# TusKANNy/seismic

Measured on AMD Instinct MI355X. Metric: queries/sec + mean latency (µs) at fixed recall@10 vs exact, SPLADE-v3 MSMARCO, higher is better.
Workload: dtype f32

## Files before the change

### include/seismic_hip_testing.h

```cpp
#ifndef SEISMIC_HIP_TESTING_H
#define SEISMIC_HIP_TESTING_H
#include "seismic_hip.h"
#ifdef __cplusplus
extern "C" {
#endif

uint32_t sgpu_debug_host_threads(void);
uint32_t sgpu_debug_chunk_bounds(uint32_t nq, uint32_t chunk_min, uint32_t chunk_max, uint32_t lanes_free, uint32_t* bounds);
uint32_t sgpu_debug_call_bounds(uint32_t nq, uint32_t chunk_min, uint32_t chunk_max, uint32_t lanes_free, uint32_t first_pm,
                                uint32_t* bounds, uint32_t cap);
uint32_t sgpu_debug_lane_chunk(sgpu_index* idx, uint32_t lane, uint32_t* info4, uint32_t* order_out, uint32_t cap);
sgpu_status sgpu_debug_pack_forward(const sgpu_index* idx, uint8_t* out_fwd, uint64_t cap, uint64_t* out_doc_ref,
                                    uint64_t* out_bytes);
sgpu_status sgpu_debug_row_dir(const sgpu_index* idx, uint32_t* out, uint64_t cap_words, uint64_t* n_words, uint32_t* n_buckets);
sgpu_status sgpu_debug_plan(const sgpu_index* idx, const uint64_t* q_off, const uint32_t* comps, const float* vals,
                            uint32_t nq, uint32_t query_cut, uint32_t* order_out, uint32_t* out3);
sgpu_status sgpu_debug_device_plan(sgpu_index* idx, const uint64_t* q_off, const uint32_t* comps, const float* vals,
                                   uint32_t nq, uint32_t query_cut, uint32_t* order_out, uint32_t* out3);
void sgpu_debug_call_timing(double* buf8);
uint32_t sgpu_debug_coop_trace(sgpu_index* idx, uint64_t* out, uint32_t cap);
sgpu_status sgpu_debug_score_stats(sgpu_index* idx, uint32_t replica, double* out8);

#ifdef __cplusplus
}
#endif
#endif
```

### seismic_amd/csrc/abi.cpp

```cpp
#include <algorithm>
#include <chrono>
#include <cstdlib>
#include <mutex>
#include <new>
#include <string>
#include <thread>
#include <vector>

#include "host_index.hpp"

struct sgpu_batch;

namespace sgpu {
struct Lane;
sgpu_status device_index_upload(const HostIndex& h, int device, DeviceIndex** out);
sgpu_status device_index_clone(const DeviceIndex* src, int device, DeviceIndex** out);
void device_index_free(DeviceIndex* d);
uint64_t device_index_bytes(const DeviceIndex* d);
Lane* lane_acquire(DeviceIndex* d);
Lane* lane_try_acquire(DeviceIndex* d);
bool call_enter(DeviceIndex* d);
void call_exit(DeviceIndex* d);
void lane_release(DeviceIndex* d, Lane* l);
Lane* lane_main(DeviceIndex* d);
sgpu_batch** lane_scratch(Lane* l);
sgpu_status batch_create(DeviceIndex* d, Lane* lane, uint64_t dim, const uint64_t* q_off, const uint32_t* comps,
                         const float* vals, uint32_t nq, uint32_t k_max, sgpu_batch** out);
void batch_free(sgpu_batch* b);
sgpu_status batch_run(DeviceIndex* d, Lane* lane, sgpu_batch* b, const sgpu_search_params& sp, uint32_t mode,
                      int sync, sgpu_launch_stats* stats);
sgpu_status batch_sync(DeviceIndex* d, sgpu_launch_stats* stats);
sgpu_status batch_fetch(DeviceIndex* d, Lane* lane, sgpu_batch* b, uint32_t k, float* out_scores, uint64_t* out_ids,
                        uint32_t* out_n);
sgpu_status batch_fetch_stats(DeviceIndex* d, sgpu_batch* b, uint32_t* out);
sgpu_status staged_launch(DeviceIndex* d, Lane* lane, uint64_t dim, const uint64_t* q_off, const uint32_t* comps,
                          const float* vals, uint32_t nq, uint32_t q_base, const sgpu_search_params& sp, sgpu_batch** slot,
                          uint32_t followed,
                          const FilterRef* flt, uint32_t chunk);
sgpu_status staged_finish(DeviceIndex* d, Lane* lane, sgpu_batch* b, float* out_scores, uint64_t* out_ids, uint32_t* out_n);
sgpu_status summary_distances(DeviceIndex* d, const HostIndex& h, uint32_t list, const uint32_t* comps,
                              const float* vals, uint32_t nnz, float* out_dots, uint32_t* out_nb);
int device_count();
double*& call_timing();
uint32_t device_plan_dots(DeviceIndex* d, const sgpu_search_params& sp, uint32_t nq, uint32_t cut);
sgpu_status debug_device_plan(DeviceIndex* d, const uint64_t* q_off, const uint32_t* comps, const float* vals, uint32_t nq,
                              uint32_t query_cut, uint32_t* order_out, uint32_t* out3);
sgpu_status debug_plan(const HostIndex& h, const uint64_t* q_off, const uint32_t* comps, const float* vals, uint32_t nq,
                       uint32_t query_cut, uint32_t* order_out, uint32_t* out3);
uint32_t coop_trace_dump(DeviceIndex* d, uint64_t* out, uint32_t cap);
uint32_t debug_lane_chunk(DeviceIndex* d, uint32_t lane, uint32_t* info4, uint32_t* order_out, uint32_t cap);
const DeviceIndex* batch_replica(const sgpu_batch* b);
sgpu_status device_index_set_knn(DeviceIndex* d, const std::vector<uint32_t>& knn, uint32_t knn_dim);
sgpu_status build_knn_on_device(DeviceIndex* d, HostIndex& h, uint32_t nknn);
sgpu_status exact_search_device(sgpu_index* idx, uint32_t replica, const uint64_t* q_off, const uint32_t* comps,
                                const float* vals, uint32_t nq, uint32_t k, float* out_scores, uint64_t* out_ids,
                                uint32_t* out_n, const sgpu_filter* filter);
sgpu_status score_documents_device(sgpu_index* idx, uint32_t replica, const uint64_t* q_off, const uint32_t* comps,
                                   const float* vals, uint32_t nq, const uint64_t* cand_off, const uint64_t* cand_ids,
                                   float* out_scores);
bool score_debug_stats(sgpu_index* idx, uint32_t replica, double* out8);
sgpu_status filter_create(sgpu_index* idx, const uint32_t* doc_ids, uint64_t n, sgpu_filter** out);
const sgpu_index* filter_index(const sgpu_filter* f);
const uint32_t* filter_host_bits(const sgpu_filter* f);
uint64_t filter_count(const sgpu_filter* f);
uint64_t filter_device_bytes(const sgpu_filter* f);
void filter_destroy(sgpu_filter* f);
bool filter_build_times(const sgpu_filter* f, uint32_t replica, double* out2);
}

using namespace sgpu;

extern "C" {

const char* sgpu_last_error(void) { return last_error().c_str(); }
uint32_t sgpu_abi_version(void) { return 4; }

sgpu_status sgpu_device_count(int32_t* n) {
  if (!n) return fail(SGPU_EINVAL, "null argument");
  *n = device_count();
  if (*n <= 0) {
    *n = 0;
    return fail(SGPU_EDEVICE, "no HIP device visible");
  }
  return SGPU_OK;
}

sgpu_status sgpu_index_create(const sgpu_index_desc* desc, sgpu_index** out) {
  if (!desc || !out) return fail(SGPU_EINVAL, "null argument");
  sgpu_index* ix = new (std::nothrow) sgpu_index();
  if (!ix) return fail(SGPU_ENOMEM, "out of memory");
  sgpu_status st = host_index_from_desc(*desc, &ix->host);
  if (st != SGPU_OK) {
    delete ix;
    return st;
  }
  *out = ix;
  return SGPU_OK;
}

sgpu_status sgpu_index_build(uint32_t comp_width, uint64_t n_docs, uint64_t dim, const uint64_t* offsets,
                             const void* comps, const float* vals, const sgpu_build_config* cfg,
                             sgpu_index** out) {
  if (!offsets || !cfg || !out || (offsets[n_docs] && (!comps || !vals))) return fail(SGPU_EINVAL, "null argument");
  sgpu_index* ix = new (std::nothrow) sgpu_index();
  if (!ix) return fail(SGPU_ENOMEM, "out of memory");
  sgpu_status st = build_host_index(comp_width, n_docs, dim, offsets, comps, vals, *cfg, &ix->host);
  if (st != SGPU_OK) {
    delete ix;
    return st;
  }
  *out = ix;
  return SGPU_OK;
}

sgpu_status sgpu_index_convert(const sgpu_index* src, uint32_t value_type, sgpu_index** out) {
  if (!src || !out) return fail(SGPU_EINVAL, "null argument");
  sgpu_index* ix = new (std::nothrow) sgpu_index();
  if (!ix) return fail(SGPU_ENOMEM, "out of memory");
  sgpu_status st = host_index_convert(src->host, value_type, &ix->host);
  if (st != SGPU_OK) {
    delete ix;
    return st;
  }
  *out = ix;
  return SGPU_OK;
}

sgpu_status sgpu_index_get_desc(const sgpu_index* idx, sgpu_index_desc* out) {
  if (!idx || !out) return fail(SGPU_EINVAL, "null argument");
  idx->host.fill_desc(out);
  return SGPU_OK;
}

sgpu_status sgpu_index_save(const sgpu_index* idx, const char* path) {
  if (!idx || !path) return fail(SGPU_EINVAL, "null argument");
  return host_index_save(idx->host, path);
}

sgpu_status sgpu_index_load(const char* path, sgpu_index** out) {
  if (!path || !out) return fail(SGPU_EINVAL, "null argument");
  sgpu_index* ix = new (std::nothrow) sgpu_index();
  if (!ix) return fail(SGPU_ENOMEM, "out of memory");
  sgpu_status st = host_index_load(path, &ix->host);
  if (st != SGPU_OK) {
    delete ix;
    return st;
  }
  *out = ix;
  return SGPU_OK;
}

struct GenerationBump {
  sgpu_index* idx;
  ~GenerationBump() { idx->generation.fetch_add(1, std::memory_order_acq_rel); }
};

static void drop_replicas(sgpu_index* idx) {
  for (ExactFile* f : idx->exact) exact_file_free(f);
  idx->exact.clear();
  for (ScoreState* s : idx->score) score_state_free(s);
  idx->score.clear();
  for (DeviceIndex* d : idx->replicas) device_index_free(d);
  idx->replicas.clear();
  idx->dev = nullptr;
}

sgpu_status sgpu_index_upload_many(sgpu_index* idx, const int32_t* device_ids, uint32_t n) {
  if (!idx || !device_ids || n == 0) return fail(SGPU_EINVAL, "null argument / no device given");
  GenerationBump bump{idx};
  drop_replicas(idx);
  DeviceIndex* first = nullptr;
  sgpu_status st = device_index_upload(idx->host, device_ids[0], &first);
  if (st != SGPU_OK) return st;
  idx->replicas.push_back(first);
  idx->dev = first;
  for (uint32_t i = 1; i < n; ++i) {
    DeviceIndex* r = nullptr;
    st = device_index_clone(first, device_ids[i], &r);
    if (st != SGPU_OK) {
      const std::string msg = last_error();
      drop_replicas(idx);
      last_error() = msg;
      return st;
    }
    idx->replicas.push_back(r);
  }
  return SGPU_OK;
}

sgpu_status sgpu_index_upload(sgpu_index* idx, int32_t device) { return sgpu_index_upload_many(idx, &device, 1); }

uint32_t sgpu_index_replicas(const sgpu_index* idx) { return idx ? (uint32_t)idx->replicas.size() : 0; }

sgpu_status sgpu_index_set_knn(sgpu_index* idx, const uint32_t* neighbours, uint64_t n_total, uint32_t knn_dim) {
  if (!idx || (n_total && !neighbours)) return fail(SGPU_EINVAL, "null argument");
  if (n_total && knn_dim == 0) return fail(SGPU_EINVAL, "knn_dim == 0 with a non-empty neighbour array");
  for (uint64_t i = 0; i < n_total; ++i)
    if (neighbours[i] >= idx->host.n_docs) return fail(SGPU_EINVAL, "neighbour id >= n_docs");
  GenerationBump bump{idx};
  try {
    idx->host.knn.assign(neighbours, neighbours + n_total);
  } catch (const std::bad_alloc&) {
    return fail(SGPU_ENOMEM, "out of memory");
  }
  idx->host.knn_dim = n_total ? knn_dim : 0;
  for (DeviceIndex* d : idx->replicas) {
    sgpu_status st = device_index_set_knn(d, idx->host.knn, idx->host.knn_dim);
    if (st != SGPU_OK) return st;
  }
  return SGPU_OK;
}

sgpu_status sgpu_index_get_knn(const sgpu_index* idx, const uint32_t** neighbours, uint64_t* n_total,
                               uint32_t* knn_dim) {
  if (!idx || !neighbours || !n_total || !knn_dim) return fail(SGPU_EINVAL, "null argument");
  *neighbours = idx->host.knn.data();
  *n_total = idx->host.knn.size();
  *knn_dim = idx->host.knn_dim;
  return SGPU_OK;
}

sgpu_status sgpu_index_build_knn(sgpu_index* idx, uint32_t nknn) {
  if (!idx) return fail(SGPU_EINVAL, "null argument");
  GenerationBump bump{idx};
  try {
    sgpu_status st = build_knn_on_device(idx->dev, idx->host, nknn);
    for (size_t i = 1; st == SGPU_OK && i < idx->replicas.size(); ++i)
      st = device_index_set_knn(idx->replicas[i], idx->host.knn, idx->host.knn_dim);
    return st;
  } catch (const std::exception&) {
    return fail(SGPU_ENOMEM, "out of host memory building the kNN graph");
  }
}

uint64_t sgpu_index_device_bytes(const sgpu_index* idx) { return idx ? device_index_bytes(idx->dev) : 0; }

sgpu_status sgpu_index_stream_stats(const sgpu_index* idx, uint64_t* raw_docs, uint64_t* raw_elements) {
  if (!idx || !raw_docs || !raw_elements) return fail(SGPU_EINVAL, "null argument");
  *raw_docs = *raw_elements = 0;
  try {
    std::vector<uint8_t> raw;
    pack_dvb_raw_flags(idx->host, &raw);
    for (uint64_t d = 0; d < raw.size(); ++d)
      if (raw[d]) {
        *raw_docs += 1;
        *raw_elements += idx->host.fwd_offsets[d + 1] - idx->host.fwd_offsets[d];
      }
  } catch (const std::bad_alloc&) {
    return fail(SGPU_ENOMEM, "out of host memory");
  }
  return SGPU_OK;
}

void sgpu_index_destroy(sgpu_index* idx) {
  if (!idx) return;
  drop_replicas(idx);
  delete idx;
}

static DeviceIndex* replica_of(sgpu_index* idx, uint32_t replica) {
  if (!idx || replica >= idx->replicas.size()) {
    fail(SGPU_EDEVICE, "index is not uploaded to a device (call sgpu_index_upload) / replica out of range");
    return nullptr;
  }
  return idx->replicas[replica];
}
static DeviceIndex* replica_of_batch(sgpu_index* idx, const sgpu_batch* b) {
  for (DeviceIndex* d : idx->replicas)
    if (batch_replica(b) == d) return d;
  fail(SGPU_EINVAL, "batch does not belong to this index");
  return nullptr;
}

sgpu_status sgpu_batch_create_on(sgpu_index* idx, uint32_t replica, const uint64_t* q_off, const uint32_t* comps,
                                 const float* vals, uint32_t nq, uint32_t k_max, sgpu_batch** out) {
  if (!idx || !q_off || !out || (q_off[nq] && (!comps || !vals))) return fail(SGPU_EINVAL, "null argument");
  *out = nullptr;
  DeviceIndex* d = replica_of(idx, replica);
  if (!d) return SGPU_EDEVICE;
  return batch_create(d, lane_main(d), idx->host.dim, q_off, comps, vals, nq, k_max, out);
}

sgpu_status sgpu_batch_create(sgpu_index* idx, const uint64_t* q_off, const uint32_t* comps, const float* vals,
                              uint32_t nq, uint32_t k_max, sgpu_batch** out) {
  return sgpu_batch_create_on(idx, 0, q_off, comps, vals, nq, k_max, out);
}

sgpu_status sgpu_batch_run(sgpu_index* idx, sgpu_batch* batch, const sgpu_search_params* params, int32_t sync,
                           sgpu_launch_stats* stats) {
  if (!idx || !batch || !params) return fail(SGPU_EINVAL, "null argument");
  DeviceIndex* d = replica_of_batch(idx, batch);
  if (!d) return SGPU_EINVAL;
  return batch_run(d, nullptr, batch, *params, 0 , sync, stats);
}

sgpu_status sgpu_batch_run_counted(sgpu_index* idx, sgpu_batch* batch, const sgpu_search_params* params,
                                   sgpu_launch_stats* stats) {
  if (!idx || !batch || !params) return fail(SGPU_EINVAL, "null argument");
  DeviceIndex* d = replica_of_batch(idx, batch);
  if (!d) return SGPU_EINVAL;
  return batch_run(d, nullptr, batch, *params, 2 , 1, stats);
}

sgpu_status sgpu_batch_sync(sgpu_index* idx, sgpu_launch_stats* stats) {
  if (!idx) return fail(SGPU_EINVAL, "null argument");
  for (size_t i = idx->replicas.size(); i-- > 1;) {
    sgpu_status st = batch_sync(idx->replicas[i], nullptr);
    if (st != SGPU_OK) return st;
  }
  return batch_sync(idx->dev, stats);
}

sgpu_status sgpu_batch_fetch(sgpu_index* idx, sgpu_batch* batch, uint32_t k, float* out_scores,
                             uint64_t* out_doc_ids, uint32_t* out_n) {
  if (!idx || !batch || !out_scores || !out_doc_ids || !out_n) return fail(SGPU_EINVAL, "null argument");
  DeviceIndex* d = replica_of_batch(idx, batch);
  if (!d) return SGPU_EINVAL;
  return batch_fetch(d, nullptr, batch, k, out_scores, out_doc_ids, out_n);
}

sgpu_status sgpu_batch_fetch_stats(sgpu_index* idx, sgpu_batch* batch, uint32_t* out_counters) {
  if (!idx || !batch || !out_counters) return fail(SGPU_EINVAL, "null argument");
  DeviceIndex* d = replica_of_batch(idx, batch);
  if (!d) return SGPU_EINVAL;
  return batch_fetch_stats(d, batch, out_counters);
}

void sgpu_batch_destroy(sgpu_batch* batch) { batch_free(batch); }

static uint32_t chunk_jobs(uint32_t nq, uint32_t chunk_min, uint32_t chunk_max) {
  if (!chunk_min) return 1u;
  const uint32_t by_rule = nq >= 2 * (uint64_t)chunk_min ? std::min<uint32_t>(chunk_max, nq / chunk_min) : 1u;
  const uint32_t by_size = (uint32_t)std::min<uint64_t>(((uint64_t)nq + kChunkQueriesMax - 1) / kChunkQueriesMax, 8u);
  return std::max(by_rule, by_size);
}
static void chunk_bounds(uint32_t nq, uint32_t n_jobs, uint32_t j, uint32_t* q0, uint32_t* q1, uint32_t first_pm = 0) {
  if (first_pm == 0 || first_pm >= 1000 || n_jobs < 2) {
    *q0 = (uint32_t)((uint64_t)nq * j / n_jobs);
    *q1 = (uint32_t)((uint64_t)nq * (j + 1) / n_jobs);
    return;
  }
  const uint32_t first = std::min<uint32_t>(std::max<uint32_t>((uint32_t)((uint64_t)nq * first_pm / 1000), 1u), nq - (n_jobs - 1));
  const uint32_t rest = nq - first;
  *q0 = j == 0 ? 0u : first + (uint32_t)((uint64_t)rest * (j - 1) / (n_jobs - 1));
  *q1 = j == 0 ? first : first + (uint32_t)((uint64_t)rest * j / (n_jobs - 1));
}
static uint32_t call_segments(uint32_t nq) {
  return (uint32_t)std::max<uint64_t>(((uint64_t)nq + 8ull * kChunkQueriesMax - 1) / (8ull * kChunkQueriesMax), 1u);
}

static sgpu_status search_segment(DeviceIndex* d, uint64_t dim, const uint64_t* q_off, const uint32_t* comps,
                                  const float* vals, uint32_t s0, uint32_t s1, uint32_t q_base, const sgpu_search_params& params,
                                  float* out_scores, uint64_t* out_doc_ids, uint32_t* out_n, const FilterRef* flt, bool shared) {
  static const uint32_t chunk_min = [] {
    const char* v = std::getenv("SGPU_CHUNK_MIN");
    return v && *v ? (uint32_t)std::strtoul(v, nullptr, 10) : 0xffffffffu;
  }();
  struct Job {
    Lane* lane;
    uint32_t q0, q1;
  };
  static const uint32_t chunk_max_env = [] {
    const char* v = std::getenv("SGPU_CHUNK_MAX");
    const uint32_t n = v && *v ? (uint32_t)std::strtoul(v, nullptr, 10) : 0u;
    return n > 8 ? 8u : n;
  }();
  static const uint32_t chunk_first_pm = [] {
    const char* t = std::getenv("SGPU_TEST_HOOKS");
    const char* v = (t && *t && *t != '0') ? std::getenv("SGPU_CHUNK_FIRST") : nullptr;
    return v && *v ? (uint32_t)std::strtoul(v, nullptr, 10) : 0u;
  }();
  const uint32_t nq = s1 - s0;
  const bool device_plans = device_plan_dots(d, params, std::min<uint32_t>(std::max<uint32_t>(nq / 2, 1u), kChunkQueriesMax), params.query_cut) != 0;
  const uint32_t chunk_max = chunk_max_env ? chunk_max_env : ((shared || device_plans) ? 2u : 4u);
  Job jobs[8];
  const uint32_t cmin = chunk_min != 0xffffffffu ? chunk_min : (device_plans ? 1300u : 600u);
  uint32_t n_jobs = chunk_jobs(nq, cmin, chunk_max);
  jobs[0].lane = lane_acquire(d);
  for (uint32_t j = 1; j < n_jobs; ++j) {
    jobs[j].lane = lane_try_acquire(d);
    if (!jobs[j].lane) {
      n_jobs = j;
      break;
    }
  }
  std::vector<uint64_t> off;
  for (;;) {
    uint32_t longest = 0;
    for (uint32_t j = 0; j < n_jobs; ++j) {
      chunk_bounds(nq, n_jobs, j, &jobs[j].q0, &jobs[j].q1, chunk_first_pm);
      jobs[j].q0 += s0;
      jobs[j].q1 += s0;
      if (jobs[j].q0 != 0) longest = std::max(longest, jobs[j].q1 - jobs[j].q0);
    }
    if (n_jobs == 1 && s0 == 0) break;
    try {
      off.resize((size_t)longest + 1);
      break;
    } catch (const std::exception&) {
      if (n_jobs == 1) {
        lane_release(d, jobs[0].lane);
        return fail(SGPU_ENOMEM, "out of host memory cutting a query batch");
      }
      for (uint32_t j = 1; j < n_jobs; ++j) lane_release(d, jobs[j].lane);
      n_jobs = 1;
    }
  }
  const uint32_t k = params.k;
  sgpu_status st = SGPU_OK;
  std::string msg;
  uint32_t launched = 0;
  if (n_jobs > 1 || s0 != 0) {
    uint32_t max_nnz = 0;
    st = q_off[0] != 0 ? fail(SGPU_EINVAL, "q_off[0] must be 0") : validate_query_offsets(q_off + s0, nq, q_base + s0, &max_nnz);
    if (st != SGPU_OK) msg = last_error();
  }
  for (uint32_t j = 0; j < n_jobs && st == SGPU_OK; ++j) {
    Job& jb = jobs[j];
    const uint64_t* qo = q_off;
    if (jb.q0 != 0) {
      for (uint32_t q = jb.q0; q <= jb.q1; ++q) off[q - jb.q0] = q_off[q] - q_off[jb.q0];
      qo = off.data();
    }
    st = staged_launch(d, jb.lane, dim, qo, comps ? comps + q_off[jb.q0] : nullptr, vals ? vals + q_off[jb.q0] : nullptr,
                       jb.q1 - jb.q0, q_base + jb.q0, params, lane_scratch(jb.lane), j + 1 < n_jobs ? 2u : (shared ? 1u : 0u),
                       flt, j);
    if (st == SGPU_OK) ++launched;
    else msg = last_error();
  }
  for (uint32_t j = 0; j < launched; ++j) {
    Job& jb = jobs[j];
    const sgpu_status fs = staged_finish(d, jb.lane, *lane_scratch(jb.lane), out_scores + (size_t)jb.q0 * k,
                                         out_doc_ids + (size_t)jb.q0 * k, out_n + jb.q0);
    if (fs != SGPU_OK && st == SGPU_OK) {
      st = fs;
      msg = last_error();
    }
  }
  for (uint32_t j = 0; j < n_jobs; ++j) lane_release(d, jobs[j].lane);
  if (st != SGPU_OK) last_error() = msg;
  return st;
}

static sgpu_status search_shard(DeviceIndex* d, uint64_t dim, const uint64_t* q_off, const uint32_t* comps,
                                const float* vals, uint32_t nq, uint32_t q_base, const sgpu_search_params& params,
                                float* out_scores, uint64_t* out_doc_ids, uint32_t* out_n, const FilterRef* flt) {
  struct InFlight {
    DeviceIndex* d;
    bool shared;
    explicit InFlight(DeviceIndex* d_) : d(d_), shared(call_enter(d_)) {}
    ~InFlight() { call_exit(d); }
  } in_flight(d);
  const uint32_t n_seg = call_segments(nq);
  sgpu_status st = SGPU_OK;
  for (uint32_t s = 0; s < n_seg && st == SGPU_OK; ++s)
    st = search_segment(d, dim, q_off, comps, vals, (uint32_t)((uint64_t)nq * s / n_seg), (uint32_t)((uint64_t)nq * (s + 1) / n_seg),
                        q_base, params, out_scores, out_doc_ids, out_n, flt, in_flight.shared);
  return st;
}

}

static sgpu_status batch_search(sgpu_index* idx, const uint64_t* q_off, const uint32_t* comps, const float* vals,
                                uint32_t nq, const sgpu_search_params* params, float* out_scores,
                                uint64_t* out_doc_ids, uint32_t* out_n, const sgpu_filter* filter) {
  if (!idx || !params || !q_off || !out_scores || !out_doc_ids || !out_n) return fail(SGPU_EINVAL, "null argument");
  if (params->k == 0) return fail(SGPU_EINVAL, "k must be > 0 (KHeap::new asserts, reference src/utils.rs:23)");
  if (idx->replicas.empty()) return fail(SGPU_EDEVICE, "index is not uploaded to a device (call sgpu_index_upload)");
  if (q_off[nq] && (!comps || !vals)) return fail(SGPU_EINVAL, "null argument");
  const uint32_t n_rep = (uint32_t)idx->replicas.size();
  if (n_rep == 1) {
    const FilterRef fr{filter, 0};
    return search_shard(idx->dev, idx->host.dim, q_off, comps, vals, nq, 0, *params, out_scores, out_doc_ids, out_n,
                        filter ? &fr : nullptr);
  }
  if (nq < 2 * n_rep) {
    const uint32_t r = idx->next_replica.fetch_add(1, std::memory_order_relaxed) % n_rep;
    const FilterRef fr{filter, r};
    return search_shard(idx->replicas[r], idx->host.dim, q_off, comps, vals, nq, 0, *params, out_scores, out_doc_ids, out_n,
                        filter ? &fr : nullptr);
  }
  {
    uint32_t max_nnz = 0;
    if (q_off[0] != 0) return fail(SGPU_EINVAL, "q_off[0] must be 0");
    const sgpu_status vst = validate_query_offsets(q_off, nq, 0, &max_nnz);
    if (vst != SGPU_OK) return vst;
  }
  const uint32_t k = params->k;
  try {
    std::vector<sgpu_status> sts(n_rep, SGPU_OK);
    std::vector<std::string> msgs(n_rep);
    std::vector<std::vector<uint64_t>> offs(n_rep);
    for (uint32_t r = 0; r < n_rep; ++r) {
      const uint32_t q0 = (uint32_t)((uint64_t)nq * r / n_rep), q1 = (uint32_t)((uint64_t)nq * (r + 1) / n_rep);
      offs[r].resize(q1 - q0 + 1);
      for (uint32_t q = q0; q <= q1; ++q) offs[r][q - q0] = q_off[q] - q_off[q0];
    }
    auto shard = [&](uint32_t r) {
      const uint32_t q0 = (uint32_t)((uint64_t)nq * r / n_rep), q1 = (uint32_t)((uint64_t)nq * (r + 1) / n_rep);
      try {
        const FilterRef fr{filter, r};
        sts[r] = search_shard(idx->replicas[r], idx->host.dim, offs[r].data(), comps ? comps + q_off[q0] : nullptr,
                              vals ? vals + q_off[q0] : nullptr, q1 - q0, q0, *params, out_scores + (size_t)q0 * k,
                              out_doc_ids + (size_t)q0 * k, out_n + q0, filter ? &fr : nullptr);
        if (sts[r] != SGPU_OK) msgs[r] = last_error();
      } catch (const std::exception&) {
        sts[r] = SGPU_ENOMEM;
      }
    };
    std::vector<std::thread> threads;
    threads.reserve(n_rep);
    for (uint32_t r = 1; r < n_rep; ++r) {
      try {
        threads.emplace_back(shard, r);
      } catch (const std::exception&) {
        shard(r);
      }
    }
    shard(0);
    for (auto& t : threads) t.join();
    for (uint32_t r = 0; r < n_rep; ++r)
      if (sts[r] != SGPU_OK) {
        if (msgs[r].empty()) return fail(sts[r], "out of host memory searching shard %u", r);
        last_error() = msgs[r];
        return sts[r];
      }
  } catch (const std::exception&) {
    return fail(SGPU_ENOMEM, "out of host memory sharding a query batch");
  }
  return SGPU_OK;
}

static sgpu_status foreign_filter(const sgpu_index* idx, const sgpu_filter* filter) {
  return filter && filter_index(filter) != idx ? fail(SGPU_EINVAL, "the filter was created on another index") : SGPU_OK;
}

extern "C" {

sgpu_status sgpu_batch_search(sgpu_index* idx, const uint64_t* q_off, const uint32_t* comps, const float* vals,
                              uint32_t nq, const sgpu_search_params* params, float* out_scores,
                              uint64_t* out_doc_ids, uint32_t* out_n) {
  return batch_search(idx, q_off, comps, vals, nq, params, out_scores, out_doc_ids, out_n, nullptr);
}

sgpu_status sgpu_batch_search_filtered(sgpu_index* idx, const uint64_t* q_off, const uint32_t* comps, const float* vals,
                                       uint32_t nq, const sgpu_search_params* params, float* out_scores,
                                       uint64_t* out_doc_ids, uint32_t* out_n, const sgpu_filter* filter) {
  const sgpu_status st = foreign_filter(idx, filter);
  if (st != SGPU_OK) return st;
  return batch_search(idx, q_off, comps, vals, nq, params, out_scores, out_doc_ids, out_n, filter);
}

sgpu_status sgpu_search_filtered(sgpu_index* idx, const uint32_t* comps, const float* vals, uint32_t nnz,
                                 const sgpu_search_params* params, float* out_scores, uint64_t* out_doc_ids,
                                 uint32_t* out_n, const sgpu_filter* filter) {
  const uint64_t q_off[2] = {0, nnz};
  return sgpu_batch_search_filtered(idx, q_off, comps, vals, 1, params, out_scores, out_doc_ids, out_n, filter);
}

sgpu_status sgpu_filter_create(sgpu_index* idx, const uint32_t* doc_ids, uint64_t n, sgpu_filter** out) {
  return filter_create(idx, doc_ids, n, out);
}
uint64_t sgpu_filter_count(const sgpu_filter* filter) { return filter_count(filter); }
uint64_t sgpu_filter_device_bytes(const sgpu_filter* filter) { return filter_device_bytes(filter); }
void sgpu_filter_destroy(sgpu_filter* filter) { filter_destroy(filter); }

sgpu_status sgpu_search(sgpu_index* idx, const uint32_t* comps, const float* vals, uint32_t nnz,
                        const sgpu_search_params* params, float* out_scores, uint64_t* out_doc_ids,
                        uint32_t* out_n) {
  const uint64_t q_off[2] = {0, nnz};
  return sgpu_batch_search(idx, q_off, comps, vals, 1, params, out_scores, out_doc_ids, out_n);
}

sgpu_status sgpu_search_sequential_timed(sgpu_index* idx, const uint64_t* q_off, const uint32_t* comps, const float* vals,
                                         uint32_t nq, const sgpu_search_params* params, float* out_scores,
                                         uint64_t* out_doc_ids, uint32_t* out_n, double* mean_us, double* breakdown_us,
                                         double* per_query_us) {
  if (!idx || !params || !q_off || !out_scores || !out_doc_ids || !out_n) return fail(SGPU_EINVAL, "null argument");
  if (params->k == 0) return fail(SGPU_EINVAL, "k must be > 0 (KHeap::new asserts, reference src/utils.rs:23)");
  double phases[8] = {0, 0, 0, 0, 0, 0, 0, 0};
  double*& slot = call_timing();
  double* const saved = slot;
  if (breakdown_us) slot = phases;
  const uint32_t k = params->k;
  sgpu_status st = SGPU_OK;
  const auto t0 = std::chrono::steady_clock::now();
  for (uint32_t q = 0; q < nq && st == SGPU_OK; ++q) {
    if (q_off[q + 1] < q_off[q] || q_off[q + 1] - q_off[q] > 0xffffffffull) {
      st = fail(SGPU_EINVAL, "query offsets must be monotone (query %u)", q);
      break;
    }
    const auto tq = per_query_us ? std::chrono::steady_clock::now() : t0;
    st = sgpu_search(idx, comps ? comps + q_off[q] : nullptr, vals ? vals + q_off[q] : nullptr,
                     (uint32_t)(q_off[q + 1] - q_off[q]), params, out_scores + (size_t)q * k,
                     out_doc_ids + (size_t)q * k, out_n + q);
    if (per_query_us) per_query_us[q] = std::chrono::duration<double, std::micro>(std::chrono::steady_clock::now() - tq).count();
  }
  const double total = std::chrono::duration<double, std::micro>(std::chrono::steady_clock::now() - t0).count();
  slot = saved;
  if (mean_us) *mean_us = nq ? total / nq : 0.0;
  if (breakdown_us)
    for (int i = 0; i < 8; ++i) breakdown_us[i] = nq ? phases[i] / nq : 0.0;
  return st;
}

sgpu_status sgpu_search_sequential(sgpu_index* idx, const uint64_t* q_off, const uint32_t* comps, const float* vals,
                                   uint32_t nq, const sgpu_search_params* params, float* out_scores,
                                   uint64_t* out_doc_ids, uint32_t* out_n, double* mean_us, double* breakdown_us) {
  return sgpu_search_sequential_timed(idx, q_off, comps, vals, nq, params, out_scores, out_doc_ids, out_n, mean_us,
                                      breakdown_us, nullptr);
}

static bool test_hooks_on() {
  const char* t = std::getenv("SGPU_TEST_HOOKS");
  return t && *t && *t != '0';
}
#define SGPU_HOOK_OR(ret)                                                                            \
  if (!test_hooks_on()) {                                                                            \
    (void)fail(SGPU_EINVAL, "%s is a test hook: set SGPU_TEST_HOOKS=1 (include/seismic_hip_testing.h)", __func__); \
    return ret;                                                                                      \
  }

uint32_t sgpu_debug_host_threads(void) {
  SGPU_HOOK_OR(0u);
  return (uint32_t)host_threads();
}

uint32_t sgpu_debug_chunk_bounds(uint32_t nq, uint32_t chunk_min, uint32_t chunk_max, uint32_t lanes_free, uint32_t* bounds) {
  SGPU_HOOK_OR(0u);
  uint32_t n_jobs = chunk_jobs(nq, chunk_min, chunk_max < 1 ? 1 : (chunk_max > 8 ? 8 : chunk_max));
  if (lanes_free >= 1 && n_jobs > lanes_free) n_jobs = lanes_free;
  for (uint32_t j = 0; j < n_jobs; ++j) chunk_bounds(nq, n_jobs, j, bounds + 2 * j, bounds + 2 * j + 1);
  return n_jobs;
}

uint32_t sgpu_debug_call_bounds(uint32_t nq, uint32_t chunk_min, uint32_t chunk_max, uint32_t lanes_free, uint32_t first_pm,
                                uint32_t* bounds, uint32_t cap) {
  SGPU_HOOK_OR(0u);
  const uint32_t n_seg = call_segments(nq);
  uint32_t n = 0;
  for (uint32_t s = 0; s < n_seg; ++s) {
    const uint32_t s0 = (uint32_t)((uint64_t)nq * s / n_seg), s1 = (uint32_t)((uint64_t)nq * (s + 1) / n_seg);
    uint32_t n_jobs = chunk_jobs(s1 - s0, chunk_min, chunk_max < 1 ? 1 : (chunk_max > 8 ? 8 : chunk_max));
    if (lanes_free >= 1 && n_jobs > lanes_free) n_jobs = lanes_free;
    for (uint32_t j = 0; j < n_jobs; ++j, ++n) {
      uint32_t q0, q1;
      chunk_bounds(s1 - s0, n_jobs, j, &q0, &q1, first_pm);
      if (n < cap) {
        bounds[2 * n] = s0 + q0;
        bounds[2 * n + 1] = s0 + q1;
      }
    }
  }
  return n;
}

uint32_t sgpu_debug_lane_chunk(sgpu_index* idx, uint32_t lane, uint32_t* info4, uint32_t* order_out, uint32_t cap) {
  SGPU_HOOK_OR(0u);
  if (!idx || !idx->dev || !info4) return 0u;
  return debug_lane_chunk(idx->dev, lane, info4, order_out, cap);
}

sgpu_status sgpu_debug_pack_forward(const sgpu_index* idx, uint8_t* out_fwd, uint64_t cap, uint64_t* out_doc_ref, uint64_t* out_bytes) {
  SGPU_HOOK_OR(SGPU_EINVAL);
  if (!idx || !out_bytes) return fail(SGPU_EINVAL, "null argument");
  try {
    std::vector<uint8_t> raw, fwd;
    std::vector<uint64_t> off16, dref;
    pack_dvb_raw_flags(idx->host, &raw);
    pack_record_offsets(idx->host, raw, 128 / 16, &off16);
    *out_bytes = std::max<uint64_t>(off16[idx->host.n_docs] * 16, 16);
    if (!out_fwd) return SGPU_OK;
    if (cap < *out_bytes || !out_doc_ref) return fail(SGPU_EINVAL, "buffer too small");
    pack_records(idx->host, raw, off16, &fwd);
    pack_doc_refs(idx->host, raw, off16, &dref);
    std::memcpy(out_fwd, fwd.data(), fwd.size());
    std::memcpy(out_doc_ref, dref.data(), dref.size() * 8);
  } catch (const std::bad_alloc&) {
    return fail(SGPU_ENOMEM, "out of host memory");
  }
  return SGPU_OK;
}

sgpu_status sgpu_debug_row_dir(const sgpu_index* idx, uint32_t* out, uint64_t cap_words, uint64_t* n_words, uint32_t* n_buckets) {
  SGPU_HOOK_OR(SGPU_EINVAL);
  if (!idx || !n_words || !n_buckets) return fail(SGPU_EINVAL, "null argument");
  try {
    std::vector<uint16_t> mid;
    std::vector<uint32_t> dir;
    pack_row_mid(idx->host, &mid);
    *n_buckets = 0;
    if (!pack_row_dir(idx->host, mid, &dir, n_buckets)) *n_buckets = 0;
    *n_words = dir.size();
    if (!out) return SGPU_OK;
    if (cap_words < dir.size()) return fail(SGPU_EINVAL, "buffer too small");
    std::memcpy(out, dir.data(), dir.size() * 4);
  } catch (const std::bad_alloc&) {
    return fail(SGPU_ENOMEM, "out of host memory");
  }
  return SGPU_OK;
}

sgpu_status sgpu_debug_plan(const sgpu_index* idx, const uint64_t* q_off, const uint32_t* comps, const float* vals, uint32_t nq,
                            uint32_t query_cut, uint32_t* order_out, uint32_t* out3) {
  SGPU_HOOK_OR(SGPU_EINVAL);
  if (!idx || !q_off || !order_out || !out3) return fail(SGPU_EINVAL, "null argument");
  return debug_plan(idx->host, q_off, comps, vals, nq, query_cut, order_out, out3);
}

sgpu_status sgpu_debug_device_plan(sgpu_index* idx, const uint64_t* q_off, const uint32_t* comps, const float* vals, uint32_t nq,
                                   uint32_t query_cut, uint32_t* order_out, uint32_t* out3) {
  SGPU_HOOK_OR(SGPU_EINVAL);
  if (!idx || !q_off || !order_out || !out3) return fail(SGPU_EINVAL, "null argument");
  return debug_device_plan(idx->dev, q_off, comps, vals, nq, query_cut, order_out, out3);
}

void sgpu_debug_call_timing(double* buf8) {
  SGPU_HOOK_OR();
  call_timing() = buf8;
}

uint32_t sgpu_debug_coop_trace(sgpu_index* idx, uint64_t* out, uint32_t cap) {
  SGPU_HOOK_OR(0u);
  return idx ? coop_trace_dump(idx->dev, out, cap) : 0;
}

sgpu_status sgpu_summary_distances(sgpu_index* idx, uint32_t list, const uint32_t* comps, const float* vals,
                                   uint32_t nnz, float* out_dots, uint32_t* out_n_blocks) {
  if (!idx || !out_dots || !out_n_blocks || (nnz && (!comps || !vals))) return fail(SGPU_EINVAL, "null argument");
  return summary_distances(idx->dev, idx->host, list, comps, vals, nnz, out_dots, out_n_blocks);
}

sgpu_status sgpu_exact_search(const sgpu_index* idx, const uint64_t* q_off, const uint32_t* comps,
                              const float* vals, uint32_t nq, uint32_t k, uint32_t num_threads,
                              float* out_scores, uint64_t* out_doc_ids, uint32_t* out_n) {
  if (!idx || !q_off || !out_scores || !out_doc_ids || !out_n) return fail(SGPU_EINVAL, "null argument");
  return exact_search_host(idx->host, q_off, comps, vals, nq, k, num_threads, out_scores, out_doc_ids, out_n);
}

sgpu_status sgpu_exact_search_filtered(const sgpu_index* idx, const uint64_t* q_off, const uint32_t* comps,
                                       const float* vals, uint32_t nq, uint32_t k, uint32_t num_threads,
                                       float* out_scores, uint64_t* out_doc_ids, uint32_t* out_n,
                                       const sgpu_filter* filter) {
  if (!filter) return sgpu_exact_search(idx, q_off, comps, vals, nq, k, num_threads, out_scores, out_doc_ids, out_n);
  const sgpu_status st = foreign_filter(idx, filter);
  if (st != SGPU_OK) return st;
  if (!idx || !q_off || !out_scores || !out_doc_ids || !out_n) return fail(SGPU_EINVAL, "null argument");
  return exact_search_host(idx->host, q_off, comps, vals, nq, k, num_threads, out_scores, out_doc_ids, out_n,
                           filter_host_bits(filter));
}

sgpu_status sgpu_exact_search_device(sgpu_index* idx, uint32_t replica, const uint64_t* q_off, const uint32_t* comps,
                                     const float* vals, uint32_t nq, uint32_t k, float* out_scores,
                                     uint64_t* out_doc_ids, uint32_t* out_n) {
  return exact_search_device(idx, replica, q_off, comps, vals, nq, k, out_scores, out_doc_ids, out_n, nullptr);
}

sgpu_status sgpu_exact_search_device_filtered(sgpu_index* idx, uint32_t replica, const uint64_t* q_off,
                                              const uint32_t* comps, const float* vals, uint32_t nq, uint32_t k,
                                              float* out_scores, uint64_t* out_doc_ids, uint32_t* out_n,
                                              const sgpu_filter* filter) {
  const sgpu_status st = foreign_filter(idx, filter);
  if (st != SGPU_OK) return st;
  return exact_search_device(idx, replica, q_off, comps, vals, nq, k, out_scores, out_doc_ids, out_n, filter);
}

sgpu_status sgpu_score_documents(sgpu_index* idx, uint32_t replica, const uint64_t* q_off, const uint32_t* comps,
                                 const float* vals, uint32_t nq, const uint64_t* cand_off, const uint64_t* cand_ids,
                                 float* out_scores) {
  return score_documents_device(idx, replica, q_off, comps, vals, nq, cand_off, cand_ids, out_scores);
}

sgpu_status sgpu_score_documents_host(const sgpu_index* idx, const uint64_t* q_off, const uint32_t* comps, const float* vals,
                                      uint32_t nq, const uint64_t* cand_off, const uint64_t* cand_ids, uint32_t num_threads,
                                      float* out_scores) {
  if (!idx) return fail(SGPU_EINVAL, "null argument");
  return score_documents_host(idx->host, q_off, comps, vals, nq, cand_off, cand_ids, num_threads, out_scores);
}

sgpu_status sgpu_debug_score_stats(sgpu_index* idx, uint32_t replica, double* out8) {
  SGPU_HOOK_OR(SGPU_EINVAL);
  if (!idx || !out8) return fail(SGPU_EINVAL, "null argument");
  if (!score_debug_stats(idx, replica, out8)) return fail(SGPU_EINVAL, "no score call has run on replica %u", replica);
  return SGPU_OK;
}

sgpu_status sgpu_debug_filter_build_times(const sgpu_filter* filter, uint32_t replica, double* out2) {
  SGPU_HOOK_OR(SGPU_EINVAL);
  if (!filter || !out2) return fail(SGPU_EINVAL, "null argument");
  if (!filter_build_times(filter, replica, out2)) return fail(SGPU_EINVAL, "the filter has no view on replica %u", replica);
  return SGPU_OK;
}

}
```

### seismic_amd/csrc/device_index.hip

```cpp
#include <hip/hip_runtime.h>

#include <algorithm>
#include <atomic>
#include <chrono>
#include <cmath>
#include <condition_variable>
#include <cstdlib>
#include <cstring>
#include <mutex>
#include <unordered_map>
#include <vector>

#include "device_types.hpp"
#include "filter.hpp"
#include "host_index.hpp"

namespace sgpu {

hipError_t run_u16_dense(const LaunchArgs& a, int* occupancy);
hipError_t run_u16_packed(const LaunchArgs& a, int* occupancy);
hipError_t run_u32_split(const LaunchArgs& a, int* occupancy);
hipError_t run_u32_packed(const LaunchArgs& a, int* occupancy);
hipError_t run_u32_hash(const LaunchArgs& a, int* occupancy);
hipError_t run_u16_dense_u8(const LaunchArgs& a, int* occupancy);
hipError_t run_u16_packed_u8(const LaunchArgs& a, int* occupancy);
hipError_t run_u32_packed_u8(const LaunchArgs& a, int* occupancy);
hipError_t run_u32_split_u8(const LaunchArgs& a, int* occupancy);
hipError_t run_u16_dense_dvb(const LaunchArgs& a, int* occupancy);
hipError_t run_u16_packed_dvb(const LaunchArgs& a, int* occupancy);

static hipError_t run_any(const LaunchArgs& a, int* occ) {
  if (a.comp_width == 2 && a.lookup != LK_DENSE && a.lookup != LK_PACKED) return hipErrorInvalidConfiguration;
  if (a.value_type == SGPU_VAL_DOTVBYTE)
    return a.lookup == LK_DENSE ? run_u16_dense_dvb(a, occ) : run_u16_packed_dvb(a, occ);
  if (a.value_type == SGPU_VAL_FIXEDU8 && a.comp_width == 4) return a.lookup == LK_SPLIT ? run_u32_split_u8(a, occ) : run_u32_packed_u8(a, occ);
  if (a.value_type == SGPU_VAL_FIXEDU8) return a.lookup == LK_DENSE ? run_u16_dense_u8(a, occ) : run_u16_packed_u8(a, occ);
  if (a.comp_width == 2) return a.lookup == LK_DENSE ? run_u16_dense(a, occ) : run_u16_packed(a, occ);
  if (a.lookup == LK_HASH) return run_u32_hash(a, occ);
  return a.lookup == LK_SPLIT ? run_u32_split(a, occ) : run_u32_packed(a, occ);
}
hipError_t occupancy_search(const LaunchArgs& a, int* blocks_per_cu) { return run_any(a, blocks_per_cu); }
hipError_t launch_search(const LaunchArgs& a) { return run_any(a, nullptr); }

#define HIP_TRY(expr)                                                                          \
  do {                                                                                         \
    hipError_t e_ = (expr);                                                                    \
    if (e_ != hipSuccess)                                                                      \
      return fail(SGPU_EDEVICE, "%s failed: %s (%s:%d)", #expr, hipGetErrorString(e_), __FILE__, __LINE__); \
  } while (0)

static const char* hook_raw(const char* name) {
  const char* t = std::getenv("SGPU_TEST_HOOKS");
  return (t && *t && *t != '0') ? std::getenv(name) : nullptr;
}

}
struct sgpu_batch;
namespace sgpu {
void batch_free(sgpu_batch* b);

struct Lane {
  hipStream_t stream = nullptr;
  uint32_t* queue = nullptr;
  uint32_t queue_pos = 0;
  bool queue_dirty = true;
  uint32_t done_seq = 0;
  sgpu_batch* scratch = nullptr;
  uint32_t* bitmaps = nullptr;
  uint32_t bitmaps_slots = 0;
  uint8_t* coop = nullptr;
  size_t coop_bytes = 0, coop_trace_off = 0;
  uint32_t coop_trace_n = 0;
  bool coop_last = false;
  std::vector<hipEvent_t> ev0, ev1;
  int ev_pending = 0;
  double sum_ms = 0;
  uint32_t n_timed = 0;
  sgpu_launch_stats last{};
  bool busy = false;
};

struct Alloc {
  void* p;
  size_t bytes;
  size_t field;
};

struct DeviceIndex {
  int device = -1;
  DevView view{};
  uint32_t comp_width = 2;
  std::vector<Alloc> allocs;
  uint64_t bytes = 0;
  uint32_t n_cu = 0;
  uint32_t max_lds = 0;
  std::vector<uint32_t> list_nb, list_np;
  uint32_t max_nb = 0;
  uint32_t value_type = SGPU_VAL_F16;
  float val_scale = 0.0f;
  bool fwd_block_major = false;
  bool coop_broken = false;
  static constexpr int kMainEvents = 64, kPool = 8;
  Lane main;
  Lane pool[kPool];
  std::unordered_map<uint64_t, int> occupancy;
  std::unordered_map<uint32_t, uint32_t> plan_dots_seen;
  std::mutex mu;
  std::atomic<uint32_t> calls_inflight{0};
  std::atomic<int64_t> concurrent_seen_us{-((int64_t)1 << 60)};
  std::mutex pool_mu;
  std::condition_variable pool_cv;
};

static sgpu_status lane_init(Lane* l, int n_events) {
  if (hipStreamCreateWithFlags(&l->stream, hipStreamNonBlocking) != hipSuccess)
    return fail(SGPU_EDEVICE, "hipStreamCreate failed");
  if (hipMalloc((void**)&l->queue, 256) != hipSuccess) return fail(SGPU_ENOMEM, "hipMalloc(queue) failed");
  if (hipMemset(l->queue, 0, 256) != hipSuccess) return fail(SGPU_EDEVICE, "hipMemset(queue) failed");
  for (int i = 0; i < n_events; ++i) {
    hipEvent_t a, b;
    if (hipEventCreate(&a) != hipSuccess) return fail(SGPU_EDEVICE, "hipEventCreate failed");
    l->ev0.push_back(a);
    if (hipEventCreate(&b) != hipSuccess) return fail(SGPU_EDEVICE, "hipEventCreate failed");
    l->ev1.push_back(b);
  }
  return SGPU_OK;
}

static void lane_free(Lane* l) {
  if (l->stream) (void)hipStreamSynchronize(l->stream);
  if (l->scratch) batch_free(l->scratch);
  if (l->queue) (void)hipFree(l->queue);
  if (l->bitmaps) (void)hipFree(l->bitmaps);
  if (l->coop) (void)hipFree(l->coop);
  for (hipEvent_t e : l->ev0) (void)hipEventDestroy(e);
  for (hipEvent_t e : l->ev1) (void)hipEventDestroy(e);
  if (l->stream) (void)hipStreamDestroy(l->stream);
  *l = Lane{};
}

Lane* lane_acquire(DeviceIndex* d) {
  std::unique_lock<std::mutex> lk(d->pool_mu);
  for (;;) {
    for (Lane& l : d->pool)
      if (!l.busy) {
        l.busy = true;
        return &l;
      }
    d->pool_cv.wait(lk);
  }
}

Lane* lane_try_acquire(DeviceIndex* d) {
  std::lock_guard<std::mutex> lk(d->pool_mu);
  int n_free = 0;
  for (Lane& l : d->pool) n_free += !l.busy;
  if (n_free < 2) return nullptr;
  for (Lane& l : d->pool)
    if (!l.busy) {
      l.busy = true;
      return &l;
    }
  return nullptr;
}

static inline int64_t mono_us() {
  return (int64_t)std::chrono::duration_cast<std::chrono::microseconds>(std::chrono::steady_clock::now().time_since_epoch()).count();
}
bool call_enter(DeviceIndex* d) {
  const uint32_t n = d->calls_inflight.fetch_add(1, std::memory_order_relaxed) + 1u;
  const int64_t now = mono_us();
  if (n > 1) d->concurrent_seen_us.store(now, std::memory_order_relaxed);
  return n > 1 || now - d->concurrent_seen_us.load(std::memory_order_relaxed) < 50000;
}
void call_exit(DeviceIndex* d) {
  if (d->calls_inflight.fetch_sub(1, std::memory_order_relaxed) > 1u) d->concurrent_seen_us.store(mono_us(), std::memory_order_relaxed);
}

void lane_release(DeviceIndex* d, Lane* l) {
  {
    std::lock_guard<std::mutex> lk(d->pool_mu);
    l->busy = false;
  }
  d->pool_cv.notify_one();
}

Lane* lane_main(DeviceIndex* d) { return &d->main; }
sgpu_batch** lane_scratch(Lane* l) { return &l->scratch; }

template <class T>
static sgpu_status dev_copy(DeviceIndex* d, const T* src, size_t n, const T** out) {
  void* p = nullptr;
  const size_t bytes = std::max<size_t>(n, 1) * sizeof(T);
  if (hipMalloc(&p, bytes) != hipSuccess) return fail(SGPU_ENOMEM, "hipMalloc of %zu bytes failed", bytes);
  d->allocs.push_back(Alloc{p, bytes, (size_t)((const char*)out - (const char*)d)});
  d->bytes += bytes;
  if (hook_raw("SGPU_DEBUG_ALLOC")) std::fprintf(stderr, "sgpu alloc: field@%zu %p..%p\n", (size_t)((const char*)out - (const char*)d), p, (void*)((char*)p + bytes));
  if (n) HIP_TRY(hipMemcpy(p, src, n * sizeof(T), hipMemcpyHostToDevice));
  *out = (const T*)p;
  return SGPU_OK;
}

void device_index_free(DeviceIndex* d) {
  if (!d) return;
  if (d->device >= 0) (void)hipSetDevice(d->device);
  lane_free(&d->main);
  for (Lane& l : d->pool) lane_free(&l);
  for (const Alloc& a : d->allocs) (void)hipFree(a.p);
  delete d;
}

uint64_t device_index_bytes(const DeviceIndex* d) { return d ? d->bytes : 0; }
int device_index_device(const DeviceIndex* d) { return d->device; }
const DevView& device_index_view(const DeviceIndex* d) { return d->view; }

int device_count() {
  int n = 0;
  if (hipGetDeviceCount(&n) != hipSuccess) return 0;
  return n;
}

__global__ __launch_bounds__(256) void replicate_records_kernel(uint8_t* fwd, const uint64_t* __restrict__ doc_ref,
                                                                const uint32_t* __restrict__ post_doc,
                                                                const uint64_t* __restrict__ post_ref, uint64_t n_postings,
                                                                uint32_t bytes_per_elem, uint32_t dvb) {
  const uint64_t g = ((uint64_t)blockIdx.x * blockDim.x + threadIdx.x) >> 4;
  const uint32_t sub = threadIdx.x & 15;
  const uint64_t n_groups = ((uint64_t)gridDim.x * blockDim.x) >> 4;
  for (uint64_t p = g; p < n_postings; p += n_groups) {
    const uint64_t dst = post_ref[p], src = doc_ref[post_doc[p]];
    uint32_t n16;
    if (dvb && !(dst & 0x8000u)) {
      const uint32_t ns = (((uint32_t)dst & 0x7fffu) + 7u) >> 3;
      n16 = (ns * 20u + 15u) >> 4;
    } else {
      const uint32_t len = (uint32_t)dst & (dvb ? 0x7fffu : 0xffffu);
      n16 = (((len + 7u) & ~7u) * bytes_per_elem + 15u) >> 4;
    }
    const uint4* s4 = (const uint4*)(fwd + (src >> 16) * 16ull);
    uint4* d4 = (uint4*)(fwd + (dst >> 16) * 16ull);
    for (uint32_t i = sub; i < n16; i += 16) d4[i] = s4[i];
  }
}

sgpu_status device_index_upload(const HostIndex& h, int device, DeviceIndex** out) {
  int n_dev = 0;
  if (hipGetDeviceCount(&n_dev) != hipSuccess || n_dev <= 0)
    return fail(SGPU_EDEVICE, "no HIP device available (the search path has no CPU fallback)");
  if (device < 0 || device >= n_dev) return fail(SGPU_EDEVICE, "device %d out of range (0..%d)", device, n_dev - 1);
  if (h.n_blocks() >= 0xffffffffull || h.n_postings() >= 0xffffffffull || h.n_rows() >= 0xffffffffull)
    return fail(SGPU_ELIMIT, "index too large for 32-bit device offsets (blocks / postings / summary rows)");
  HIP_TRY(hipSetDevice(device));
  DeviceIndex* d = new DeviceIndex();
  d->device = device;
  d->comp_width = h.comp_width;
  sgpu_status st = SGPU_OK;
  auto bail = [&](sgpu_status s) {
    device_index_free(d);
    return s;
  };
  hipDeviceProp_t prop;
  if (hipGetDeviceProperties(&prop, device) != hipSuccess) return bail(fail(SGPU_EDEVICE, "hipGetDeviceProperties failed"));
  d->n_cu = (uint32_t)prop.multiProcessorCount;
  d->max_lds = (uint32_t)prop.sharedMemPerBlock;
  if ((st = lane_init(&d->main, DeviceIndex::kMainEvents)) != SGPU_OK) return bail(st);
  for (Lane& l : d->pool)
    if ((st = lane_init(&l, 1)) != SGPU_OK) return bail(st);

  try {
    const uint32_t cw = h.comp_width, vb = h.val_bytes();
    d->value_type = h.value_type;
    d->val_scale = h.val_scale;
    std::vector<uint64_t> rec_off16;
    std::vector<uint8_t> dvb_raw;
    pack_dvb_raw_flags(h, &dvb_raw);
    {
      const char* env_line = hook_raw("SGPU_REC_LINE");
      pack_record_offsets(h, dvb_raw, std::max<uint64_t>(16, env_line ? std::strtoul(env_line, nullptr, 10) : 128) / 16, &rec_off16);
    }
    if (rec_off16[h.n_docs] >= (1ull << 48)) return bail(fail(SGPU_ELIMIT, "forward index exceeds 48-bit record offsets"));
    std::vector<uint8_t> fwd;
    pack_records(h, dvb_raw, rec_off16, &fwd);
    const uint64_t doc_units = rec_off16[h.n_docs];
    std::vector<uint64_t> pref;
    uint64_t blk_units = 0;
    {
      std::vector<uint64_t> bsize;
      pack_block_sizes(h, dvb_raw, &bsize);
      blk_units = bsize[h.n_blocks()];
      size_t free_b = 0, total_b = 0;
      (void)hipMemGetInfo(&free_b, &total_b);
      const char* env_layout = std::getenv("SGPU_FWD_LAYOUT");
      const uint64_t need = (doc_units + blk_units) * 16 + h.n_postings() * 24 + h.n_entries() * 8;
      bool block_major = blk_units > 0 && (doc_units + 8 + blk_units) < (1ull << 48) &&
                         need < (uint64_t)(0.6 * (double)free_b) && blk_units * 16 <= (96ull << 30);
      if (env_layout && std::strcmp(env_layout, "doc") == 0) block_major = false;
      if (env_layout && std::strcmp(env_layout, "block") == 0 && blk_units > 0) block_major = true;
      const uint64_t blk_base = (doc_units + 7) & ~7ull;
      void* fp = nullptr;
      size_t fbytes = 0;
      for (;;) {
        const uint64_t total_units = block_major ? blk_base + blk_units : doc_units;
        fbytes = std::max<uint64_t>(total_units * 16, 16) + 16;
        if (hipMalloc(&fp, fbytes) == hipSuccess) break;
        (void)hipGetLastError();
        if (!block_major) return bail(fail(SGPU_ENOMEM, "hipMalloc of %zu bytes failed", fbytes));
        block_major = false;
      }
      d->fwd_block_major = block_major;
      pack_post_refs(h, dvb_raw, rec_off16, bsize, block_major, blk_base, &pref);
      d->allocs.push_back(Alloc{fp, fbytes, (size_t)((const char*)&d->view.fwd - (const char*)d)});
      d->bytes += fbytes;
      d->view.fwd = (const uint8_t*)fp;
      if (hook_raw("SGPU_DEBUG_ALLOC")) std::fprintf(stderr, "sgpu alloc: fwd %p..%p\n", fp, (void*)((char*)fp + fbytes));
      HIP_TRY(hipMemcpy(fp, fwd.data(), fwd.size(), hipMemcpyHostToDevice));
    }
    fwd.clear();
    fwd.shrink_to_fit();
    if ((st = dev_copy(d, pref.data(), pref.size(), &d->view.post_ref)) != SGPU_OK) return bail(st);
    {
      std::vector<uint64_t> dref;
      pack_doc_refs(h, dvb_raw, rec_off16, &dref);
      if ((st = dev_copy(d, dref.data(), dref.size(), &d->view.doc_ref)) != SGPU_OK) return bail(st);
    }
    pref.clear();
    pref.shrink_to_fit();
    if ((st = dev_copy(d, h.post_doc.data(), h.post_doc.size(), &d->view.post_doc)) != SGPU_OK) return bail(st);
    if (d->fwd_block_major && h.n_postings()) {
      (void)hipGetLastError();
      hipLaunchKernelGGL(replicate_records_kernel, dim3(d->n_cu * 8), dim3(256), 0, d->main.stream,
                         (uint8_t*)d->view.fwd, d->view.doc_ref, d->view.post_doc, d->view.post_ref,
                         (uint64_t)h.n_postings(), (uint32_t)(cw + vb), (uint32_t)(!dvb_raw.empty()));
      HIP_TRY(hipGetLastError());
      HIP_TRY(hipStreamSynchronize(d->main.stream));
    }
    auto narrow = [](const std::vector<uint64_t>& v) {
      std::vector<uint32_t> o;
      pack_narrow(v, &o);
      return o;
    };
    {
      auto v = narrow(h.list_block_start);
      if ((st = dev_copy(d, v.data(), v.size(), &d->view.list_block_start)) != SGPU_OK) return bail(st);
      v = narrow(h.block_post_start);
      if ((st = dev_copy(d, v.data(), v.size(), &d->view.block_post_start)) != SGPU_OK) return bail(st);
    }
    if ((st = dev_copy(d, h.sum_bid.data(), h.sum_bid.size(), &d->view.sum_bid)) != SGPU_OK) return bail(st);
    {
      std::vector<uint16_t> mid;
      pack_row_mid(h, &mid);
      d->view.list_row_start = nullptr;
      d->view.row_ptr = nullptr;
      d->view.row_comp = nullptr;
      d->view.row_mid = nullptr;
      d->view.row_dir = nullptr;
      d->view.row_dir_buckets = 0;
      if (cw == 2) {
        std::vector<uint32_t> dir;
        uint32_t n_buckets = 0;
        if (!pack_row_dir(h, mid, &dir, &n_buckets))
          return bail(fail(SGPU_ELIMIT, h.dim > 65535 ? "u16 components need dim <= 65535 for the device's row directory"
                                                       : "the index has too many summary rows for the device's row directory (2^31 buckets)"));
        static_assert(sizeof(d->view.row_dir) == sizeof(const uint32_t*), "pointer field");
        if ((st = dev_copy(d, dir.data(), dir.size(), (const uint32_t**)&d->view.row_dir)) != SGPU_OK) return bail(st);
        d->view.row_dir_buckets = n_buckets;
      } else {
        auto v = narrow(h.list_row_start);
        if ((st = dev_copy(d, v.data(), v.size(), &d->view.list_row_start)) != SGPU_OK) return bail(st);
        if ((st = dev_copy(d, h.row_ptr.data(), h.row_ptr.size(), &d->view.row_ptr)) != SGPU_OK) return bail(st);
        static_assert(sizeof(d->view.row_comp) == sizeof(const uint8_t*), "pointer field");
        if ((st = dev_copy(d, h.row_comp.data(), h.row_comp.size(), (const uint8_t**)&d->view.row_comp)) != SGPU_OK)
          return bail(st);
        if ((st = dev_copy(d, mid.data(), mid.size(), &d->view.row_mid)) != SGPU_OK) return bail(st);
      }
    }
    {
      std::vector<float> deq;
      pack_sum_deq(h, &deq);
      if ((st = dev_copy(d, deq.data(), deq.size(), &d->view.sum_deq)) != SGPU_OK) return bail(st);
    }
    d->view.knn = nullptr;
    d->view.knn_total = 0;
    d->view.knn_dim = 0;
    if (!h.knn.empty() && h.knn_dim) {
      if ((st = dev_copy(d, h.knn.data(), h.knn.size(), &d->view.knn)) != SGPU_OK) return bail(st);
      d->view.knn_total = h.knn.size();
      d->view.knn_dim = h.knn_dim;
    }
    d->view.dim = (uint32_t)h.dim;
    d->view.n_docs = (uint32_t)h.n_docs;
    d->view.n_bitmap_words = (uint32_t)((h.n_docs + 31) / 32);
    d->list_nb.resize(h.dim);
    d->list_np.resize(h.dim);
    for (uint64_t c = 0; c < h.dim; ++c) {
      d->list_nb[c] = (uint32_t)(h.list_block_start[c + 1] - h.list_block_start[c]);
      d->list_np[c] = (uint32_t)(h.block_post_start[h.list_block_start[c + 1]] - h.block_post_start[h.list_block_start[c]]);
      d->max_nb = std::max(d->max_nb, d->list_nb[c]);
    }
  } catch (const std::bad_alloc&) {
    return bail(fail(SGPU_ENOMEM, "out of host memory packing the index for upload"));
  }
  *out = d;
  return SGPU_OK;
}

sgpu_status device_index_clone(const DeviceIndex* src, int device, DeviceIndex** out) {
  int n_dev = 0;
  if (hipGetDeviceCount(&n_dev) != hipSuccess || n_dev <= 0) return fail(SGPU_EDEVICE, "no HIP device available");
  if (device < 0 || device >= n_dev) return fail(SGPU_EDEVICE, "device %d out of range (0..%d)", device, n_dev - 1);
  HIP_TRY(hipSetDevice(device));
  if (device != src->device) {
    int can = 0;
    (void)hipDeviceCanAccessPeer(&can, device, src->device);
    if (can) {
      const hipError_t e = hipDeviceEnablePeerAccess(src->device, 0);
      if (e != hipSuccess && e != hipErrorPeerAccessAlreadyEnabled) (void)hipGetLastError();
    }
  }
  DeviceIndex* d = new DeviceIndex();
  d->device = device;
  d->comp_width = src->comp_width;
  d->view = src->view;
  d->n_cu = src->n_cu;
  d->max_lds = src->max_lds;
  d->list_nb = src->list_nb;
  d->list_np = src->list_np;
  d->max_nb = src->max_nb;
  d->fwd_block_major = src->fwd_block_major;
  d->value_type = src->value_type;
  d->val_scale = src->val_scale;
  auto bail = [&](sgpu_status s) {
    device_index_free(d);
    return s;
  };
  hipDeviceProp_t prop;
  if (hipGetDeviceProperties(&prop, device) != hipSuccess) return bail(fail(SGPU_EDEVICE, "hipGetDeviceProperties failed"));
  d->n_cu = (uint32_t)prop.multiProcessorCount;
  d->max_lds = (uint32_t)prop.sharedMemPerBlock;
  sgpu_status st;
  if ((st = lane_init(&d->main, DeviceIndex::kMainEvents)) != SGPU_OK) return bail(st);
  for (Lane& l : d->pool)
    if ((st = lane_init(&l, 1)) != SGPU_OK) return bail(st);
  for (const Alloc& a : src->allocs) *(const void**)((char*)d + a.field) = nullptr;
  for (const Alloc& a : src->allocs) {
    void* p = nullptr;
    if (hipMalloc(&p, a.bytes) != hipSuccess) return bail(fail(SGPU_ENOMEM, "hipMalloc of %zu bytes failed on device %d", a.bytes, device));
    d->allocs.push_back(Alloc{p, a.bytes, a.field});
    d->bytes += a.bytes;
    *(const void**)((char*)d + a.field) = p;
    const hipError_t e = hipMemcpyPeerAsync(p, device, a.p, src->device, a.bytes, d->main.stream);
    if (e != hipSuccess) return bail(fail(SGPU_EDEVICE, "hipMemcpyPeerAsync %d -> %d failed: %s", src->device, device, hipGetErrorString(e)));
  }
  if (hipStreamSynchronize(d->main.stream) != hipSuccess) return bail(fail(SGPU_EDEVICE, "peer copy failed"));
  *out = d;
  return SGPU_OK;
}

}

struct sgpu_batch_plan {
  uint32_t query_cut = 0;
  uint32_t dots_cap = 1;
  uint32_t max_nb = 0;
  uint32_t max_list_nb = 1;
  std::vector<uint32_t> order;
  bool hash_ok = true;
};

struct sgpu_batch {
  std::vector<uint64_t> h_off;
  std::vector<uint32_t> h_off32;
  std::vector<uint32_t> h_comp;
  std::vector<float> h_val;
  std::vector<sgpu_batch_plan> plans;
  int device = -1;
  const sgpu::DeviceIndex* owner = nullptr;
  uint32_t nq = 0, k_max = 0, max_nnz = 0;
  uint64_t cap_nq = 0, cap_nnz = 0, cap_slab = 0;
  uint32_t* q_off = nullptr;
  uint32_t* q_comp = nullptr;
  float* q_val = nullptr;
  uint32_t* q_order = nullptr;
  uint32_t* h_order = nullptr;
  uint32_t order_cut = 0xffffffffu;
  float* out_scores = nullptr;
  uint64_t* out_ids = nullptr;
  uint32_t* out_n = nullptr;
  uint32_t* out_stats = nullptr;
  uint32_t* status = nullptr;
  size_t status_off = 0;
  bool staged = false;
  uint8_t* arena_dev = nullptr;
  uint8_t* arena_host = nullptr;
  uint8_t* arena_host_dev = nullptr;
  bool direct_out = false;
  uint32_t done_seq = 0;
  bool direct_in = false;
  uint32_t queue_base = 0;
  size_t arena_cap = 0, in_bytes = 0, out_off = 0, out_bytes = 0;
  uint32_t* queue_dev = nullptr;
  uint32_t device_plan_cut = 0xffffffffu;
  bool followed = false;
  bool plan_identity = false;
  uint32_t q_base = 0;
  size_t order_off = 0;
};

namespace sgpu {

}
extern char** environ;
namespace sgpu {
struct EnvCache {
  uint64_t fp = 0;
  int n = 0;
  struct E {
    const char* name;
    const char* val;
  } e[96];
};
static thread_local EnvCache tl_env;
static void env_refresh() {
  uint64_t h = 1469598103934665603ull;
  for (char** p = environ; p && *p; ++p) h = (h ^ (uint64_t)(uintptr_t)*p) * 1099511628211ull;
  if (h != tl_env.fp || tl_env.n == 0) {
    tl_env.fp = h;
    tl_env.n = 0;
  }
}
static const char* env_get(const char* name) {
  EnvCache& c = tl_env;
  for (int i = 0; i < c.n; ++i)
    if (c.e[i].name == name) return c.e[i].val;
  const char* v = std::getenv(name);
  if (c.n < (int)(sizeof(c.e) / sizeof(c.e[0]))) c.e[c.n++] = EnvCache::E{name, v};
  return v;
}
static uint32_t env_u32(const char* name, uint32_t dflt) {
  const char* v = env_get(name);
  if (!v || !*v) return dflt;
  return (uint32_t)std::strtoul(v, nullptr, 10);
}
static bool hooks_on() {
  const char* v = env_get("SGPU_TEST_HOOKS");
  return v && *v && *v != '0';
}
static void hook_ignored(const char* name) {
  static std::atomic<bool> said{false};
  const char* v = env_get(name);
  if (v && *v && !said.exchange(true))
    std::fprintf(stderr, "seismic_hip: %s is a test hook and is ignored unless SGPU_TEST_HOOKS=1 is set (further ignored hooks are not reported)\n", name);
}
static uint32_t hook_u32(const char* name, uint32_t dflt) {
  if (hooks_on()) return env_u32(name, dflt);
  hook_ignored(name);
  return dflt;
}
static const char* hook_get(const char* name) {
  if (hooks_on()) return env_get(name);
  hook_ignored(name);
  return nullptr;
}

double*& call_timing() {
  static thread_local double* t = nullptr;
  return t;
}
static inline double now_us() {
  return (double)std::chrono::duration_cast<std::chrono::nanoseconds>(std::chrono::steady_clock::now().time_since_epoch()).count() * 1e-3;
}
struct PhaseClock {
  double* acc;
  double t;
  PhaseClock() : acc(call_timing()), t(acc ? now_us() : 0.0) {}
  inline void lap(int i) {
    if (!acc) return;
    const double n = now_us();
    acc[i] += n - t;
    t = n;
  }
};

static hipError_t wait_lane(hipStream_t s, uint32_t nq, const volatile uint32_t* done = nullptr, uint32_t done_seq = 0) {
  const char* wv = env_get("SGPU_WAIT");
  const int mode = (wv && !std::strcmp(wv, "block")) ? 0 : ((wv && !std::strcmp(wv, "spin")) ? 2 : 1);
  const double spin_us = (double)env_u32("SGPU_SPIN_US", 2000);
  if (mode == 2 || (mode == 1 && nq <= 256)) {
    const double t0 = now_us();
    for (;;) {
      if (done && __atomic_load_n((const uint32_t*)done, __ATOMIC_ACQUIRE) == done_seq) return hipSuccess;
      const hipError_t e = hipStreamQuery(s);
      if (e == hipSuccess) return hipSuccess;
      if (e != hipErrorNotReady) return e;
      if (now_us() - t0 > spin_us) break;
#if defined(__x86_64__) || defined(__i386__)
      __builtin_ia32_pause();
#elif defined(__aarch64__)
      asm volatile("yield");
#endif
    }
  }
  return hipStreamSynchronize(s);
}

void batch_free(sgpu_batch* b) {
  if (!b) return;
  if (b->device >= 0) (void)hipSetDevice(b->device);
  if (b->staged) {
    (void)hipFree(b->arena_dev);
    (void)hipHostFree(b->arena_host);
    delete b;
    return;
  }
  (void)hipFree(b->q_off);
  (void)hipFree(b->q_comp);
  (void)hipFree(b->q_val);
  (void)hipFree(b->q_order);
  (void)hipHostFree(b->h_order);
  (void)hipFree(b->out_scores);
  (void)hipFree(b->out_ids);
  (void)hipFree(b->out_n);
  (void)hipFree(b->out_stats);
  delete b;
}

sgpu_status batch_create(DeviceIndex* d, Lane* lane, uint64_t dim, const uint64_t* q_off, const uint32_t* comps,
                         const float* vals, uint32_t nq, uint32_t k_max, sgpu_batch** out) {
  if (!d) return fail(SGPU_EDEVICE, "index is not uploaded to a device (call sgpu_index_upload)");
  if (k_max == 0) return fail(SGPU_EINVAL, "k == 0");
  if (k_max > 1024) return fail(SGPU_ELIMIT, "k = %u exceeds the heap limit of 1024", k_max);
  uint32_t max_nnz = 0;
  sgpu_status st = validate_queries(dim, q_off, comps, vals, nq, &max_nnz);
  if (st != SGPU_OK) return st;
  HIP_TRY(hipSetDevice(d->device));
  const uint64_t nnz = q_off[nq];
  const size_t slab = std::max<size_t>((size_t)nq * k_max, 1);
  sgpu_batch* b = *out;
  const bool reuse = b && b->owner == d && b->cap_nq >= nq && b->cap_nnz >= nnz && b->cap_slab >= slab;
  if (b && !reuse) {
    HIP_TRY(hipStreamSynchronize(lane->stream));
    batch_free(b);
    b = nullptr;
    *out = nullptr;
  }
  if (reuse) HIP_TRY(hipStreamSynchronize(lane->stream));
  try {
    if (!b) b = new sgpu_batch();
    b->device = d->device;
    b->owner = d;
    b->nq = nq;
    b->k_max = k_max;
    b->max_nnz = max_nnz;
    b->plans.clear();
    b->order_cut = 0xffffffffu;
    b->h_off.assign(q_off, q_off + nq + 1);
    b->h_comp.assign(comps, comps + nnz);
    b->h_val.assign(vals, vals + nnz);
    b->h_off32.resize((size_t)nq + 1);
  } catch (const std::bad_alloc&) {
    if (!reuse) delete b;
    else b->nq = 0;
    return fail(SGPU_ENOMEM, "out of host memory creating a query batch");
  }
  for (uint32_t q = 0; q <= nq; ++q) b->h_off32[q] = (uint32_t)q_off[q];
  bool ok = true;
  if (!reuse) {
    b->cap_nq = std::max<uint64_t>(nq, 1);
    b->cap_nnz = std::max<uint64_t>(nnz, 1);
    b->cap_slab = slab;
    ok = hipMalloc((void**)&b->q_off, (b->cap_nq + 1) * 4) == hipSuccess &&
         hipMalloc((void**)&b->q_comp, b->cap_nnz * 4) == hipSuccess &&
         hipMalloc((void**)&b->q_val, b->cap_nnz * 4) == hipSuccess &&
         hipMalloc((void**)&b->q_order, b->cap_nq * 8) == hipSuccess &&
         hipHostMalloc((void**)&b->h_order, b->cap_nq * 8, hipHostMallocDefault) == hipSuccess &&
         hipMalloc((void**)&b->out_scores, std::max<size_t>(slab, 65536) * 4) == hipSuccess &&
         hipMalloc((void**)&b->out_ids, slab * 8) == hipSuccess &&
         hipMalloc((void**)&b->out_n, b->cap_nq * 4) == hipSuccess &&
         hipMalloc((void**)&b->out_stats, b->cap_nq * STATS_WORDS * 4) == hipSuccess;
  }
  if (!ok) {
    batch_free(b);
    *out = nullptr;
    return fail(SGPU_ENOMEM, "hipMalloc failed creating a query batch");
  }
  ok = hipMemcpyAsync(b->q_off, b->h_off32.data(), (nq + 1) * 4, hipMemcpyHostToDevice, lane->stream) == hipSuccess &&
       (nnz == 0 ||
        (hipMemcpyAsync(b->q_comp, b->h_comp.data(), nnz * 4, hipMemcpyHostToDevice, lane->stream) == hipSuccess &&
         hipMemcpyAsync(b->q_val, b->h_val.data(), nnz * 4, hipMemcpyHostToDevice, lane->stream) == hipSuccess));
  if (!ok) {
    (void)hipStreamSynchronize(lane->stream);
    batch_free(b);
    *out = nullptr;
    return fail(SGPU_EDEVICE, "hipMemcpy of the query batch failed");
  }
  *out = b;
  return SGPU_OK;
}

const DeviceIndex* batch_replica(const sgpu_batch* b) { return b ? b->owner : nullptr; }
static inline size_t al16_(size_t x) { return (x + 15) & ~(size_t)15; }

static sgpu_status make_plan(const DeviceIndex* d, const uint64_t* h_off, const uint32_t* h_comp, const float* h_val,
                             uint32_t nq, uint32_t query_cut, sgpu_batch_plan* out) {
  try {
    sgpu_batch_plan& pl = *out;
    pl.query_cut = query_cut;
    std::vector<uint64_t> keys(nq);
    uint32_t max_nb = 0, dots_cap = 1, max_list_nb = 1;
    {
      constexpr uint32_t kSmall = 16;
      std::vector<std::pair<int32_t, uint32_t>> kv;
      for (int64_t q = 0; q < (int64_t)nq; ++q) {
        const uint64_t qa = h_off[q], qe = h_off[q + 1];
        int32_t tk[kSmall];
        uint32_t tc[kSmall];
        const uint32_t* sel = tc;
        size_t nl = 0;
        if (query_cut == 0) {
        } else if (query_cut <= kSmall) {
          for (uint64_t i = qa; i < qe; ++i) {
            const int32_t key = total_key(h_val[i]);
            if (nl == query_cut && !(key > tk[nl - 1])) continue;
            size_t j = nl < query_cut ? nl++ : nl - 1;
            while (j > 0 && tk[j - 1] < key) {
              tk[j] = tk[j - 1];
              tc[j] = tc[j - 1];
              --j;
            }
            tk[j] = key;
            tc[j] = h_comp[i];
          }
        } else {
          kv.clear();
          for (uint64_t i = qa; i < qe; ++i) kv.emplace_back(total_key(h_val[i]), h_comp[i]);
          nl = std::min<size_t>(query_cut, kv.size());
          std::partial_sort(kv.begin(), kv.begin() + (long)nl, kv.end(),
                            [](const std::pair<int32_t, uint32_t>& a, const std::pair<int32_t, uint32_t>& c) {
                              if (a.first != c.first) return a.first > c.first;
                              return a.second < c.second;
                            });
        }
        uint64_t np = 0;
        uint32_t nb = 0;
        for (size_t i = 0; i < nl; ++i) {
          const uint32_t c = query_cut <= kSmall ? sel[i] : kv[i].second;
          nb += d->list_nb[c];
          np += d->list_np[c];
          max_list_nb = std::max(max_list_nb, d->list_nb[c]);
        }
        const uint32_t c0 = nl ? (query_cut <= kSmall ? sel[0] : kv[0].second) : 0xffffffffu;
        if (nl) max_nb = std::max(max_nb, d->list_nb[c0]);
        dots_cap = std::max(dots_cap, nb);
        keys[(size_t)q] = ((uint64_t)(0xffffffffu - (uint32_t)std::min<uint64_t>(np, 0xffffffffull)) << 32) | (uint32_t)q;
      }
    }
    pl.max_nb = max_nb;
    pl.dots_cap = dots_cap;
    pl.max_list_nb = max_list_nb;
    std::sort(keys.begin(), keys.end());
    pl.order.resize(2 * (size_t)nq);
    for (uint32_t i = 0; i < nq; ++i) pl.order[i] = (uint32_t)keys[i];
    pl.hash_ok = d->view.dim < (1u << 24) && d->comp_width == 4 && d->value_type == SGPU_VAL_F16 && !hook_u32("SGPU_NO_HASH", 0);
    if (pl.hash_ok) {
      std::vector<uint32_t> stamp(kHashSlots, 0xffffffffu);
      uint32_t epoch = 0;
      for (uint32_t q = 0; q < nq && pl.hash_ok; ++q) {
        const uint64_t a = h_off[q], e = h_off[q + 1];
        uint32_t seed = kHashSeeds;
        if (e - a <= kHashSlots / 4)
          for (uint32_t s = 0; s < kHashSeeds && seed == kHashSeeds; ++s) {
            const uint32_t mult = hash_mult(s);
            bool clash = false;
            for (uint64_t i = a; i < e && !clash; ++i) {
              uint32_t& slot = stamp[hash_slot(h_comp[i], mult)];
              clash = slot == epoch;
              slot = epoch;
            }
            ++epoch;
            if (!clash) seed = s;
          }
        if (seed == kHashSeeds) pl.hash_ok = false;
        pl.order[(size_t)nq + q] = seed & (kHashSeeds - 1);
      }
    }
  } catch (const std::bad_alloc&) {
    return fail(SGPU_ENOMEM, "out of host memory planning a query batch");
  }
  return SGPU_OK;
}

sgpu_status debug_plan(const HostIndex& h, const uint64_t* q_off, const uint32_t* comps, const float* vals, uint32_t nq,
                       uint32_t query_cut, uint32_t* order_out, uint32_t* out3) {
  DeviceIndex d;
  d.comp_width = h.comp_width;
  d.view.dim = (uint32_t)h.dim;
  d.list_nb.resize(h.dim);
  d.list_np.resize(h.dim);
  for (uint64_t c = 0; c < h.dim; ++c) {
    d.list_nb[c] = (uint32_t)(h.list_block_start[c + 1] - h.list_block_start[c]);
    d.list_np[c] = (uint32_t)(h.block_post_start[h.list_block_start[c + 1]] - h.block_post_start[h.list_block_start[c]]);
  }
  sgpu_batch_plan pl;
  env_refresh();
  const sgpu_status st = make_plan(&d, q_off, comps, vals, nq, query_cut, &pl);
  if (st != SGPU_OK) return st;
  for (uint32_t i = 0; i < nq; ++i) order_out[i] = pl.order[i];
  out3[0] = pl.dots_cap;
  out3[1] = pl.max_nb;
  out3[2] = pl.max_list_nb;
  return SGPU_OK;
}

static_assert((uint32_t)kDevicePlanMaxQueries == kChunkQueriesMax, "abi.cpp cuts calls by kChunkQueriesMax");
uint32_t device_plan_dots(DeviceIndex* d, const sgpu_search_params& sp, uint32_t nq, uint32_t cut) {
  env_refresh();
  const bool hash_family = d->comp_width == 4 && d->value_type == SGPU_VAL_F16 && d->view.dim < (1u << 24);
  if (nq < kDevicePlanMinQueries || nq > kDevicePlanMaxQueries || cut < 1 || cut > kDevicePlanCutMax || sp.first_sorted ||
      hash_family || !env_u32("SGPU_DEVICE_PLAN", 1) || hook_u32("SGPU_NO_LPT", 0))
    return 0;
  std::lock_guard<std::mutex> lock(d->mu);
  const auto it = d->plan_dots_seen.find(cut);
  return it != d->plan_dots_seen.end() ? it->second : 0u;
}
bool later_chunks_on_host() {
  env_refresh();
  const char* v = env_get("SGPU_CHUNK_PLAN");
  return !(v && !std::strcmp(v, "device"));
}

sgpu_status debug_device_plan(DeviceIndex* d, const uint64_t* q_off, const uint32_t* comps, const float* vals, uint32_t nq,
                              uint32_t query_cut, uint32_t* order_out, uint32_t* out3) {
  if (!d) return fail(SGPU_EDEVICE, "index is not uploaded to a device");
  if (nq == 0 || nq > kDevicePlanMaxQueries || query_cut == 0 || query_cut > kDevicePlanCutMax)
    return fail(SGPU_EINVAL, "the device plans 1 ... %u queries at query_cut 1 ... %u", (unsigned)kDevicePlanMaxQueries, (unsigned)kDevicePlanCutMax);
  HIP_TRY(hipSetDevice(d->device));
  const uint64_t nnz = q_off[nq];
  uint32_t n2 = 2;
  while (n2 < nq) n2 <<= 1;
  std::vector<uint32_t> off32((size_t)nq + 1);
  for (uint32_t q = 0; q <= nq; ++q) off32[q] = (uint32_t)q_off[q];
  const size_t o_comp = al16_((size_t)(nq + 1) * 4), o_val = o_comp + al16_(nnz * 4), o_keys = o_val + al16_(nnz * 4),
               o_max = o_keys + (size_t)n2 * 8, o_order = o_max + 16, total = o_order + (size_t)nq * 4;
  uint8_t* buf = nullptr;
  if (hipMalloc((void**)&buf, total) != hipSuccess) return fail(SGPU_ENOMEM, "hipMalloc of %zu bytes failed", total);
  hipError_t e = hipMemcpy(buf, off32.data(), (size_t)(nq + 1) * 4, hipMemcpyHostToDevice);
  if (e == hipSuccess && nnz) e = hipMemcpy(buf + o_comp, comps, nnz * 4, hipMemcpyHostToDevice);
  if (e == hipSuccess && nnz) e = hipMemcpy(buf + o_val, vals, nnz * 4, hipMemcpyHostToDevice);
  if (e == hipSuccess) e = hipMemset(buf + o_max, 0, 16);
  if (e == hipSuccess)
    e = launch_device_plan(d->view, (const uint32_t*)buf, (const uint32_t*)(buf + o_comp), (const float*)(buf + o_val), nq, query_cut,
                           (uint64_t*)(buf + o_keys), (uint32_t*)(buf + o_max), (uint32_t*)(buf + o_order), d->main.stream);
  if (e == hipSuccess) e = hipStreamSynchronize(d->main.stream);
  if (e == hipSuccess) e = hipMemcpy(order_out, buf + o_order, (size_t)nq * 4, hipMemcpyDeviceToHost);
  if (e == hipSuccess) e = hipMemcpy(out3, buf + o_max, 12, hipMemcpyDeviceToHost);
  (void)hipFree(buf);
  if (e != hipSuccess) return fail(SGPU_EDEVICE, "device plan failed: %s", hipGetErrorString(e));
  return SGPU_OK;
}

static sgpu_status plan_for(DeviceIndex* d, sgpu_batch* b, uint32_t query_cut, const sgpu_batch_plan** out) {
  for (const auto& pl : b->plans)
    if (pl.query_cut == query_cut) {
      *out = &pl;
      return SGPU_OK;
    }
  if (b->staged) return fail(SGPU_EINVAL, "a staged batch is planned when it is staged");
  sgpu_batch_plan pl;
  sgpu_status st = make_plan(d, b->h_off.data(), b->h_comp.data(), b->h_val.data(), b->nq, query_cut, &pl);
  if (st != SGPU_OK) return st;
  try {
    b->plans.push_back(std::move(pl));
  } catch (const std::bad_alloc&) {
    return fail(SGPU_ENOMEM, "out of host memory planning a query batch");
  }
  *out = &b->plans.back();
  return SGPU_OK;
}

static bool coop_by_size(const DeviceIndex* d, uint32_t nq) {
  const char* v = env_get("SGPU_COOP_MAX_NQ");
  if (v && *v) return nq <= (uint32_t)std::strtoul(v, nullptr, 10);
  return nq <= d->n_cu * 11u / 16u || (nq > d->n_cu && nq <= d->n_cu * 7u / 4u);
}

static sgpu_status configure(DeviceIndex* d, Lane* lane, sgpu_batch* b, const sgpu_search_params& sp, uint32_t mode,
                             LaunchArgs* a, const DevView* ov = nullptr) {
  if (sp.k == 0) return fail(SGPU_EINVAL, "k must be > 0 (KHeap::new asserts, reference src/utils.rs:23)");
  if (sp.k > b->k_max) return fail(SGPU_EINVAL, "k = %u exceeds the batch's k_max = %u", sp.k, b->k_max);
  if (std::isnan(sp.heap_factor)) return fail(SGPU_EINVAL, "heap_factor is NaN");
  uint32_t NT = hook_u32("SGPU_BLOCK", (mode != MODE_DOTS && b->nq <= d->n_cu) ? 1024 : 512);
  if (NT != 512 && NT != 1024) return fail(SGPU_EINVAL, "SGPU_BLOCK must be 512 or 1024");
  const bool want_counted = mode == MODE_COUNTED || hook_u32("SGPU_VISITED_BITMAP", 0);
  if (NT == 1024 && (want_counted || heap_variant(sp.k) > 2)) NT = 512;
  const uint32_t qn = std::max<uint32_t>(4, (b->max_nnz + 3u) & ~3u);
  const bool searching = mode != MODE_DOTS;
  const uint32_t cut = mode == MODE_DOTS ? 1u : std::min<uint32_t>(sp.query_cut, qn);
  const uint32_t qc = std::max<uint32_t>(1, cut);
  const uint32_t words = d->view.dim / 32 + 1;
  uint32_t items_max = hook_u32("SGPU_ITEMS_MAX", 1024);
  uint32_t dots_cap = 1, sort_nb = 0;
  const sgpu_batch_plan* pl = nullptr;
  if (mode == MODE_DOTS) {
    dots_cap = std::max<uint32_t>(1, d->list_nb[sp.query_cut]);
  } else {
    sgpu_status pst = plan_for(d, b, cut, &pl);
    if (pst != SGPU_OK) return pst;
    dots_cap = pl->dots_cap;
    sort_nb = pl->max_nb;
  }
  const uint64_t lds_limit = std::min<uint32_t>(d->max_lds ? d->max_lds : 65536, 160 * 1024);
  auto up = [](uint64_t x) { return (x + 15ull) & ~15ull; };
  LdsLayout L{};
  uint64_t o = 0;
  static_assert(kQscOffset == 0, "the weights come first");
  L.q_sc = (uint32_t)o; o += up(((uint64_t)qn + 1) * 4);
  L.q_val = L.q_sc;
  if (d->value_type != SGPU_VAL_F16) {
    L.q_val = (uint32_t)o;
    o += up(((uint64_t)qn + 1) * 4);
  }
  L.q_comp = (uint32_t)o; o += up((uint64_t)qn * 4);
  L.sel = (uint32_t)o; o += up((6ull * qc + 1) * 4);
  const uint64_t target = hook_u32("SGPU_LDS_TARGET", 160u * 1024u / 2u);
  const uint64_t rest = up((sp.first_sorted && searching) ? (uint64_t)sort_nb * 2 : 0) + up(2 * (NT / 64 + 1) * 4) +
                        up((uint64_t)heap_variant(sp.k) * 64 * 8) +
                        up(kStateWords * 4) +
                        ((d->comp_width == 2 && d->view.dim <= 65535 && b->max_nnz <= 255) ? up((uint64_t)d->view.dim + 1)
                                                                                           : up((uint64_t)words * 6)) +
                        up(512 * 16 + NT * 12);
  auto rt_bytes = [&](uint64_t g) { return up(g * qn * 8) + up(g * qn * 2) + up(2ull * g * (qn + 1) * 4); };
  uint32_t qg = qc;
  if (pl && qc > 4 && o + rt_bytes(qc) + rest + (uint64_t)dots_cap * 4 > target) qg = 4;
  qg = std::max<uint32_t>(1, std::min<uint32_t>(qg, hook_u32("SGPU_LIST_GROUP", qc)));
  if (o + rt_bytes(qg) > lds_limit)
    return fail(SGPU_ELIMIT, "query_cut %u x %u query components do not fit the row tables in LDS", qc, qn);
  L.rt_start = (uint32_t)o; o += up((uint64_t)qg * qn * 8);
  L.rt_mid = (uint32_t)o; o += up((uint64_t)qg * qn * 2);
  L.rt_pre = (uint32_t)o; o += up(2ull * qg * (qn + 1) * 4);
  if (pl && (uint64_t)dots_cap * 4 > 24u * 1024u) {
    const uint64_t fit = target > o + rest ? (target - o - rest) / 4 : 0;
    dots_cap = (uint32_t)std::max<uint64_t>(pl->max_list_nb, std::min<uint64_t>(dots_cap, std::max<uint64_t>(fit, 6144)));
  }
  dots_cap = std::min<uint32_t>(dots_cap, hook_u32("SGPU_DOTS_CAP", 0xffffffffu));
  if (pl) dots_cap = std::max(dots_cap, pl->max_list_nb);
  L.dots_cap = dots_cap;
  L.dots = (uint32_t)o; o += up((uint64_t)dots_cap * 4);
  L.order = (uint32_t)o; o += up((sp.first_sorted && searching) ? (uint64_t)sort_nb * 2 : 0);
  L.part = (uint32_t)o; o += up(2 * (NT / 64 + 1) * 4);
  L.heap = (uint32_t)o; o += up((uint64_t)heap_variant(sp.k) * 64 * 8);
  L.st = (uint32_t)o; o += up(kStateWords * 4);
  uint64_t sort_bytes = 0;
  if (sp.first_sorted && searching && sort_nb > 1) {
    uint64_t n2 = 1;
    while (n2 < sort_nb) n2 <<= 1;
    sort_bytes = n2 * 8;
  }
  if (o > lds_limit)
    return fail(SGPU_ELIMIT, "query needs %llu bytes of LDS before its lookup table (dots %u blocks) > %llu available",
                (unsigned long long)o, dots_cap, (unsigned long long)lds_limit);
  const uint64_t budget = hook_u32("SGPU_LDS_TARGET", 160u * 1024u / 2u);
  const uint64_t dense_bytes = std::max<uint64_t>(up((uint64_t)d->view.dim + 1), hook_u32("SGPU_DENSE_BYTES", 0)), bitmap_bytes = up((uint64_t)words * 8);
  const bool dense_ok = d->comp_width == 2 && d->view.dim <= 65535 && b->max_nnz <= 255 &&
                        !hook_u32("SGPU_NO_DENSE", 0) && searching;
  const uint64_t split_bits = up((uint64_t)words * 4), split_bytes = split_bits + up((uint64_t)words * 2);
  const bool coop_wanted = [&] {
    const char* cm = env_get("SGPU_COOP");
    const bool force = cm && !std::strcmp(cm, "force");
    const bool off = (cm && !std::strcmp(cm, "0")) || d->coop_broken;
    return !off && !want_counted && mode == MODE_SEARCH && (force || coop_by_size(d, b->nq)) &&
           variant_built(NT, heap_variant(sp.k), false, true);
  }();
  const bool stream_wanted = !coop_wanted && !want_counted && mode == MODE_SEARCH && hook_u32("SGPU_STREAM", 1) &&
                             variant_built(NT, heap_variant(sp.k), false, false, true);
  const uint32_t ring_cap = [&] {
    uint32_t r = std::min<uint32_t>(1024, std::max<uint32_t>(256, hook_u32("SGPU_RING_MAX", 1024)));
    while (r & (r - 1)) r &= r - 1;
    return r;
  }();
  auto ring_of = [&](uint32_t items) { return std::min<uint32_t>(ring_cap, items >= 1024 ? 1024u : (items >= 512 ? 512u : 256u)); };
  auto uni_for = [&](uint32_t items) {
    if (stream_wanted)
      return up(std::max<uint64_t>(std::max<uint64_t>(stream_ring_bytes(ring_of(items)), 128 * 16 + NT * 12), sort_bytes));
    return up(std::max<uint64_t>((uint64_t)items * 16 + NT * 12, sort_bytes));
  };
  const uint64_t smallest_lookup = (d->comp_width == 4) ? split_bytes : bitmap_bytes;
  const uint32_t want_items = items_max;
  if (!hook_get("SGPU_ITEMS_MAX")) {
    const uint32_t want = items_max;
    if (dense_ok)
      while (items_max > 512 && o + dense_bytes + uni_for(items_max) > budget) items_max -= 128;
    if (!dense_ok || o + dense_bytes + uni_for(items_max) > budget) {
      items_max = want;
      while (items_max > 256 && o + smallest_lookup + uni_for(items_max) > budget) items_max -= 128;
    }
  }
  const uint64_t min_uni = uni_for(items_max);
  const bool dense = dense_ok && (o + dense_bytes + min_uni <= budget || hook_u32("SGPU_FORCE_DENSE", 0));
  const bool split = !dense && d->comp_width == 4 && b->max_nnz <= 65535 &&
                     (o + bitmap_bytes + min_uni > budget || hook_u32("SGPU_FORCE_SPLIT", 0)) &&
                     !hook_u32("SGPU_NO_SPLIT", 0);
  const uint64_t hash_bytes = (uint64_t)kHashSlots * 8;
  const bool hash_family = d->comp_width == 4 && d->value_type == SGPU_VAL_F16;
  bool hashed = searching && hash_family && pl && pl->hash_ok && !hook_u32("SGPU_NO_LPT", 0) && !hook_u32("SGPU_NO_HASH", 0) &&
                !hook_u32("SGPU_FORCE_SPLIT", 0) && !hook_u32("SGPU_FORCE_DENSE", 0) &&
                (d->comp_width == 4 || !dense || hook_u32("SGPU_FORCE_HASH", 0));
  if (hashed && !hook_get("SGPU_ITEMS_MAX") && !hook_u32("SGPU_FORCE_HASH", 0)) {
    uint32_t im = want_items;
    while (im > 512 && o + hash_bytes + uni_for(im) > budget) im -= 128;
    if (o + hash_bytes + uni_for(im) <= budget) items_max = im;
    else hashed = false;
  } else if (hashed && !hook_u32("SGPU_FORCE_HASH", 0) && o + hash_bytes + uni_for(items_max) > budget) {
    hashed = false;
  }
  const uint32_t lookup = hashed ? LK_HASH : (dense ? LK_DENSE : (split ? LK_SPLIT : LK_PACKED));
  const uint64_t lookup_bytes =
      mode == MODE_DOTS ? 0u : (hashed ? hash_bytes : (dense ? dense_bytes : (split ? split_bytes : bitmap_bytes)));
  L.q_bits = (uint32_t)o;
  L.q_rank = (uint32_t)(o + (split && !hashed ? split_bits : lookup_bytes));
  o += lookup_bytes;
  L.uni = (uint32_t)std::min<uint64_t>(o, 0xffffffffu);
  const uint64_t uni = uni_for(items_max);
  o += uni;
  L.qc = qc;
  L.qn = qn;
  L.qg = qg;
  a->lookup = lookup;
  if (o > lds_limit)
    return fail(SGPU_ELIMIT,
                "query needs %llu bytes of LDS (dots %u blocks, %u-word bitmap, sort %llu B) > %llu available; "
                "lower query_cut / use first_sorted=0 / rebuild with a smaller centroid_fraction",
                (unsigned long long)o, dots_cap, words, (unsigned long long)sort_bytes, (unsigned long long)lds_limit);
  L.total = (uint32_t)o;
  a->L = L;
  a->p.k = sp.k;
  a->p.query_cut = cut;
  a->p.heap_factor = sp.heap_factor;
  a->p.first_sorted = sp.first_sorted != 0;
  a->p.mode = mode == MODE_COUNTED ? (uint32_t)MODE_SEARCH : mode;
  a->p.n_knn = mode == MODE_DOTS ? 0u : sp.n_knn;
  a->counted = want_counted ? 1u : 0u;
  const uint32_t ring = stream_wanted ? ring_of(items_max) : 0u;
  if (stream_wanted) items_max = std::max<uint32_t>(128, std::min<uint32_t>(1024, (uint32_t)((uni - NT * 12) / 16) & ~127u));
  a->p.items_max = items_max;
  a->p.items_init = std::min<uint32_t>(items_max, hook_u32("SGPU_ITEMS_INIT", 128));
  a->p.items_min = std::min<uint32_t>(a->p.items_init, hook_u32("SGPU_ITEMS_MIN", 64));
  a->p.rblocks_max = std::min<uint32_t>(32, std::max<uint32_t>(1, hook_u32("SGPU_RBLOCKS", 8)));
  a->p.target_list = mode == MODE_DOTS ? sp.query_cut : 0;
  a->p.val_scale = d->val_scale;
  a->p.queue_base = b->staged ? b->queue_base : 0u;
  a->value_type = d->value_type;
  a->ix = ov ? *ov : d->view;
  a->comp_width = d->comp_width;
  a->block = NT;
  a->lds_bytes = (uint32_t)o;
  if (env_u32("SGPU_DEBUG", 0))
    std::fprintf(stderr, "sgpu configure: nq %u NT %u lookup %u items_max %u ring %u dots_cap %u lists/group %u of %u uni %llu lds %llu\n", b->nq, NT, lookup,
                 items_max, ring, dots_cap, qg, qc, (unsigned long long)uni, (unsigned long long)o);
  a->stream = lane->stream;
  a->qb.q_off = b->q_off;
  a->qb.q_comp = b->q_comp;
  a->qb.q_val = b->q_val;
  a->qb.nq = b->nq;
  a->qb.k_stride = b->k_max;
  a->qb.out_scores = b->out_scores;
  a->qb.out_ids = b->out_ids;
  a->qb.out_n = b->out_n;
  a->qb.q_order = nullptr;
  a->qb.q_seed = nullptr;
  if (pl && !hook_u32("SGPU_NO_LPT", 0) && b->nq && !b->plan_identity) {
    if (b->order_cut != cut) {
      if (b->order_cut != 0xffffffffu) HIP_TRY(hipStreamSynchronize(lane->stream));
      std::memcpy(b->h_order, pl->order.data(), (size_t)b->nq * 8);
      HIP_TRY(hipMemcpyAsync(b->q_order, b->h_order, (size_t)b->nq * 8, hipMemcpyHostToDevice, lane->stream));
      b->order_cut = cut;
    }
    a->qb.q_order = b->q_order;
    a->qb.q_seed = b->q_order + b->nq;
  }
  a->qb.out_stats = mode != MODE_DOTS ? b->out_stats : nullptr;
  a->qb.status = b->staged ? b->status : lane->queue + 32;
  a->qb.done = nullptr;
  a->qb.done_seq = 0;
  a->coop = CoopView{};
  {
    const char* cm = env_get("SGPU_COOP");
    const bool force = cm && !std::strcmp(cm, "force");
    const bool off = (cm && !std::strcmp(cm, "0")) || d->coop_broken;
    if (!off && !a->counted && mode == MODE_SEARCH && a->lds_bytes - a->L.uni >= 4096 && (force || coop_by_size(d, b->nq)) &&
        variant_built(NT, heap_variant(sp.k), false, true))
      a->coop.enabled = force ? 2u : 1u;
  }
  a->streamed = 0;
  a->p.ring = 0;
  if (stream_wanted && !a->coop.enabled && dots_cap <= 65535u && stream_ring_bytes(ring) <= a->lds_bytes - a->L.uni) {
    a->streamed = 1;
    a->p.ring = ring;
    a->p.items_init = std::min<uint32_t>(std::min<uint32_t>(hook_u32("SGPU_ITEMS_INIT", 128), 1024), ring);
    a->p.items_min = std::min<uint32_t>(a->p.items_min, a->p.items_init);
  }
  int per_cu = 0;
  {
    const uint64_t key = ((uint64_t)(a->streamed != 0) << 59) | ((uint64_t)(a->coop.enabled != 0) << 58) | ((uint64_t)a->comp_width << 56) | ((uint64_t)a->counted << 55) | ((uint64_t)a->value_type << 52) | ((uint64_t)a->block << 40) | ((uint64_t)a->lookup << 36) |
                         ((uint64_t)heap_variant(a->p.k) << 28) | (uint64_t)(a->lds_bytes >> 4);
    auto it = d->occupancy.find(key);
    if (it == d->occupancy.end()) {
      HIP_TRY(occupancy_search(*a, &per_cu));
      d->occupancy[key] = per_cu;
    } else {
      per_cu = it->second;
    }
  }
  if (per_cu < 1) return fail(SGPU_ELIMIT, "the search kernel does not fit on a CU with %llu bytes of LDS", (unsigned long long)o);
  const uint32_t cap = hook_u32("SGPU_WG_PER_CU", 0);
  if (cap && (uint32_t)per_cu > cap) per_cu = (int)cap;
  uint32_t grid = d->n_cu * (uint32_t)per_cu;
  {
    const bool force = a->coop.enabled == 2;
    const uint64_t uni_bytes = a->lds_bytes - a->L.uni;
    if (a->coop.enabled && !force) {
      const uint32_t rule = (uint32_t)(((uint64_t)48 + 32ull * b->nq) * d->n_cu / 256);
      uint32_t cg = hook_u32("SGPU_COOP_GRID", 0xffffffffu);
      if (cg == 0xffffffffu) cg = std::max<uint32_t>(rule, 8);
      if (cg) grid = std::max<uint32_t>(std::min<uint32_t>(grid, cg), std::min<uint32_t>(b->nq, grid));
    }
    if (a->coop.enabled && grid > 512) {
      if (env_u32("SGPU_DEBUG", 0)) std::fprintf(stderr, "sgpu coop: grid %u capped at 512 (board size)\n", grid);
      grid = 512;
    }
    if (a->coop.enabled) {
      CoopView& c = a->coop;
      c.max_pos = std::min<uint32_t>(65535u, std::max<uint32_t>(a->L.dots_cap, 1u));
      c.max_cand = (uint32_t)std::min<uint64_t>(std::min<uint32_t>(hook_u32("SGPU_COOP_MAX_CAND", 1024), NT), uni_bytes / 20);
      c.chunk = (uint32_t)std::min<uint64_t>(std::min<uint32_t>(std::max<uint32_t>(hook_u32("SGPU_COOP_CHUNK", 128), 1u), std::min<uint32_t>(NT, 1023u)),
                                             uni_bytes / 16);
      c.chunk_min = std::min<uint32_t>(c.chunk, std::max<uint32_t>(hook_u32("SGPU_COOP_CHUNK_MIN", 4), 1u));
      c.min_items = hook_u32("SGPU_COOP_MIN_ITEMS", 64);
      c.first_reach = std::max<uint32_t>(1, hook_u32("SGPU_COOP_FIRST_REACH", 256));
      c.idle_min = hook_u32("SGPU_COOP_IDLE_MIN", force ? 0 : 8);
      c.idle_ratio = hook_u32("SGPU_COOP_IDLE_RATIO", force ? 0 : 1);
      c.poll_sleep = std::max<uint32_t>(1, hook_u32("SGPU_COOP_POLL", 2));
      c.enabled = 1u;
      const size_t o_slots = 128, o_pos = o_slots + (size_t)grid * kCoopSlotWords * 8,
                   o_cand = o_pos + (size_t)grid * c.max_pos * 8, o_trace = o_cand + (size_t)grid * c.max_cand * 16,
                   total = o_trace + (size_t)grid * 16 * 8;
      if (lane->coop_bytes < total) {
        if (lane->coop) {
          HIP_TRY(hipStreamSynchronize(lane->stream));
          (void)hipFree(lane->coop);
        }
        lane->coop = nullptr;
        lane->coop_bytes = 0;
        if (hipMalloc((void**)&lane->coop, total) != hipSuccess)
          return fail(SGPU_ENOMEM, "hipMalloc of the %zu-byte cooperative board failed", total);
        lane->coop_bytes = total;
        HIP_TRY(hipMemsetAsync(lane->coop, 0, total, lane->stream));
      } else if (lane->coop_bytes && hook_u32("SGPU_COOP_RESET", 0)) {
        HIP_TRY(hipMemsetAsync(lane->coop, 0, o_pos, lane->stream));
      }
      if (env_u32("SGPU_DEBUG", 0))
        std::fprintf(stderr, "sgpu coop: board %p..%p slots@%zu pos@%zu cand@%zu grid %u max_pos %u max_cand %u chunk %u..%u min_items %u idle_min %u idle_ratio %u\n",
                     (void*)lane->coop, (void*)(lane->coop + total), o_slots, o_pos, o_cand, grid, c.max_pos, c.max_cand, c.chunk_min, c.chunk,
                     c.min_items, c.idle_min, c.idle_ratio);
      c.open = (uint64_t*)lane->coop;
      c.counters = (uint32_t*)(lane->coop + 64);
      c.slots = (uint64_t*)(lane->coop + o_slots);
      c.pos_pub = (uint64_t*)(lane->coop + o_pos);
      c.cands = (uint64_t*)(lane->coop + o_cand);
      c.trace = nullptr;
      if (hook_u32("SGPU_COOP_TRACE", 0)) {
        c.trace = (uint64_t*)(lane->coop + o_trace);
        HIP_TRY(hipMemsetAsync(lane->coop + o_trace, 0, (size_t)grid * 16 * 8, lane->stream));
        lane->coop_trace_off = o_trace;
        lane->coop_trace_n = grid * 16;
      }
    }
  }
  if (a->coop.enabled && b->nq <= d->n_cu && !hook_get("SGPU_ITEMS_INIT"))
    a->p.items_init = std::min<uint32_t>(a->p.items_max, std::max<uint32_t>(1, hook_u32("SGPU_COOP_ITEMS_INIT", 128)));
  if (!a->coop.enabled) grid = std::max<uint32_t>(1, std::min<uint32_t>(grid, b->nq));
  a->grid = grid;
  b->done_seq = 0;
  if (a->coop.enabled && b->staged && b->direct_out && b->status && env_u32("SGPU_EARLY_DONE", 1)) {
    lane->done_seq = lane->done_seq == 0xffffffffu ? 1u : lane->done_seq + 1u;
    b->done_seq = lane->done_seq;
    a->qb.done = b->status + 1;
    a->qb.done_seq = b->done_seq;
  }
  a->bitmaps = nullptr;
  if (a->counted) {
    if (lane->bitmaps_slots < grid) {
      if (lane->bitmaps) {
        HIP_TRY(hipStreamSynchronize(lane->stream));
        (void)hipFree(lane->bitmaps);
      }
      lane->bitmaps = nullptr;
      lane->bitmaps_slots = 0;
      const uint32_t slots = std::max<uint32_t>(grid, d->n_cu * (uint32_t)per_cu);
      const size_t bytes = (size_t)slots * std::max<uint32_t>(d->view.n_bitmap_words, 1) * 4;
      if (hipMalloc((void**)&lane->bitmaps, bytes) != hipSuccess)
        return fail(SGPU_ENOMEM, "hipMalloc of %zu bytes of visited bitmaps failed", bytes);
      HIP_TRY(hipMemsetAsync(lane->bitmaps, 0, bytes, lane->stream));
      lane->bitmaps_slots = slots;
    }
    a->bitmaps = lane->bitmaps;
  }
  a->queue = b->staged ? b->queue_dev : lane->queue;
  lane->coop_last = a->coop.enabled != 0;
  return SGPU_OK;
}

static void drain_events(Lane* l) {
  for (int i = 0; i < l->ev_pending; ++i) {
    float ms = 0;
    if (hipEventElapsedTime(&ms, l->ev0[i], l->ev1[i]) == hipSuccess) {
      l->sum_ms += ms;
      l->n_timed += 1;
    }
  }
  l->ev_pending = 0;
}

static sgpu_status coop_report(DeviceIndex* d, Lane* lane, uint32_t code) {
  if (!code) return SGPU_OK;
  if (code >= 16) {
    (void)hipStreamSynchronize(lane->stream);
    return fail(SGPU_EDEVICE, "search kernel (streamed stage 2): a bounded wait gave up (code %u)", code);
  }
  if (lane->coop) (void)hipMemsetAsync(lane->coop + 64 + 12, 0, 4, lane->stream);
  (void)hipStreamSynchronize(lane->stream);
  if (!d->coop_broken) std::fprintf(stderr, "seismic_hip: cooperative search kernel reported protocol error %u on device %d; "
                                            "the cooperative variant is switched off for this index replica\n", code, d->device);
  d->coop_broken = true;
  return fail(SGPU_EDEVICE, "cooperative search kernel: protocol wait gave up (code %u)", code);
}
static sgpu_status coop_check_board(DeviceIndex* d, Lane* lane) {
  uint32_t flag = 0;
  HIP_TRY(hipMemcpy(&flag, lane->queue + 32, 4, hipMemcpyDeviceToHost));
  if (flag) {
    (void)hipMemset(lane->queue + 32, 0, 4);
    return coop_report(d, lane, flag);
  }
  if (!lane->coop || !lane->coop_last) return SGPU_OK;
  HIP_TRY(hipMemcpy(&flag, lane->coop + 64 + 12, 4, hipMemcpyDeviceToHost));
  return coop_report(d, lane, flag);
}

sgpu_status batch_run(DeviceIndex* d, Lane* lane, sgpu_batch* b, const sgpu_search_params& sp, uint32_t mode,
                      int sync, sgpu_launch_stats* stats) {
  if (!d) return fail(SGPU_EDEVICE, "index is not uploaded to a device (call sgpu_index_upload)");
  if (!b || b->owner != d) return fail(SGPU_EINVAL, "batch does not belong to this index replica");
  if (!lane) lane = &d->main;
  HIP_TRY(hipSetDevice(d->device));
  if (b->nq == 0) {
    if (stats) *stats = sgpu_launch_stats{};
    return SGPU_OK;
  }
  env_refresh();
  {
    std::lock_guard<std::mutex> lock(d->mu);
    LaunchArgs a{};
    sgpu_status st = configure(d, lane, b, sp, mode, &a);
    if (st != SGPU_OK) return st;
    if (lane->ev_pending == (int)lane->ev0.size()) {
      HIP_TRY(hipStreamSynchronize(lane->stream));
      drain_events(lane);
    }
    HIP_TRY(hipMemsetAsync(lane->queue, 0, 4, lane->stream));
    if (a.qb.out_stats) HIP_TRY(hipMemsetAsync(b->out_stats, 0, (size_t)b->nq * STATS_WORDS * 4, lane->stream));
    const int e = lane->ev_pending++;
    HIP_TRY(hipEventRecord(lane->ev0[e], lane->stream));
    HIP_TRY(launch_search(a));
    HIP_TRY(hipEventRecord(lane->ev1[e], lane->stream));
    lane->last.n_queries = b->nq;
    lane->last.grid = a.grid;
    lane->last.block = a.block;
    lane->last.lds_bytes = a.lds_bytes;
  }
  if (sync) {
    HIP_TRY(hipStreamSynchronize(lane->stream));
    std::lock_guard<std::mutex> lock(d->mu);
    float ms = 0;
    HIP_TRY(hipEventElapsedTime(&ms, lane->ev0[lane->ev_pending - 1], lane->ev1[lane->ev_pending - 1]));
    drain_events(lane);
    lane->last.kernel_ms = ms;
    if (stats) *stats = lane->last;
  }
  return SGPU_OK;
}

sgpu_status batch_sync(DeviceIndex* d, sgpu_launch_stats* stats) {
  if (!d) return fail(SGPU_EDEVICE, "index is not uploaded to a device");
  Lane* l = &d->main;
  HIP_TRY(hipSetDevice(d->device));
  HIP_TRY(hipStreamSynchronize(l->stream));
  std::lock_guard<std::mutex> lock(d->mu);
  drain_events(l);
  if (stats) {
    *stats = l->last;
    stats->kernel_ms = l->n_timed ? (float)(l->sum_ms / l->n_timed) : 0.0f;
  }
  l->sum_ms = 0;
  l->n_timed = 0;
  return SGPU_OK;
}

sgpu_status batch_fetch(DeviceIndex* d, Lane* lane, sgpu_batch* b, uint32_t k, float* out_scores, uint64_t* out_ids,
                        uint32_t* out_n) {
  if (!d || !b) return fail(SGPU_EINVAL, "null index/batch");
  if (k == 0 || k > b->k_max) return fail(SGPU_EINVAL, "k out of range for this batch");
  if (!lane) lane = &d->main;
  HIP_TRY(hipSetDevice(d->device));
  if (b->nq == 0) {
    HIP_TRY(hipStreamSynchronize(lane->stream));
    return SGPU_OK;
  }
  if (k == b->k_max) {
    HIP_TRY(hipMemcpyAsync(out_scores, b->out_scores, (size_t)b->nq * k * 4, hipMemcpyDeviceToHost, lane->stream));
    HIP_TRY(hipMemcpyAsync(out_ids, b->out_ids, (size_t)b->nq * k * 8, hipMemcpyDeviceToHost, lane->stream));
  } else {
    HIP_TRY(hipMemcpy2DAsync(out_scores, (size_t)k * 4, b->out_scores, (size_t)b->k_max * 4, (size_t)k * 4, b->nq,
                             hipMemcpyDeviceToHost, lane->stream));
    HIP_TRY(hipMemcpy2DAsync(out_ids, (size_t)k * 8, b->out_ids, (size_t)b->k_max * 8, (size_t)k * 8, b->nq,
                             hipMemcpyDeviceToHost, lane->stream));
  }
  HIP_TRY(hipMemcpyAsync(out_n, b->out_n, (size_t)b->nq * 4, hipMemcpyDeviceToHost, lane->stream));
  HIP_TRY(hipStreamSynchronize(lane->stream));
  return coop_check_board(d, lane);
}

sgpu_status batch_fetch_stats(DeviceIndex* d, sgpu_batch* b, uint32_t* out) {
  if (!d || !b || !out) return fail(SGPU_EINVAL, "null index/batch/out");
  HIP_TRY(hipSetDevice(d->device));
  HIP_TRY(hipStreamSynchronize(d->main.stream));
  if (b->nq) HIP_TRY(hipMemcpy(out, b->out_stats, (size_t)b->nq * STATS_WORDS * 4, hipMemcpyDeviceToHost));
  return SGPU_OK;
}

uint32_t coop_trace_dump(DeviceIndex* d, uint64_t* out, uint32_t cap) {
  if (!d) return 0;
  (void)hipSetDevice(d->device);
  Lane* lanes[DeviceIndex::kPool + 1];
  int nl = 0;
  lanes[nl++] = &d->main;
  for (Lane& l : d->pool) lanes[nl++] = &l;
  for (int i = 0; i < nl; ++i) {
    Lane* l = lanes[i];
    if (!l->coop || !l->coop_trace_n) continue;
    (void)hipStreamSynchronize(l->stream);
    const uint32_t n = std::min<uint32_t>(cap, l->coop_trace_n);
    if (hipMemcpy(out, l->coop + l->coop_trace_off, (size_t)n * 8, hipMemcpyDeviceToHost) != hipSuccess) return 0;
    return n;
  }
  return 0;
}

static inline size_t al16(size_t x) { return (x + 15) & ~(size_t)15; }

sgpu_status staged_launch(DeviceIndex* d, Lane* lane, uint64_t dim, const uint64_t* q_off, const uint32_t* comps,
                          const float* vals, uint32_t nq, uint32_t q_base, const sgpu_search_params& sp, sgpu_batch** slot,
                          uint32_t followed, const FilterRef* flt, uint32_t chunk) {
  if (!d) return fail(SGPU_EDEVICE, "index is not uploaded to a device (call sgpu_index_upload)");
  if (sp.k == 0) return fail(SGPU_EINVAL, "k must be > 0 (KHeap::new asserts, reference src/utils.rs:23)");
  if (sp.k > 1024) return fail(SGPU_ELIMIT, "k = %u exceeds the heap limit of 1024", sp.k);
  uint32_t max_nnz = 0;
  PhaseClock pc;
  env_refresh();
  if (!q_off || q_off[0] != 0) return fail(SGPU_EINVAL, "q_off[0] must be 0");
  sgpu_status st = validate_query_offsets(q_off, nq, q_base, &max_nnz);
  if (st != SGPU_OK) return st;
  if (q_off[nq] && (!comps || !vals)) return fail(SGPU_EINVAL, "null query arrays");
  bool validated = false;
  HIP_TRY(hipSetDevice(d->device));
  const uint64_t nnz = q_off[nq];
  const uint32_t k = sp.k;
  const size_t o_fix = 16, o_off = 32, o_comp = o_off + al16((size_t)(nq + 1) * 4), o_val = o_comp + al16(nnz * 4),
               o_order = o_val + al16(nnz * 4), o_status = o_order + al16((size_t)nq * 8),
               in_bytes = o_status + 16;
  const size_t r_n = in_bytes, r_sc = r_n + al16((size_t)nq * 4), r_id = r_sc + al16((size_t)nq * k * 4),
               total = r_id + al16((size_t)nq * k * 8);
  sgpu_batch* b = *slot;
  if (b && (!b->staged || b->owner != d || b->arena_cap < total)) {
    HIP_TRY(hipStreamSynchronize(lane->stream));
    batch_free(b);
    b = nullptr;
    *slot = nullptr;
  }
  if (!b) {
    b = new (std::nothrow) sgpu_batch();
    if (!b) return fail(SGPU_ENOMEM, "out of host memory");
    b->staged = true;
    b->device = d->device;
    b->owner = d;
    b->arena_cap = std::max<size_t>(std::min<size_t>(total * 5 / 2, total + ((size_t)64 << 20)), 1 << 16);
    if (hipMalloc((void**)&b->arena_dev, b->arena_cap) != hipSuccess ||
        hipHostMalloc((void**)&b->arena_host, b->arena_cap, hipHostMallocMapped | hipHostMallocCoherent) != hipSuccess) {
      batch_free(b);
      return fail(SGPU_ENOMEM, "allocation of a %zu-byte staging arena failed", b->arena_cap);
    }
    if (hipHostGetDevicePointer((void**)&b->arena_host_dev, b->arena_host, 0) != hipSuccess) b->arena_host_dev = nullptr;
    *slot = b;
    if (hook_raw("SGPU_DEBUG_ALLOC")) std::fprintf(stderr, "sgpu alloc: arena %p..%p\n", (void*)b->arena_dev, (void*)(b->arena_dev + b->arena_cap));
  }
  b->nq = nq;
  b->k_max = k;
  b->max_nnz = max_nnz;
  b->in_bytes = in_bytes;
  b->q_base = q_base;
  b->order_off = o_order;
  b->out_off = r_n;
  b->out_bytes = total - r_n;
  if (nq == 0) {
    b->status_off = o_status;
    return SGPU_OK;
  }
  const uint32_t direct_max = hook_u32("SGPU_DIRECT_OUT_MAX", 16);
  const uint32_t qn = std::max<uint32_t>(4, (max_nnz + 3u) & ~3u);
  const uint32_t cut = std::min<uint32_t>(sp.query_cut, qn);
  try {
    b->plans.clear();
    b->plans.emplace_back();
  } catch (const std::bad_alloc&) {
    return fail(SGPU_ENOMEM, "out of host memory planning a query batch");
  }
  b->device_plan_cut = 0xffffffffu;
  b->followed = followed != 0;
  b->plan_identity = false;
  {
    uint32_t seen = device_plan_dots(d, sp, nq, cut);
    if (seen && chunk > 0 && later_chunks_on_host()) seen = 0;
    if (seen && nq <= direct_max) seen = 0;
    if (!seen) {
      st = validate_queries(dim, q_off, comps, vals, nq, &max_nnz, q_base);
      if (st != SGPU_OK) return st;
      validated = true;
    }
    if (seen) {
      sgpu_batch_plan& pl = b->plans.back();
      pl.query_cut = cut;
      pl.dots_cap = std::max(seen, std::max<uint32_t>(d->max_nb, 1));
      pl.max_nb = 0;
      pl.max_list_nb = std::max<uint32_t>(d->max_nb, 1);
      pl.hash_ok = false;
      pl.order.clear();
      b->device_plan_cut = cut;
      b->plan_identity = followed == 2 && hook_u32("SGPU_PLAN_IDENTITY", 1) != 0;
    } else {
      st = make_plan(d, q_off, comps, vals, nq, cut, &b->plans.back());
      if (st != SGPU_OK) return st;
      if (nq >= kDevicePlanMinQueries) {
        std::lock_guard<std::mutex> lock(d->mu);
        uint32_t& v = d->plan_dots_seen[cut];
        v = std::max(v, b->plans.back().dots_cap);
      }
    }
  }
  pc.lap(0);
  uint8_t* hs = b->arena_host;
  std::memset(hs, 0, 16);
  uint32_t* h32 = (uint32_t*)(hs + o_off);
  for (uint32_t q = 0; q <= nq; ++q) h32[q] = (uint32_t)q_off[q];
  if (nnz) {
    std::memcpy(hs + o_comp, comps, nnz * 4);
    std::memcpy(hs + o_val, vals, nnz * 4);
  }
  if (b->device_plan_cut == 0xffffffffu) std::memcpy(hs + o_order, b->plans.back().order.data(), (size_t)nq * 8);
  std::memset(hs + o_status, 0, 16);
  std::memset(hs + o_fix, 0, 16);
  const uint32_t direct_in_on = env_u32("SGPU_DIRECT_IN", 1);
  b->direct_out = b->arena_host_dev != nullptr && nq <= direct_max;
  b->direct_in = b->direct_out && direct_in_on != 0;
  uint8_t* in_base = b->direct_in ? b->arena_host_dev : b->arena_dev;
  b->queue_dev = b->direct_in ? lane->queue + 16 : (uint32_t*)b->arena_dev;
  b->queue_base = 0;
  b->q_off = (uint32_t*)(in_base + o_off);
  b->q_comp = (uint32_t*)(in_base + o_comp);
  b->q_val = (float*)(in_base + o_val);
  b->q_order = (uint32_t*)(in_base + o_order);
  b->order_cut = cut;
  uint8_t* out_base = b->direct_out ? b->arena_host_dev : b->arena_dev;
  b->out_n = (uint32_t*)(out_base + r_n);
  b->out_scores = (float*)(out_base + r_sc);
  b->out_ids = (uint64_t*)(out_base + r_id);
  b->out_stats = nullptr;
  b->status_off = b->direct_out ? o_fix : o_status;
  b->status = (uint32_t*)(out_base + b->status_off);
  pc.lap(1);
  if (b->direct_in) {
    if (lane->queue_dirty) {
      HIP_TRY(hipMemsetAsync(lane->queue + 16, 0, 4, lane->stream));
      lane->queue_pos = 0;
      lane->queue_dirty = false;
    }
    b->queue_base = lane->queue_pos;
  } else {
    HIP_TRY(hipMemcpyAsync(b->arena_dev, hs, in_bytes, hipMemcpyHostToDevice, lane->stream));
    if (!validated) {
      st = validate_queries(dim, q_off, comps, vals, nq, &max_nnz, q_base);
      if (st != SGPU_OK) {
        const std::string msg = last_error();
        (void)hipStreamSynchronize(lane->stream);
        last_error() = msg;
        return st;
      }
      validated = true;
    }
  }
  const DevView* view = &d->view;
  if (flt && flt->f) {
    const FilterDeviceView* fv = nullptr;
    st = filter_view(flt->f, flt->replica, &fv);
    if (st != SGPU_OK) {
      const std::string msg = last_error();
      (void)hipStreamSynchronize(lane->stream);
      last_error() = msg;
      return st;
    }
    view = &fv->view;
    HIP_TRY(hipSetDevice(d->device));
  }
  if (!b->direct_in && b->device_plan_cut != 0xffffffffu && !b->plan_identity) {
    HIP_TRY(launch_device_plan(*view, b->q_off, b->q_comp, b->q_val, nq, cut, (uint64_t*)(b->arena_dev + r_n),
                               (uint32_t*)(b->arena_dev + o_status) + 1, b->q_order, lane->stream));
  }
  pc.lap(2);
  hipError_t he = hipSuccess;
  {
    std::lock_guard<std::mutex> lock(d->mu);
    LaunchArgs a{};
    st = configure(d, lane, b, sp, MODE_SEARCH, &a, view);
    if (st == SGPU_OK) he = launch_search(a);
    if (b->direct_in) {
      if (st == SGPU_OK && he == hipSuccess) lane->queue_pos += nq + a.grid;
      else lane->queue_dirty = true;
    }
  }
  pc.lap(3);
  if (st == SGPU_OK && he == hipSuccess && !b->direct_out)
    he = hipMemcpyAsync(hs + o_status, b->arena_dev + o_status, 16 + b->out_bytes, hipMemcpyDeviceToHost, lane->stream);
  pc.lap(4);
  if (st != SGPU_OK || he != hipSuccess) {
    (void)hipStreamSynchronize(lane->stream);
    if (st == SGPU_OK) st = fail(SGPU_EDEVICE, "launch of the search failed: %s", hipGetErrorString(he));
    return st;
  }
  return SGPU_OK;
}

uint32_t debug_lane_chunk(DeviceIndex* d, uint32_t lane, uint32_t* info4, uint32_t* order_out, uint32_t cap) {
  if (!d || lane >= (uint32_t)DeviceIndex::kPool) return 0;
  std::lock_guard<std::mutex> lk(d->pool_mu);
  const Lane& l = d->pool[lane];
  const sgpu_batch* b = l.scratch;
  if (l.busy || !b || !b->staged || b->nq == 0) return 0;
  const bool host = b->device_plan_cut == 0xffffffffu;
  info4[0] = b->nq;
  info4[1] = b->q_base;
  info4[2] = host ? 0u : (b->plan_identity ? 2u : 1u);
  info4[3] = b->order_cut;
  if (host && order_out) std::memcpy(order_out, b->arena_host + b->order_off, (size_t)std::min<uint32_t>(cap, b->nq) * 4);
  return 1;
}

sgpu_status staged_finish(DeviceIndex* d, Lane* lane, sgpu_batch* b, float* out_scores, uint64_t* out_ids, uint32_t* out_n) {
  HIP_TRY(hipSetDevice(d->device));
  PhaseClock pc;
  {
    const volatile uint32_t* done = (b && b->done_seq) ? (const volatile uint32_t*)(b->arena_host + b->status_off + 4) : nullptr;
    const hipError_t we = wait_lane(lane->stream, b ? b->nq : 0, done, b ? b->done_seq : 0u);
    if (we != hipSuccess) lane->queue_dirty = true;
    HIP_TRY(we);
  }
  pc.lap(5);
  if (!b || b->nq == 0) return SGPU_OK;
  {
    const sgpu_status cs = coop_report(d, lane, *(const volatile uint32_t*)(b->arena_host + b->status_off));
    if (cs != SGPU_OK) {
      lane->queue_dirty = true;
      return cs;
    }
  }
  if (b->device_plan_cut != 0xffffffffu) {
    const uint32_t need = ((const volatile uint32_t*)(b->arena_host + b->status_off))[1];
    std::lock_guard<std::mutex> lock(d->mu);
    uint32_t& v = d->plan_dots_seen[b->device_plan_cut];
    v = std::max(v, need);
  }
  const size_t nq = b->nq, k = b->k_max;
  const uint8_t* r = b->arena_host + b->out_off;
  std::memcpy(out_n, r, nq * 4);
  std::memcpy(out_scores, r + al16(nq * 4), nq * k * 4);
  std::memcpy(out_ids, r + al16(nq * 4) + al16(nq * k * 4), nq * k * 8);
  pc.lap(6);
  return SGPU_OK;
}

sgpu_status summary_distances(DeviceIndex* d, const HostIndex& h, uint32_t list, const uint32_t* comps,
                              const float* vals, uint32_t nnz, float* out_dots, uint32_t* out_nb) {
  if (!d) return fail(SGPU_EDEVICE, "index is not uploaded to a device (call sgpu_index_upload)");
  if (list >= h.dim) return fail(SGPU_EINVAL, "list %u >= dim", list);
  const uint32_t nb = (uint32_t)(h.list_block_start[list + 1] - h.list_block_start[list]);
  *out_nb = nb;
  if (nb == 0 || nnz == 0) {
    for (uint32_t i = 0; i < nb; ++i) out_dots[i] = 0.0f;
    return SGPU_OK;
  }
  const uint64_t q_off[2] = {0, nnz};
  sgpu_batch* b = nullptr;
  sgpu_status st = batch_create(d, &d->main, h.dim, q_off, comps, vals, 1, 1, &b);
  if (st != SGPU_OK) return st;
  sgpu_search_params sp{};
  sp.k = 1;
  sp.query_cut = list;
  sp.heap_factor = 0;
  st = batch_run(d, nullptr, b, sp, MODE_DOTS, 1, nullptr);
  if (st == SGPU_OK) {
    if (hipMemcpy(out_dots, b->out_scores, (size_t)nb * 4, hipMemcpyDeviceToHost) != hipSuccess)
      st = fail(SGPU_EDEVICE, "hipMemcpy of summary dots failed");
  }
  batch_free(b);
  return st;
}


sgpu_status device_index_set_knn(DeviceIndex* d, const std::vector<uint32_t>& knn, uint32_t knn_dim) {
  if (!d) return SGPU_OK;
  std::lock_guard<std::mutex> lock(d->mu);
  HIP_TRY(hipSetDevice(d->device));
  HIP_TRY(hipDeviceSynchronize());
  if (d->view.knn) {
    auto it = std::find_if(d->allocs.begin(), d->allocs.end(), [&](const Alloc& a) { return a.p == (void*)d->view.knn; });
    if (it != d->allocs.end()) d->allocs.erase(it);
    (void)hipFree((void*)d->view.knn);
    d->bytes -= std::min<uint64_t>(d->bytes, d->view.knn_total * 4);
  }
  d->view.knn = nullptr;
  d->view.knn_total = 0;
  d->view.knn_dim = 0;
  if (knn.empty() || !knn_dim) return SGPU_OK;
  sgpu_status st = dev_copy(d, knn.data(), knn.size(), &d->view.knn);
  if (st != SGPU_OK) return st;
  d->view.knn_total = knn.size();
  d->view.knn_dim = knn_dim;
  return SGPU_OK;
}

sgpu_status build_knn_on_device(DeviceIndex* d, HostIndex& h, uint32_t nknn) {
  if (!d) return fail(SGPU_EDEVICE, "index is not uploaded to a device (call sgpu_index_upload)");
  if (nknn == 0 || nknn + 1 > 1024) return fail(SGPU_EINVAL, "nknn must be in 1..1023");
  const uint32_t k = nknn + 1;
  const uint64_t chunk = hook_u32("SGPU_KNN_CHUNK", 32768);
  std::vector<uint32_t> out;
  out.reserve((size_t)h.n_docs * nknn);
  sgpu_search_params sp{};
  sp.k = k;
  sp.query_cut = 10;
  sp.heap_factor = 0.7f;
  sp.n_knn = 0;
  sp.first_sorted = 0;
  sgpu_status st = device_index_set_knn(d, {}, 0);
  if (st != SGPU_OK) return st;
  std::vector<uint64_t> q_off;
  std::vector<uint32_t> q_comp;
  std::vector<float> q_val, sc;
  std::vector<uint64_t> ids;
  std::vector<uint32_t> n;
  for (uint64_t d0 = 0; d0 < h.n_docs; d0 += chunk) {
    const uint64_t d1 = std::min<uint64_t>(h.n_docs, d0 + chunk);
    const uint32_t nq = (uint32_t)(d1 - d0);
    const uint64_t e0 = h.fwd_offsets[d0], e1 = h.fwd_offsets[d1];
    q_off.resize(nq + 1);
    q_comp.resize(e1 - e0);
    q_val.resize(e1 - e0);
    for (uint32_t q = 0; q <= nq; ++q) q_off[q] = h.fwd_offsets[d0 + q] - e0;
    for (uint64_t i = e0; i < e1; ++i) {
      q_comp[i - e0] = h.comp(i);
      q_val[i - e0] = h.val(i);
    }
    sgpu_batch* b = nullptr;
    st = batch_create(d, &d->main, h.dim, q_off.data(), q_comp.data(), q_val.data(), nq, k, &b);
    if (st != SGPU_OK) return st;
    st = batch_run(d, nullptr, b, sp, MODE_SEARCH, 1, nullptr);
    sc.resize((size_t)nq * k);
    ids.resize((size_t)nq * k);
    n.resize(nq);
    if (st == SGPU_OK) st = batch_fetch(d, nullptr, b, k, sc.data(), ids.data(), n.data());
    batch_free(b);
    if (st != SGPU_OK) return st;
    for (uint32_t q = 0; q < nq; ++q) {
      uint32_t taken = 0;
      for (uint32_t i = 0; i < n[q] && taken < nknn; ++i) {
        const uint64_t id = ids[(size_t)q * k + i];
        if (id == d0 + q) continue;
        out.push_back((uint32_t)id);
        ++taken;
      }
    }
  }
  h.knn.swap(out);
  h.knn_dim = nknn;
  return device_index_set_knn(d, h.knn, h.knn_dim);
}

}
```

### seismic_amd/csrc/host_index.cpp

```cpp
#include "host_index.hpp"

#include <cerrno>
#include <cmath>
#include <cstdlib>
#include <exception>

namespace sgpu {

static double cgroup_cpu_quota() {
  const char* root_env = std::getenv("SGPU_CGROUP_ROOT");
  const std::string root = root_env && *root_env ? root_env : "/sys/fs/cgroup";
  double q = 0, per = 0;
  char word[32] = {0};
  if (FILE* f = std::fopen((root + "/cpu.max").c_str(), "r")) {
    const int n = std::fscanf(f, "%31s %lf", word, &per);
    std::fclose(f);
    if (n == 2 && per > 0 && std::strcmp(word, "max") != 0) return std::atof(word) / per;
    if (n == 2) return 0;
  }
  if (FILE* f = std::fopen((root + "/cpu/cpu.cfs_quota_us").c_str(), "r")) {
    const int n = std::fscanf(f, "%lf", &q);
    std::fclose(f);
    if (n == 1 && q > 0) {
      if (FILE* g = std::fopen((root + "/cpu/cpu.cfs_period_us").c_str(), "r")) {
        const int m = std::fscanf(g, "%lf", &per);
        std::fclose(g);
        if (m == 1 && per > 0) return q / per;
      }
    }
  }
  return 0;
}
int default_host_threads(int omp_max_threads) {
  if (const char* e = std::getenv("SGPU_HOST_THREADS")) {
    const int v = std::atoi(e);
    if (v > 0) return v;
  }
  int nt = omp_max_threads > 0 ? omp_max_threads : 1;
  const double quota = cgroup_cpu_quota();
  if (quota > 0) {
    const int cap = (int)(quota + 0.999);
    if (cap >= 1 && cap < nt) nt = cap;
  }
  return nt;
}
std::string& last_error() {
  static thread_local std::string e;
  return e;
}

sgpu_status fail(sgpu_status st, const char* fmt, ...) {
  char buf[512];
  va_list ap;
  va_start(ap, fmt);
  vsnprintf(buf, sizeof buf, fmt, ap);
  va_end(ap);
  last_error() = buf;
  return st;
}

void HostIndex::fill_desc(sgpu_index_desc* d) const {
  std::memset(d, 0, sizeof *d);
  d->comp_width = comp_width;
  d->value_type = value_type;
  d->val_scale = value_type == SGPU_VAL_F16 ? 0.0f : val_scale;
  d->n_docs = n_docs;
  d->dim = dim;
  d->nnz = nnz();
  d->n_blocks = n_blocks();
  d->n_postings = n_postings();
  d->n_rows = n_rows();
  d->n_entries = n_entries();
  d->fwd_offsets = fwd_offsets.data();
  d->fwd_comps = fwd_comps.data();
  d->fwd_vals = value_type == SGPU_VAL_F16 ? (const void*)fwd_vals.data() : (const void*)fwd_codes.data();
  d->list_block_start = list_block_start.data();
  d->block_post_start = block_post_start.data();
  d->post_doc = post_doc.data();
  d->blk_min = blk_min.data();
  d->blk_quant = blk_quant.data();
  d->list_row_start = list_row_start.data();
  d->row_comp = row_comp.data();
  d->row_ptr = row_ptr.data();
  d->sum_bid = sum_bid.data();
  d->sum_code = sum_code.data();
}

static bool monotone(const uint64_t* a, uint64_t n_plus_1, uint64_t last) {
  if (a[0] != 0) return false;
  for (uint64_t i = 1; i < n_plus_1; ++i)
    if (a[i] < a[i - 1]) return false;
  return a[n_plus_1 - 1] == last;
}

sgpu_status validate_desc(const sgpu_index_desc& d) {
  if (d.comp_width != 2 && d.comp_width != 4) return fail(SGPU_EINVAL, "comp_width must be 2 or 4");
  if (d.dim == 0) return fail(SGPU_EINVAL, "dim == 0");
  if (d.value_type > SGPU_VAL_DOTVBYTE) return fail(SGPU_EINVAL, "unknown value_type %u", d.value_type);
  if (d.value_type == SGPU_VAL_DOTVBYTE && d.comp_width != 2)
    return fail(SGPU_EINVAL, "a DotVByte index has u16 components (reference src/pylib/dotvbyte.rs:20-27)");
  if (d.value_type != SGPU_VAL_F16) {
    int e = 0;
    if (!(d.val_scale > 0.0f) || std::frexp(d.val_scale, &e) != 0.5f) return fail(SGPU_EINVAL, "val_scale must be a positive power of two");
  }
  if (d.comp_width == 2 && d.dim > 65535) return fail(SGPU_EINVAL, "dim %llu does not fit u16 components (at most 65535; use comp_width 4)", (unsigned long long)d.dim);
  if (d.dim > 0xffffffffull || d.n_docs > 0x7fffffffull) return fail(SGPU_EINVAL, "dim/n_docs out of range");
  if (!d.fwd_offsets || !d.list_block_start || !d.block_post_start || !d.list_row_start || !d.row_ptr)
    return fail(SGPU_EINVAL, "null offset array in descriptor");
  if (!monotone(d.fwd_offsets, d.n_docs + 1, d.nnz)) return fail(SGPU_EINVAL, "fwd_offsets not monotone / nnz mismatch");
  if (!monotone(d.list_block_start, d.dim + 1, d.n_blocks)) return fail(SGPU_EINVAL, "list_block_start not monotone / n_blocks mismatch");
  if (!monotone(d.block_post_start, d.n_blocks + 1, d.n_postings)) return fail(SGPU_EINVAL, "block_post_start not monotone / n_postings mismatch");
  if (!monotone(d.list_row_start, d.dim + 1, d.n_rows)) return fail(SGPU_EINVAL, "list_row_start not monotone / n_rows mismatch");
  if (!monotone(d.row_ptr, d.n_rows + 1, d.n_entries)) return fail(SGPU_EINVAL, "row_ptr not monotone / n_entries mismatch");
  if ((d.nnz && (!d.fwd_comps || !d.fwd_vals)) || (d.n_postings && !d.post_doc) ||
      (d.n_blocks && (!d.blk_min || !d.blk_quant)) || (d.n_rows && !d.row_comp) ||
      (d.n_entries && (!d.sum_bid || !d.sum_code)))
    return fail(SGPU_EINVAL, "null data array in descriptor");
  auto compv = [&](const void* p, uint64_t i) -> uint32_t {
    return d.comp_width == 2 ? (uint32_t)((const uint16_t*)p)[i] : ((const uint32_t*)p)[i];
  };
  for (uint64_t doc = 0; doc < d.n_docs; ++doc) {
    const uint64_t s = d.fwd_offsets[doc], e = d.fwd_offsets[doc + 1];
    if (e - s > 65535) return fail(SGPU_EINVAL, "document %llu has more than 65535 components (16-bit length, reference src/posting_list.rs:45-48)", (unsigned long long)doc);
    if (d.value_type == SGPU_VAL_DOTVBYTE && e - s > 32767) return fail(SGPU_ELIMIT, "document %llu has more than 32767 components (DotVByte forward index)", (unsigned long long)doc);
    for (uint64_t i = s; i < e; ++i) {
      const uint32_t c = compv(d.fwd_comps, i);
      if (c >= d.dim) return fail(SGPU_EINVAL, "document component >= dim");
      if (i > s && c <= compv(d.fwd_comps, i - 1)) return fail(SGPU_EINVAL, "document %llu components not strictly ascending", (unsigned long long)doc);
    }
  }
  for (uint64_t p = 0; p < d.n_postings; ++p)
    if (d.post_doc[p] >= d.n_docs) return fail(SGPU_EINVAL, "posting refers to doc >= n_docs");
  for (uint64_t c = 0; c < d.dim; ++c) {
    const uint64_t nb = d.list_block_start[c + 1] - d.list_block_start[c];
    if (nb > 65535) return fail(SGPU_EINVAL, "list %llu has more than 65535 blocks (reference src/posting_list.rs:243-246)", (unsigned long long)c);
    for (uint64_t r = d.list_row_start[c]; r < d.list_row_start[c + 1]; ++r) {
      const uint32_t rc = compv(d.row_comp, r);
      if (rc >= d.dim) return fail(SGPU_EINVAL, "summary row component >= dim");
      if (r > d.list_row_start[c] && rc <= compv(d.row_comp, r - 1)) return fail(SGPU_EINVAL, "summary rows of list %llu not strictly ascending", (unsigned long long)c);
      for (uint64_t e = d.row_ptr[r]; e < d.row_ptr[r + 1]; ++e) {
        if (d.sum_bid[e] >= nb) return fail(SGPU_EINVAL, "summary entry block id out of range");
        if (e > d.row_ptr[r] && d.sum_bid[e] <= d.sum_bid[e - 1]) return fail(SGPU_EINVAL, "summary row block ids not strictly ascending");
      }
    }
  }
  return SGPU_OK;
}

sgpu_status host_index_from_desc(const sgpu_index_desc& d, HostIndex* out) {
  sgpu_status st = validate_desc(d);
  if (st != SGPU_OK) return st;
  try {
    HostIndex& h = *out;
    h.comp_width = d.comp_width;
    h.n_docs = d.n_docs;
    h.dim = d.dim;
    h.fwd_offsets.assign(d.fwd_offsets, d.fwd_offsets + d.n_docs + 1);
    h.fwd_comps.assign((const uint8_t*)d.fwd_comps, (const uint8_t*)d.fwd_comps + d.nnz * d.comp_width);
    h.value_type = d.value_type;
    h.val_scale = d.value_type == SGPU_VAL_F16 ? 0.0f : d.val_scale;
    if (d.value_type == SGPU_VAL_F16) h.fwd_vals.assign((const uint16_t*)d.fwd_vals, (const uint16_t*)d.fwd_vals + d.nnz);
    else h.fwd_codes.assign((const uint8_t*)d.fwd_vals, (const uint8_t*)d.fwd_vals + d.nnz);
    h.list_block_start.assign(d.list_block_start, d.list_block_start + d.dim + 1);
    h.block_post_start.assign(d.block_post_start, d.block_post_start + d.n_blocks + 1);
    h.post_doc.assign(d.post_doc, d.post_doc + d.n_postings);
    h.blk_min.assign(d.blk_min, d.blk_min + d.n_blocks);
    h.blk_quant.assign(d.blk_quant, d.blk_quant + d.n_blocks);
    h.list_row_start.assign(d.list_row_start, d.list_row_start + d.dim + 1);
    h.row_comp.assign((const uint8_t*)d.row_comp, (const uint8_t*)d.row_comp + d.n_rows * d.comp_width);
    h.row_ptr.assign(d.row_ptr, d.row_ptr + d.n_rows + 1);
    h.sum_bid.assign(d.sum_bid, d.sum_bid + d.n_entries);
    h.sum_code.assign(d.sum_code, d.sum_code + d.n_entries);
  } catch (const std::bad_alloc&) {
    return fail(SGPU_ENOMEM, "out of host memory copying the index descriptor");
  }
  return SGPU_OK;
}

sgpu_status validate_query_offsets(const uint64_t* q_off, uint32_t nq, uint32_t q_base, uint32_t* max_nnz) {
  if (!q_off) return fail(SGPU_EINVAL, "null q_off");
  uint32_t mx = 0;
  for (uint32_t q = 0; q < nq; ++q) {
    if (q_off[q + 1] < q_off[q]) return fail(SGPU_EINVAL, "q_off not monotone");
    const uint64_t n = q_off[q + 1] - q_off[q];
    if (n > 0xffffu)
      return fail(SGPU_ELIMIT, "query %u has %llu components (limit 65535)", q_base + q, (unsigned long long)n);
    mx = std::max<uint32_t>(mx, (uint32_t)n);
  }
  if (q_off[nq] - q_off[0] >= 0xffffffffull) return fail(SGPU_ELIMIT, "batch too large");
  *max_nnz = mx;
  return SGPU_OK;
}

sgpu_status validate_queries(uint64_t dim, const uint64_t* q_off, const uint32_t* comps, const float* vals,
                             uint32_t nq, uint32_t* max_nnz, uint32_t q_base) {
  if (!q_off || q_off[0] != 0) return fail(SGPU_EINVAL, "q_off[0] must be 0");
  uint32_t mx = 0;
  const sgpu_status ost = validate_query_offsets(q_off, nq, q_base, &mx);
  if (ost != SGPU_OK) return ost;
  if (q_off[nq] && (!comps || !vals)) return fail(SGPU_EINVAL, "null query arrays");
  int bad_kind = 0;
  uint32_t bad_q = 0xffffffffu;
  const uint32_t dim32 = dim > 0xffffffffull ? 0xffffffffu : (uint32_t)dim;
  for (uint32_t q = 0; q < nq && !bad_kind; ++q) {
    const uint64_t a = q_off[q], e = q_off[q + 1];
    uint32_t bad = 0;
    for (uint64_t i = a; i < e; ++i) bad |= (uint32_t)(comps[i] >= dim32) | (uint32_t)(vals[i] != vals[i]);
    for (uint64_t i = a + 1; i < e; ++i) bad |= (uint32_t)(comps[i] <= comps[i - 1]);
    if (!bad) continue;
    for (uint64_t i = a; i < e && !bad_kind; ++i) {
      if (comps[i] >= dim) bad_kind = 1;
      else if (i > a && comps[i] <= comps[i - 1]) bad_kind = 2;
      else if (std::isnan(vals[i])) bad_kind = 3;
    }
    bad_q = q_base + q;
  }
  if (bad_kind == 1) return fail(SGPU_EINVAL, "query %u: component >= dim", bad_q);
  if (bad_kind == 2) return fail(SGPU_EINVAL, "query %u: components must be strictly ascending", bad_q);
  if (bad_kind == 3) return fail(SGPU_EINVAL, "query %u: NaN value", bad_q);
  *max_nnz = mx;
  return SGPU_OK;
}

static const char kMagic[8] = {'S', 'G', 'P', 'U', 'I', 'D', 'X', '2'};
static constexpr int kHdr = 12;

template <class T>
static bool wr(FILE* f, const std::vector<T>& v) {
  return v.empty() || fwrite(v.data(), sizeof(T), v.size(), f) == v.size();
}
template <class T>
static bool rd(FILE* f, std::vector<T>& v, uint64_t n) {
  v.resize(n);
  return n == 0 || fread(v.data(), sizeof(T), n, f) == n;
}

sgpu_status host_index_save(const HostIndex& ix, const char* path) {
  FILE* f = fopen(path, "wb");
  if (!f) return fail(SGPU_EIO, "cannot open %s for writing: %s", path, strerror(errno));
  uint32_t scale_bits = 0;
  std::memcpy(&scale_bits, &ix.val_scale, 4);
  uint64_t hdr[kHdr] = {ix.comp_width,   ix.n_docs,   ix.dim,         ix.nnz(),   ix.n_blocks(),
                        ix.n_postings(), ix.n_rows(), ix.n_entries(), ix.knn.empty() ? 0u : ix.knn_dim, ix.knn.size(),
                        ix.value_type,   scale_bits};
  bool ok = fwrite(kMagic, 1, 8, f) == 8 && fwrite(hdr, 8, kHdr, f) == kHdr && wr(f, ix.fwd_offsets) &&
            wr(f, ix.fwd_comps) && wr(f, ix.fwd_vals) && wr(f, ix.fwd_codes) && wr(f, ix.list_block_start) &&
            wr(f, ix.block_post_start) && wr(f, ix.post_doc) && wr(f, ix.blk_min) && wr(f, ix.blk_quant) &&
            wr(f, ix.list_row_start) && wr(f, ix.row_comp) && wr(f, ix.row_ptr) && wr(f, ix.sum_bid) &&
            wr(f, ix.sum_code) && wr(f, ix.knn);
  ok = (fclose(f) == 0) && ok;
  if (!ok) return fail(SGPU_EIO, "short write to %s", path);
  return SGPU_OK;
}

sgpu_status host_index_load(const char* path, HostIndex* out) {
  FILE* f = fopen(path, "rb");
  if (!f) return fail(SGPU_EIO, "cannot open %s: %s", path, strerror(errno));
  char magic[8];
  uint64_t hdr[kHdr] = {0};
  static const char kMagic1[8] = {'S', 'G', 'P', 'U', 'I', 'D', 'X', '1'};
  bool got = fread(magic, 1, 8, f) == 8;
  const bool v1 = got && memcmp(magic, kMagic1, 8) == 0;
  got = got && (v1 || memcmp(magic, kMagic, 8) == 0);
  if (got && v1) {
    uint64_t h1[10];
    got = fread(h1, 8, 10, f) == 10;
    if (got) {
      for (int i = 0; i < 10; ++i) hdr[i] = h1[i];
      hdr[10] = SGPU_VAL_F16;
      hdr[11] = 0;
    }
  } else if (got) {
    got = fread(hdr, 8, kHdr, f) == kHdr;
  }
  if (!got) {
    fclose(f);
    return fail(SGPU_EIO, "%s is not an SGPUIDX1 / SGPUIDX2 index file", path);
  }
  HostIndex& h = *out;
  h.comp_width = (uint32_t)hdr[0];
  h.n_docs = hdr[1];
  h.dim = hdr[2];
  const uint64_t nnz = hdr[3], nb = hdr[4], np = hdr[5], nr = hdr[6], ne = hdr[7], knn_dim = hdr[8], nk = hdr[9];
  h.value_type = (uint32_t)hdr[10];
  {
    const uint32_t scale_bits = (uint32_t)hdr[11];
    std::memcpy(&h.val_scale, &scale_bits, 4);
  }
  bool ok = (h.comp_width == 2 || h.comp_width == 4) && h.value_type <= SGPU_VAL_DOTVBYTE &&
            (h.value_type != SGPU_VAL_DOTVBYTE || h.comp_width == 2);
  const uint64_t vb = h.value_type == SGPU_VAL_F16 ? 2 : 1;
  if (ok) {
    const uint64_t lim = 1ull << 48;
    ok = h.n_docs < lim && h.dim < lim && nnz < lim && nb < lim && np < lim && nr < lim && ne < lim && nk < lim &&
         knn_dim <= 0xffffffffull && ((knn_dim == 0) == (nk == 0));
    long pos = ftell(f);
    ok = ok && pos >= 0 && fseek(f, 0, SEEK_END) == 0;
    const long end = ok ? ftell(f) : -1;
    ok = ok && end >= 0 && fseek(f, pos, SEEK_SET) == 0;
    if (ok) {
      const uint64_t cw = h.comp_width;
      const uint64_t need = 8 * (h.n_docs + 1) + nnz * cw + nnz * vb + 8 * (h.dim + 1) + 8 * (nb + 1) + 4 * np + 8 * nb +
                            8 * (h.dim + 1) + nr * cw + 8 * (nr + 1) + 3 * ne + 4 * nk;
      ok = (uint64_t)(end - pos) == need;
    }
  }
  if (!ok) {
    fclose(f);
    return fail(SGPU_EIO, "corrupt index file %s (header does not match the file size)", path);
  }
  try {
    ok = rd(f, h.fwd_offsets, h.n_docs + 1) && rd(f, h.fwd_comps, nnz * h.comp_width) &&
         rd(f, h.fwd_vals, vb == 2 ? nnz : 0) && rd(f, h.fwd_codes, vb == 1 ? nnz : 0) &&
         rd(f, h.list_block_start, h.dim + 1) && rd(f, h.block_post_start, nb + 1) &&
         rd(f, h.post_doc, np) && rd(f, h.blk_min, nb) && rd(f, h.blk_quant, nb) &&
         rd(f, h.list_row_start, h.dim + 1) && rd(f, h.row_comp, nr * h.comp_width) && rd(f, h.row_ptr, nr + 1) &&
         rd(f, h.sum_bid, ne) && rd(f, h.sum_code, ne) && rd(f, h.knn, nk);
  } catch (const std::bad_alloc&) {
    fclose(f);
    return fail(SGPU_ENOMEM, "out of host memory loading %s", path);
  } catch (const std::exception& e) {
    fclose(f);
    return fail(SGPU_EIO, "cannot load %s: %s", path, e.what());
  }
  fclose(f);
  if (!ok) return fail(SGPU_EIO, "truncated or corrupt index file %s", path);
  h.knn_dim = (uint32_t)knn_dim;
  for (uint32_t id : h.knn)
    if (id >= h.n_docs) return fail(SGPU_EIO, "corrupt index file %s: kNN neighbour id >= n_docs", path);
  sgpu_index_desc d;
  h.fill_desc(&d);
  return validate_desc(d);
}

sgpu_status host_index_convert(const HostIndex& src, uint32_t value_type, HostIndex* out) {
  if (value_type > SGPU_VAL_DOTVBYTE) return fail(SGPU_EINVAL, "unknown value_type %u", value_type);
  if (value_type == SGPU_VAL_DOTVBYTE) {
    if (src.comp_width != 2) return fail(SGPU_EINVAL, "a DotVByte index has u16 components (reference src/pylib/dotvbyte.rs:20-27)");
    for (uint64_t doc = 0; doc < src.n_docs; ++doc)
      if (src.fwd_offsets[doc + 1] - src.fwd_offsets[doc] > 32767)
        return fail(SGPU_ELIMIT, "document %llu has more than 32767 components (DotVByte forward index)", (unsigned long long)doc);
  }
  try {
    *out = src;
    HostIndex& h = *out;
    const uint64_t nnz = src.nnz();
    if (value_type == src.value_type) return SGPU_OK;
    if (value_type != SGPU_VAL_F16 && src.value_type != SGPU_VAL_F16) {
      h.value_type = value_type;
      return SGPU_OK;
    }
    if (value_type != SGPU_VAL_F16) {
      float vmax = 0.0f;
      for (uint64_t i = 0; i < nnz; ++i) {
        const float v = src.val(i);
        if (v > vmax) vmax = v;
      }
      float step = 0.00390625f;
      while (255.0f * step < vmax) step *= 2.0f;
      h.value_type = value_type;
      h.val_scale = step;
      h.fwd_codes.resize(nnz);
      h.fwd_vals.clear();
      h.fwd_vals.shrink_to_fit();
#pragma omp parallel for schedule(static) num_threads(sgpu::host_threads())
      for (int64_t i = 0; i < (int64_t)nnz; ++i) {
        const float r = std::round(src.val((uint64_t)i) / step);
        h.fwd_codes[(size_t)i] = r >= 255.0f ? 255 : (r > 0.0f ? (uint8_t)r : 0);
      }
    } else {
      h.value_type = SGPU_VAL_F16;
      h.val_scale = 0.0f;
      h.fwd_vals.resize(nnz);
      for (uint64_t i = 0; i < nnz; ++i) h.fwd_vals[i] = f32_to_f16_sat(src.val(i));
      h.fwd_codes.clear();
      h.fwd_codes.shrink_to_fit();
    }
  } catch (const std::bad_alloc&) {
    return fail(SGPU_ENOMEM, "out of host memory converting the index");
  }
  return SGPU_OK;
}

}
```

### seismic_amd/csrc/host_index.hpp

```cpp
#pragma once
#include <cstdint>
#include <atomic>
#include <mutex>
#include <vector>

#include "common.hpp"

namespace sgpu {

struct DeviceIndex;
struct ExactFile;
struct ScoreState;

struct HostIndex {
  uint32_t comp_width = 2;
  uint64_t n_docs = 0, dim = 0;
  std::vector<uint64_t> fwd_offsets;
  std::vector<uint8_t> fwd_comps;
  std::vector<uint16_t> fwd_vals;
  std::vector<uint8_t> fwd_codes;
  uint32_t value_type = SGPU_VAL_F16;
  float val_scale = 0.0f;
  std::vector<uint64_t> list_block_start, block_post_start;
  std::vector<uint32_t> post_doc;
  std::vector<float> blk_min, blk_quant;
  std::vector<uint64_t> list_row_start;
  std::vector<uint8_t> row_comp;
  std::vector<uint64_t> row_ptr;
  std::vector<uint16_t> sum_bid;
  std::vector<uint8_t> sum_code;
  std::vector<uint32_t> knn;
  uint32_t knn_dim = 0;

  uint64_t nnz() const { return fwd_offsets.empty() ? 0 : fwd_offsets.back(); }
  uint64_t n_blocks() const { return list_block_start.empty() ? 0 : list_block_start.back(); }
  uint64_t n_postings() const { return block_post_start.empty() ? 0 : block_post_start.back(); }
  uint64_t n_rows() const { return list_row_start.empty() ? 0 : list_row_start.back(); }
  uint64_t n_entries() const { return row_ptr.empty() ? 0 : row_ptr.back(); }
  inline uint32_t comp(uint64_t i) const {
    return comp_width == 2 ? (uint32_t)((const uint16_t*)fwd_comps.data())[i]
                           : ((const uint32_t*)fwd_comps.data())[i];
  }
  inline float val(uint64_t i) const {
    return value_type == SGPU_VAL_F16 ? f16_to_f32(fwd_vals[i]) : (float)fwd_codes[i] * val_scale;
  }
  inline uint32_t val_bytes() const { return value_type == SGPU_VAL_F16 ? 2u : 1u; }
  inline uint32_t rcomp(uint64_t i) const {
    return comp_width == 2 ? (uint32_t)((const uint16_t*)row_comp.data())[i]
                           : ((const uint32_t*)row_comp.data())[i];
  }
  void fill_desc(sgpu_index_desc* d) const;
};

sgpu_status validate_desc(const sgpu_index_desc& d);
sgpu_status host_index_from_desc(const sgpu_index_desc& d, HostIndex* out);
sgpu_status host_index_save(const HostIndex& ix, const char* path);
sgpu_status host_index_load(const char* path, HostIndex* out);
sgpu_status host_index_convert(const HostIndex& src, uint32_t value_type, HostIndex* out);

sgpu_status validate_queries(uint64_t dim, const uint64_t* q_off, const uint32_t* comps, const float* vals,
                             uint32_t nq, uint32_t* max_nnz, uint32_t q_base = 0);
sgpu_status validate_query_offsets(const uint64_t* q_off, uint32_t nq, uint32_t q_base, uint32_t* max_nnz);
void pack_dvb_raw_flags(const HostIndex& h, std::vector<uint8_t>* raw);
void pack_record_offsets(const HostIndex& h, const std::vector<uint8_t>& raw, uint64_t line16, std::vector<uint64_t>* rec_off16);
void pack_records(const HostIndex& h, const std::vector<uint8_t>& raw, const std::vector<uint64_t>& rec_off16, std::vector<uint8_t>* fwd);
void pack_block_sizes(const HostIndex& h, const std::vector<uint8_t>& raw, std::vector<uint64_t>* bsize);
void pack_post_refs(const HostIndex& h, const std::vector<uint8_t>& raw, const std::vector<uint64_t>& rec_off16,
                    const std::vector<uint64_t>& bsize, bool block_major, uint64_t blk_base, std::vector<uint64_t>* pref);
void pack_doc_refs(const HostIndex& h, const std::vector<uint8_t>& raw, const std::vector<uint64_t>& rec_off16, std::vector<uint64_t>* dref);
void pack_narrow(const std::vector<uint64_t>& v, std::vector<uint32_t>* out);
void pack_row_mid(const HostIndex& h, std::vector<uint16_t>* mid);
bool pack_row_dir(const HostIndex& h, const std::vector<uint16_t>& mid, std::vector<uint32_t>* out, uint32_t* n_buckets);
void pack_sum_deq(const HostIndex& h, std::vector<float>* deq);

sgpu_status build_host_index(uint32_t comp_width, uint64_t n_docs, uint64_t dim, const uint64_t* offsets,
                             const void* comps, const float* vals, const sgpu_build_config& cfg,
                             HostIndex* out);
sgpu_status exact_search_host(const HostIndex& ix, const uint64_t* q_off, const uint32_t* comps,
                              const float* vals, uint32_t nq, uint32_t k, uint32_t num_threads,
                              float* out_scores, uint64_t* out_ids, uint32_t* out_n, const uint32_t* allow = nullptr);
void exact_file_free(ExactFile* f);
constexpr uint32_t kScoreMaxQueryNnz = 8192;
sgpu_status score_check_args(const HostIndex& h, const uint64_t* q_off, const uint32_t* comps, const float* vals, uint32_t nq,
                             const uint64_t* cand_off, const uint64_t* cand_ids, const float* out_scores, uint32_t* max_nnz);
sgpu_status score_documents_host(const HostIndex& h, const uint64_t* q_off, const uint32_t* comps, const float* vals, uint32_t nq,
                                 const uint64_t* cand_off, const uint64_t* cand_ids, uint32_t num_threads, float* out_scores);
void score_state_free(ScoreState* s);

struct FilterRef {
  const sgpu_filter* f;
  uint32_t replica;
};

}

struct sgpu_index {
  sgpu::HostIndex host;
  std::vector<sgpu::DeviceIndex*> replicas;
  sgpu::DeviceIndex* dev = nullptr;
  std::atomic<uint32_t> next_replica{0};
  std::vector<sgpu::ExactFile*> exact;
  std::mutex exact_mu;
  std::vector<sgpu::ScoreState*> score;
  std::mutex score_mu;
  std::atomic<uint64_t> generation{0};
};
```

Baseline: 1.753 million.

## Fuse query validation into host planning, radix-sort plan keys, add load-aware first-chunk planning

Result: no change. 1.754 million, median of 3 (+0.0%).

```diff
diff --git a/include/seismic_hip_testing.h b/include/seismic_hip_testing.h
--- a/include/seismic_hip_testing.h
+++ b/include/seismic_hip_testing.h
@@ -10,11 +10,16 @@
 uint32_t sgpu_debug_call_bounds(uint32_t nq, uint32_t chunk_min, uint32_t chunk_max, uint32_t lanes_free, uint32_t first_pm,
                                 uint32_t* bounds, uint32_t cap);
 uint32_t sgpu_debug_lane_chunk(sgpu_index* idx, uint32_t lane, uint32_t* info4, uint32_t* order_out, uint32_t cap);
+uint32_t sgpu_debug_pending_queries(sgpu_index* idx, uint32_t replica);
+uint32_t sgpu_debug_first_chunk_rule(uint64_t other_pending, uint32_t chunk_nq, uint32_t n_chunks, uint32_t device_could_plan);
+uint32_t sgpu_debug_chunk_events(sgpu_index* idx, double* out7, uint32_t cap);
 sgpu_status sgpu_debug_pack_forward(const sgpu_index* idx, uint8_t* out_fwd, uint64_t cap, uint64_t* out_doc_ref,
                                     uint64_t* out_bytes);
 sgpu_status sgpu_debug_row_dir(const sgpu_index* idx, uint32_t* out, uint64_t cap_words, uint64_t* n_words, uint32_t* n_buckets);
 sgpu_status sgpu_debug_plan(const sgpu_index* idx, const uint64_t* q_off, const uint32_t* comps, const float* vals,
                             uint32_t nq, uint32_t query_cut, uint32_t* order_out, uint32_t* out3);
+sgpu_status sgpu_debug_plan_checked(const sgpu_index* idx, const uint64_t* q_off, const uint32_t* comps, const float* vals,
+                                    uint32_t nq, uint32_t q_base, uint32_t query_cut, uint32_t* order_out, uint32_t* out3);
 sgpu_status sgpu_debug_device_plan(sgpu_index* idx, const uint64_t* q_off, const uint32_t* comps, const float* vals,
                                    uint32_t nq, uint32_t query_cut, uint32_t* order_out, uint32_t* out3);
 void sgpu_debug_call_timing(double* buf8);
diff --git a/seismic_amd/csrc/abi.cpp b/seismic_amd/csrc/abi.cpp
--- a/seismic_amd/csrc/abi.cpp
+++ b/seismic_amd/csrc/abi.cpp
@@ -36,7 +36,13 @@
 sgpu_status staged_launch(DeviceIndex* d, Lane* lane, uint64_t dim, const uint64_t* q_off, const uint32_t* comps,
                           const float* vals, uint32_t nq, uint32_t q_base, const sgpu_search_params& sp, sgpu_batch** slot,
                           uint32_t followed,
-                          const FilterRef* flt, uint32_t chunk);
+                          const FilterRef* flt, uint32_t chunk,
+                          uint64_t other_pending);
+bool first_chunk_on_host(uint64_t other_pending, uint32_t chunk_nq, bool device_could_plan, bool multi_chunk, uint32_t mode);
+uint32_t first_chunk_mode();
+uint32_t pending_queries(const DeviceIndex* d);
+uint64_t pending_for_rule(const DeviceIndex* d, uint32_t own);
+uint32_t chunk_events_read(DeviceIndex* d, double* out, uint32_t cap);
 sgpu_status staged_finish(DeviceIndex* d, Lane* lane, sgpu_batch* b, float* out_scores, uint64_t* out_ids, uint32_t* out_n);
 sgpu_status summary_distances(DeviceIndex* d, const HostIndex& h, uint32_t list, const uint32_t* comps,
                               const float* vals, uint32_t nnz, float* out_dots, uint32_t* out_nb);
@@ -46,7 +52,7 @@
 sgpu_status debug_device_plan(DeviceIndex* d, const uint64_t* q_off, const uint32_t* comps, const float* vals, uint32_t nq,
                               uint32_t query_cut, uint32_t* order_out, uint32_t* out3);
 sgpu_status debug_plan(const HostIndex& h, const uint64_t* q_off, const uint32_t* comps, const float* vals, uint32_t nq,
-                       uint32_t query_cut, uint32_t* order_out, uint32_t* out3);
+                       uint32_t query_cut, uint32_t* order_out, uint32_t* out3, bool check, uint32_t q_base);
 uint32_t coop_trace_dump(DeviceIndex* d, uint64_t* out, uint32_t cap);
 uint32_t debug_lane_chunk(DeviceIndex* d, uint32_t lane, uint32_t* info4, uint32_t* order_out, uint32_t cap);
 const DeviceIndex* batch_replica(const sgpu_batch* b);
@@ -372,7 +378,9 @@
   }();
   const uint32_t nq = s1 - s0;
   const bool device_plans = device_plan_dots(d, params, std::min<uint32_t>(std::max<uint32_t>(nq / 2, 1u), kChunkQueriesMax), params.query_cut) != 0;
-  const uint32_t chunk_max = chunk_max_env ? chunk_max_env : ((shared || device_plans) ? 2u : 4u);
+  uint32_t chunk_max = chunk_max_env ? chunk_max_env : ((shared || device_plans) ? 2u : 4u);
+  if (device_plans && nq <= kChunkQueriesMax && first_chunk_mode() == 2 && first_chunk_on_host(pending_for_rule(d, 0), nq, true, false, 2))
+    chunk_max = 1;
   Job jobs[8];
   const uint32_t cmin = chunk_min != 0xffffffffu ? chunk_min : (device_plans ? 1300u : 600u);
   uint32_t n_jobs = chunk_jobs(nq, cmin, chunk_max);
@@ -409,7 +417,7 @@
   const uint32_t k = params.k;
   sgpu_status st = SGPU_OK;
   std::string msg;
-  uint32_t launched = 0;
+  uint32_t launched = 0, own_pending = 0;
   if (n_jobs > 1 || s0 != 0) {
     uint32_t max_nnz = 0;
     st = q_off[0] != 0 ? fail(SGPU_EINVAL, "q_off[0] must be 0") : validate_query_offsets(q_off + s0, nq, q_base + s0, &max_nnz);
@@ -424,8 +432,8 @@
     }
     st = staged_launch(d, jb.lane, dim, qo, comps ? comps + q_off[jb.q0] : nullptr, vals ? vals + q_off[jb.q0] : nullptr,
                        jb.q1 - jb.q0, q_base + jb.q0, params, lane_scratch(jb.lane), j + 1 < n_jobs ? 2u : (shared ? 1u : 0u),
-                       flt, j);
-    if (st == SGPU_OK) ++launched;
+                       flt, j, pending_for_rule(d, own_pending));
+    if (st == SGPU_OK) ++launched, own_pending += jb.q1 - jb.q0;
     else msg = last_error();
   }
   for (uint32_t j = 0; j < launched; ++j) {
@@ -705,7 +713,36 @@
                             uint32_t query_cut, uint32_t* order_out, uint32_t* out3) {
   SGPU_HOOK_OR(SGPU_EINVAL);
   if (!idx || !q_off || !order_out || !out3) return fail(SGPU_EINVAL, "null argument");
-  return debug_plan(idx->host, q_off, comps, vals, nq, query_cut, order_out, out3);
+  return debug_plan(idx->host, q_off, comps, vals, nq, query_cut, order_out, out3, false, 0);
+}
+
+sgpu_status sgpu_debug_plan_checked(const sgpu_index* idx, const uint64_t* q_off, const uint32_t* comps, const float* vals,
+                                    uint32_t nq, uint32_t q_base, uint32_t query_cut, uint32_t* order_out, uint32_t* out3) {
+  SGPU_HOOK_OR(SGPU_EINVAL);
+  if (!idx || !q_off || !order_out || !out3) return fail(SGPU_EINVAL, "null argument");
+  if (q_off[0] != 0) return fail(SGPU_EINVAL, "q_off[0] must be 0");
+  uint32_t max_nnz = 0;
+  const sgpu_status st = validate_query_offsets(q_off, nq, q_base, &max_nnz);
+  if (st != SGPU_OK) return st;
+  if (q_off[nq] && (!comps || !vals)) return fail(SGPU_EINVAL, "null query arrays");
+  return debug_plan(idx->host, q_off, comps, vals, nq, query_cut, order_out, out3, true, q_base);
+}
+
+uint32_t sgpu_debug_first_chunk_rule(uint64_t other_pending, uint32_t chunk_nq, uint32_t n_chunks, uint32_t device_could_plan) {
+  SGPU_HOOK_OR(0u);
+  return first_chunk_on_host(other_pending, chunk_nq, device_could_plan != 0, n_chunks > 1, first_chunk_mode()) ? 1u : 0u;
+}
+
+uint32_t sgpu_debug_pending_queries(sgpu_index* idx, uint32_t replica) {
+  SGPU_HOOK_OR(0u);
+  if (!idx || replica >= idx->replicas.size()) return 0u;
+  return pending_queries(idx->replicas[replica]);
+}
+
+uint32_t sgpu_debug_chunk_events(sgpu_index* idx, double* out7, uint32_t cap) {
+  SGPU_HOOK_OR(0u);
+  if (!idx || !idx->dev || (!out7 && cap)) return 0u;
+  return chunk_events_read(idx->dev, out7, cap);
 }
 
 sgpu_status sgpu_debug_device_plan(sgpu_index* idx, const uint64_t* q_off, const uint32_t* comps, const float* vals, uint32_t nq,
diff --git a/seismic_amd/csrc/device_index.hip b/seismic_amd/csrc/device_index.hip
--- a/seismic_amd/csrc/device_index.hip
+++ b/seismic_amd/csrc/device_index.hip
@@ -7,7 +7,9 @@
 #include <condition_variable>
 #include <cstdlib>
 #include <cstring>
+#include <functional>
 #include <mutex>
+#include <thread>
 #include <unordered_map>
 #include <vector>
 
@@ -108,6 +110,12 @@
   std::mutex mu;
   std::atomic<uint32_t> calls_inflight{0};
   std::atomic<int64_t> concurrent_seen_us{-((int64_t)1 << 60)};
+  std::atomic<uint32_t> pending{0};
+  struct ChunkEvent {
+    hipEvent_t e0, e1;
+    uint32_t thread, lane, chunk, planner, nq;
+  };
+  std::vector<ChunkEvent> chunk_events;
   std::mutex pool_mu;
   std::condition_variable pool_cv;
 };
@@ -206,6 +214,10 @@
   if (d->device >= 0) (void)hipSetDevice(d->device);
   lane_free(&d->main);
   for (Lane& l : d->pool) lane_free(&l);
+  for (const DeviceIndex::ChunkEvent& ce : d->chunk_events) {
+    (void)hipEventDestroy(ce.e0);
+    (void)hipEventDestroy(ce.e1);
+  }
   for (const Alloc& a : d->allocs) (void)hipFree(a.p);
   delete d;
 }
@@ -502,6 +514,7 @@
   uint32_t device_plan_cut = 0xffffffffu;
   bool followed = false;
   bool plan_identity = false;
+  uint32_t pending_nq = 0;
   uint32_t q_base = 0;
   size_t order_off = 0;
 };
@@ -701,65 +714,18 @@
 static inline size_t al16_(size_t x) { return (x + 15) & ~(size_t)15; }
 
 static sgpu_status make_plan(const DeviceIndex* d, const uint64_t* h_off, const uint32_t* h_comp, const float* h_val,
-                             uint32_t nq, uint32_t query_cut, sgpu_batch_plan* out) {
+                             uint32_t nq, uint32_t query_cut, sgpu_batch_plan* out, bool check = false, uint64_t dim = 0,
+                             uint32_t q_base = 0) {
   try {
     sgpu_batch_plan& pl = *out;
     pl.query_cut = query_cut;
-    std::vector<uint64_t> keys(nq);
-    uint32_t max_nb = 0, dots_cap = 1, max_list_nb = 1;
-    {
-      constexpr uint32_t kSmall = 16;
-      std::vector<std::pair<int32_t, uint32_t>> kv;
-      for (int64_t q = 0; q < (int64_t)nq; ++q) {
-        const uint64_t qa = h_off[q], qe = h_off[q + 1];
-        int32_t tk[kSmall];
-        uint32_t tc[kSmall];
-        const uint32_t* sel = tc;
-        size_t nl = 0;
-        if (query_cut == 0) {
-        } else if (query_cut <= kSmall) {
-          for (uint64_t i = qa; i < qe; ++i) {
-            const int32_t key = total_key(h_val[i]);
-            if (nl == query_cut && !(key > tk[nl - 1])) continue;
-            size_t j = nl < query_cut ? nl++ : nl - 1;
-            while (j > 0 && tk[j - 1] < key) {
-              tk[j] = tk[j - 1];
-              tc[j] = tc[j - 1];
-              --j;
-            }
-            tk[j] = key;
-            tc[j] = h_comp[i];
-          }
-        } else {
-          kv.clear();
-          for (uint64_t i = qa; i < qe; ++i) kv.emplace_back(total_key(h_val[i]), h_comp[i]);
-          nl = std::min<size_t>(query_cut, kv.size());
-          std::partial_sort(kv.begin(), kv.begin() + (long)nl, kv.end(),
-                            [](const std::pair<int32_t, uint32_t>& a, const std::pair<int32_t, uint32_t>& c) {
-                              if (a.first != c.first) return a.first > c.first;
-                              return a.second < c.second;
-                            });
-        }
-        uint64_t np = 0;
-        uint32_t nb = 0;
-        for (size_t i = 0; i < nl; ++i) {
-          const uint32_t c = query_cut <= kSmall ? sel[i] : kv[i].second;
-          nb += d->list_nb[c];
-          np += d->list_np[c];
-          max_list_nb = std::max(max_list_nb, d->list_nb[c]);
-        }
-        const uint32_t c0 = nl ? (query_cut <= kSmall ? sel[0] : kv[0].second) : 0xffffffffu;
-        if (nl) max_nb = std::max(max_nb, d->list_nb[c0]);
-        dots_cap = std::max(dots_cap, nb);
-        keys[(size_t)q] = ((uint64_t)(0xffffffffu - (uint32_t)std::min<uint64_t>(np, 0xffffffffull)) << 32) | (uint32_t)q;
-      }
-    }
-    pl.max_nb = max_nb;
-    pl.dots_cap = dots_cap;
-    pl.max_list_nb = max_list_nb;
-    std::sort(keys.begin(), keys.end());
-    pl.order.resize(2 * (size_t)nq);
-    for (uint32_t i = 0; i < nq; ++i) pl.order[i] = (uint32_t)keys[i];
+    uint32_t out3[3];
+    const sgpu_status pst = plan_queries(d->list_nb.data(), d->list_np.data(), h_off, h_comp, h_val, nq, query_cut, check, dim,
+                                         q_base, &pl.order, out3);
+    if (pst != SGPU_OK) return pst;
+    pl.dots_cap = out3[0];
+    pl.max_nb = out3[1];
+    pl.max_list_nb = out3[2];
     pl.hash_ok = d->view.dim < (1u << 24) && d->comp_width == 4 && d->value_type == SGPU_VAL_F16 && !hook_u32("SGPU_NO_HASH", 0);
     if (pl.hash_ok) {
       std::vector<uint32_t> stamp(kHashSlots, 0xffffffffu);
@@ -790,7 +756,7 @@
 }
 
 sgpu_status debug_plan(const HostIndex& h, const uint64_t* q_off, const uint32_t* comps, const float* vals, uint32_t nq,
-                       uint32_t query_cut, uint32_t* order_out, uint32_t* out3) {
+                       uint32_t query_cut, uint32_t* order_out, uint32_t* out3, bool check, uint32_t q_base) {
   DeviceIndex d;
   d.comp_width = h.comp_width;
   d.view.dim = (uint32_t)h.dim;
@@ -802,7 +768,7 @@
   }
   sgpu_batch_plan pl;
   env_refresh();
-  const sgpu_status st = make_plan(&d, q_off, comps, vals, nq, query_cut, &pl);
+  const sgpu_status st = make_plan(&d, q_off, comps, vals, nq, query_cut, &pl, check, h.dim, q_base);
   if (st != SGPU_OK) return st;
   for (uint32_t i = 0; i < nq; ++i) order_out[i] = pl.order[i];
   out3[0] = pl.dots_cap;
@@ -826,6 +792,25 @@
   env_refresh();
   const char* v = env_get("SGPU_CHUNK_PLAN");
   return !(v && !std::strcmp(v, "device"));
+}
+
+bool first_chunk_on_host(uint64_t other_pending, uint32_t chunk_nq, bool device_could_plan, bool multi_chunk, uint32_t mode) {
+  if (mode == 0 || !device_could_plan || chunk_nq == 0) return false;
+  if (!multi_chunk && mode != 2) return false;
+  return other_pending >= chunk_nq;
+}
+uint32_t first_chunk_mode() {
+  env_refresh();
+  const char* v = env_get("SGPU_FIRST_CHUNK_PLAN");
+  if (v && !std::strcmp(v, "loaded")) return 1u;
+  if (v && !std::strcmp(v, "call")) return 2u;
+  return 0u;
+}
+uint32_t pending_queries(const DeviceIndex* d) { return d ? d->pending.load(std::memory_order_relaxed) : 0u; }
+uint64_t pending_for_rule(const DeviceIndex* d, uint32_t own) {
+  env_refresh();
+  const uint32_t all = pending_queries(d);
+  return (uint64_t)(all > own ? all - own : 0u) + hook_u32("SGPU_PENDING_ADD", 0);
 }
 
 sgpu_status debug_device_plan(DeviceIndex* d, const uint64_t* q_off, const uint32_t* comps, const float* vals, uint32_t nq,
@@ -1358,7 +1343,7 @@
 
 sgpu_status staged_launch(DeviceIndex* d, Lane* lane, uint64_t dim, const uint64_t* q_off, const uint32_t* comps,
                           const float* vals, uint32_t nq, uint32_t q_base, const sgpu_search_params& sp, sgpu_batch** slot,
-                          uint32_t followed, const FilterRef* flt, uint32_t chunk) {
+                          uint32_t followed, const FilterRef* flt, uint32_t chunk, uint64_t other_pending) {
   if (!d) return fail(SGPU_EDEVICE, "index is not uploaded to a device (call sgpu_index_upload)");
   if (sp.k == 0) return fail(SGPU_EINVAL, "k must be > 0 (KHeap::new asserts, reference src/utils.rs:23)");
   if (sp.k > 1024) return fail(SGPU_ELIMIT, "k = %u exceeds the heap limit of 1024", sp.k);
@@ -1406,6 +1391,7 @@
   b->max_nnz = max_nnz;
   b->in_bytes = in_bytes;
   b->q_base = q_base;
+  b->pending_nq = 0;
   b->order_off = o_order;
   b->out_off = r_n;
   b->out_bytes = total - r_n;
@@ -1429,11 +1415,7 @@
     uint32_t seen = device_plan_dots(d, sp, nq, cut);
     if (seen && chunk > 0 && later_chunks_on_host()) seen = 0;
     if (seen && nq <= direct_max) seen = 0;
-    if (!seen) {
-      st = validate_queries(dim, q_off, comps, vals, nq, &max_nnz, q_base);
-      if (st != SGPU_OK) return st;
-      validated = true;
-    }
+    if (seen && chunk == 0 && first_chunk_on_host(other_pending, nq, true, followed == 2, first_chunk_mode())) seen = 0;
     if (seen) {
       sgpu_batch_plan& pl = b->plans.back();
       pl.query_cut = cut;
@@ -1445,8 +1427,9 @@
       b->device_plan_cut = cut;
       b->plan_identity = followed == 2 && hook_u32("SGPU_PLAN_IDENTITY", 1) != 0;
     } else {
-      st = make_plan(d, q_off, comps, vals, nq, cut, &b->plans.back());
+      st = make_plan(d, q_off, comps, vals, nq, cut, &b->plans.back(), true, dim, q_base);
       if (st != SGPU_OK) return st;
+      validated = true;
       if (nq >= kDevicePlanMinQueries) {
         std::lock_guard<std::mutex> lock(d->mu);
         uint32_t& v = d->plan_dots_seen[cut];
@@ -1528,7 +1511,29 @@
     std::lock_guard<std::mutex> lock(d->mu);
     LaunchArgs a{};
     st = configure(d, lane, b, sp, MODE_SEARCH, &a, view);
-    if (st == SGPU_OK) he = launch_search(a);
+    DeviceIndex::ChunkEvent ce{};
+    const bool timed = st == SGPU_OK && hook_u32("SGPU_CHUNK_EVENTS", 0) != 0 && d->chunk_events.size() < 4096 &&
+                       hipEventCreate(&ce.e0) == hipSuccess;
+    if (timed && hipEventCreate(&ce.e1) != hipSuccess) {
+      (void)hipEventDestroy(ce.e0);
+      st = fail(SGPU_EDEVICE, "hipEventCreate failed");
+    }
+    if (st == SGPU_OK && timed) he = hipEventRecord(ce.e0, lane->stream);
+    if (st == SGPU_OK && he == hipSuccess) he = launch_search(a);
+    if (st == SGPU_OK && timed) {
+      if (he == hipSuccess) he = hipEventRecord(ce.e1, lane->stream);
+      ce.thread = (uint32_t)std::hash<std::thread::id>()(std::this_thread::get_id());
+      ce.lane = (uint32_t)(lane - d->pool);
+      ce.chunk = chunk;
+      ce.planner = b->device_plan_cut == 0xffffffffu ? 0u : (b->plan_identity ? 2u : 1u);
+      ce.nq = nq;
+      try {
+        d->chunk_events.push_back(ce);
+      } catch (const std::bad_alloc&) {
+        (void)hipEventDestroy(ce.e0);
+        (void)hipEventDestroy(ce.e1);
+      }
+    }
     if (b->direct_in) {
       if (st == SGPU_OK && he == hipSuccess) lane->queue_pos += nq + a.grid;
       else lane->queue_dirty = true;
@@ -1543,7 +1548,33 @@
     if (st == SGPU_OK) st = fail(SGPU_EDEVICE, "launch of the search failed: %s", hipGetErrorString(he));
     return st;
   }
+  b->pending_nq = nq;
+  d->pending.fetch_add(nq, std::memory_order_relaxed);
   return SGPU_OK;
+}
+
+uint32_t chunk_events_read(DeviceIndex* d, double* out, uint32_t cap) {
+  if (!d) return 0;
+  (void)hipSetDevice(d->device);
+  std::lock_guard<std::mutex> lock(d->mu);
+  uint32_t n = 0;
+  for (const DeviceIndex::ChunkEvent& ce : d->chunk_events) {
+    float t0 = 0, t1 = 0;
+    if (hipEventSynchronize(ce.e1) != hipSuccess || hipEventElapsedTime(&t0, d->chunk_events[0].e0, ce.e0) != hipSuccess ||
+        hipEventElapsedTime(&t1, d->chunk_events[0].e0, ce.e1) != hipSuccess)
+      break;
+    if (n < cap) {
+      double* r = out + (size_t)n * 7;
+      r[0] = ce.thread, r[1] = ce.lane, r[2] = ce.chunk, r[3] = ce.planner, r[4] = ce.nq, r[5] = (double)t0 * 1e3, r[6] = (double)t1 * 1e3;
+    }
+    ++n;
+  }
+  for (const DeviceIndex::ChunkEvent& ce : d->chunk_events) {
+    (void)hipEventDestroy(ce.e0);
+    (void)hipEventDestroy(ce.e1);
+  }
+  d->chunk_events.clear();
+  return n;
 }
 
 uint32_t debug_lane_chunk(DeviceIndex* d, uint32_t lane, uint32_t* info4, uint32_t* order_out, uint32_t cap) {
@@ -1562,11 +1593,21 @@
 }
 
 sgpu_status staged_finish(DeviceIndex* d, Lane* lane, sgpu_batch* b, float* out_scores, uint64_t* out_ids, uint32_t* out_n) {
+  struct NoLongerPending {
+    DeviceIndex* d;
+    sgpu_batch* b;
+    void release() {
+      if (b && b->pending_nq) d->pending.fetch_sub(b->pending_nq, std::memory_order_relaxed);
+      if (b) b->pending_nq = 0;
+    }
+    ~NoLongerPending() { release(); }
+  } no_longer_pending{d, b};
   HIP_TRY(hipSetDevice(d->device));
   PhaseClock pc;
   {
     const volatile uint32_t* done = (b && b->done_seq) ? (const volatile uint32_t*)(b->arena_host + b->status_off + 4) : nullptr;
     const hipError_t we = wait_lane(lane->stream, b ? b->nq : 0, done, b ? b->done_seq : 0u);
+    no_longer_pending.release();
     if (we != hipSuccess) lane->queue_dirty = true;
     HIP_TRY(we);
   }
diff --git a/seismic_amd/csrc/host_index.cpp b/seismic_amd/csrc/host_index.cpp
--- a/seismic_amd/csrc/host_index.cpp
+++ b/seismic_amd/csrc/host_index.cpp
@@ -199,26 +199,23 @@
   const sgpu_status ost = validate_query_offsets(q_off, nq, q_base, &mx);
   if (ost != SGPU_OK) return ost;
   if (q_off[nq] && (!comps || !vals)) return fail(SGPU_EINVAL, "null query arrays");
-  int bad_kind = 0;
-  uint32_t bad_q = 0xffffffffu;
   const uint32_t dim32 = dim > 0xffffffffull ? 0xffffffffu : (uint32_t)dim;
-  for (uint32_t q = 0; q < nq && !bad_kind; ++q) {
+  for (uint32_t q = 0; q < nq; ++q) {
     const uint64_t a = q_off[q], e = q_off[q + 1];
-    uint32_t bad = 0;
-    for (uint64_t i = a; i < e; ++i) bad |= (uint32_t)(comps[i] >= dim32) | (uint32_t)(vals[i] != vals[i]);
-    for (uint64_t i = a + 1; i < e; ++i) bad |= (uint32_t)(comps[i] <= comps[i - 1]);
-    if (!bad) continue;
-    for (uint64_t i = a; i < e && !bad_kind; ++i) {
-      if (comps[i] >= dim) bad_kind = 1;
-      else if (i > a && comps[i] <= comps[i - 1]) bad_kind = 2;
-      else if (std::isnan(vals[i])) bad_kind = 3;
-    }
-    bad_q = q_base + q;
-  }
-  if (bad_kind == 1) return fail(SGPU_EINVAL, "query %u: component >= dim", bad_q);
-  if (bad_kind == 2) return fail(SGPU_EINVAL, "query %u: components must be strictly ascending", bad_q);
-  if (bad_kind == 3) return fail(SGPU_EINVAL, "query %u: NaN value", bad_q);
+    if (!query_components_bad(dim32, comps, vals, a, e)) continue;
+    const sgpu_status st = fail_query_components(dim, comps, vals, a, e, q_base + q);
+    if (st != SGPU_OK) return st;
+  }
   *max_nnz = mx;
+  return SGPU_OK;
+}
+
+sgpu_status fail_query_components(uint64_t dim, const uint32_t* comps, const float* vals, uint64_t a, uint64_t e, uint32_t q_named) {
+  for (uint64_t i = a; i < e; ++i) {
+    if (comps[i] >= dim) return fail(SGPU_EINVAL, "query %u: component >= dim", q_named);
+    if (i > a && comps[i] <= comps[i - 1]) return fail(SGPU_EINVAL, "query %u: components must be strictly ascending", q_named);
+    if (std::isnan(vals[i])) return fail(SGPU_EINVAL, "query %u: NaN value", q_named);
+  }
   return SGPU_OK;
 }
 
diff --git a/seismic_amd/csrc/host_index.hpp b/seismic_amd/csrc/host_index.hpp
--- a/seismic_amd/csrc/host_index.hpp
+++ b/seismic_amd/csrc/host_index.hpp
@@ -61,6 +61,16 @@
 sgpu_status validate_queries(uint64_t dim, const uint64_t* q_off, const uint32_t* comps, const float* vals,
                              uint32_t nq, uint32_t* max_nnz, uint32_t q_base = 0);
 sgpu_status validate_query_offsets(const uint64_t* q_off, uint32_t nq, uint32_t q_base, uint32_t* max_nnz);
+inline uint32_t query_components_bad(uint32_t dim32, const uint32_t* comps, const float* vals, uint64_t a, uint64_t e) {
+  uint32_t bad = 0;
+  for (uint64_t i = a; i < e; ++i) bad |= (uint32_t)(comps[i] >= dim32) | (uint32_t)(vals[i] != vals[i]);
+  for (uint64_t i = a + 1; i < e; ++i) bad |= (uint32_t)(comps[i] <= comps[i - 1]);
+  return bad;
+}
+sgpu_status fail_query_components(uint64_t dim, const uint32_t* comps, const float* vals, uint64_t a, uint64_t e, uint32_t q_named);
+sgpu_status plan_queries(const uint32_t* list_nb, const uint32_t* list_np, const uint64_t* h_off, const uint32_t* h_comp,
+                         const float* h_val, uint32_t nq, uint32_t query_cut, bool check, uint64_t dim, uint32_t q_base,
+                         std::vector<uint32_t>* order, uint32_t out3[3]);
 void pack_dvb_raw_flags(const HostIndex& h, std::vector<uint8_t>* raw);
 void pack_record_offsets(const HostIndex& h, const std::vector<uint8_t>& raw, uint64_t line16, std::vector<uint64_t>* rec_off16);
 void pack_records(const HostIndex& h, const std::vector<uint8_t>& raw, const std::vector<uint64_t>& rec_off16, std::vector<uint8_t>* fwd);
diff --git a/seismic_amd/csrc/launch_plan.cpp b/seismic_amd/csrc/launch_plan.cpp
--- /dev/null
+++ b/seismic_amd/csrc/launch_plan.cpp
@@ -0,0 +1,120 @@
+#include <algorithm>
+#include <utility>
+#include <vector>
+
+#include "common.hpp"
+#include "host_index.hpp"
+
+namespace sgpu {
+
+static void sort_plan_keys(std::vector<uint64_t>& keys, std::vector<uint64_t>& tmp) {
+  const size_t n = keys.size();
+  if (n < 256) {
+    std::sort(keys.begin(), keys.end());
+    return;
+  }
+  constexpr int kBits = 11, kDigits = 3;
+  constexpr uint32_t kMask = (1u << kBits) - 1;
+  uint32_t all_or = 0, all_and = 0xffffffffu;
+  static thread_local uint32_t hist[kDigits][1u << kBits];
+  std::memset(hist, 0, sizeof(hist));
+  for (size_t i = 0; i < n; ++i) {
+    const uint32_t c = (uint32_t)(keys[i] >> 32);
+    all_or |= c;
+    all_and &= c;
+    ++hist[0][c & kMask];
+    ++hist[1][(c >> kBits) & kMask];
+    ++hist[2][c >> (2 * kBits)];
+  }
+  const uint32_t vary = all_or ^ all_and;
+  tmp.resize(n);
+  uint64_t* src = keys.data();
+  uint64_t* dst = tmp.data();
+  for (int d = 0; d < kDigits; ++d) {
+    const int shift = 32 + d * kBits;
+    if (((vary >> (d * kBits)) & kMask) == 0) continue;
+    uint32_t* h = hist[d];
+    uint32_t pos = 0;
+    for (uint32_t v = 0; v <= kMask; ++v) {
+      const uint32_t c = h[v];
+      h[v] = pos;
+      pos += c;
+    }
+    for (size_t i = 0; i < n; ++i) dst[h[(uint32_t)(src[i] >> shift) & kMask]++] = src[i];
+    std::swap(src, dst);
+  }
+  if (src != keys.data()) keys.swap(tmp);
+}
+
+sgpu_status plan_queries(const uint32_t* list_nb, const uint32_t* list_np, const uint64_t* h_off, const uint32_t* h_comp,
+                         const float* h_val, uint32_t nq, uint32_t query_cut, bool check, uint64_t dim, uint32_t q_base,
+                         std::vector<uint32_t>* order, uint32_t out3[3]) {
+  try {
+    std::vector<uint64_t> keys(nq), tmp;
+    uint32_t max_nb = 0, dots_cap = 1, max_list_nb = 1;
+    const uint32_t dim32 = dim > 0xffffffffull ? 0xffffffffu : (uint32_t)dim;
+    {
+      constexpr uint32_t kSmall = 16;
+      std::vector<std::pair<int32_t, uint32_t>> kv;
+      for (int64_t q = 0; q < (int64_t)nq; ++q) {
+        const uint64_t qa = h_off[q], qe = h_off[q + 1];
+        if (check && query_components_bad(dim32, h_comp, h_val, qa, qe)) {
+          const sgpu_status st = fail_query_components(dim, h_comp, h_val, qa, qe, q_base + (uint32_t)q);
+          if (st != SGPU_OK) return st;
+        }
+        int32_t tk[kSmall];
+        uint32_t tc[kSmall];
+        const uint32_t* sel = tc;
+        size_t nl = 0;
+        if (query_cut == 0) {
+        } else if (query_cut <= kSmall) {
+          for (uint64_t i = qa; i < qe; ++i) {
+            const int32_t key = total_key(h_val[i]);
+            if (nl == query_cut && !(key > tk[nl - 1])) continue;
+            size_t j = nl < query_cut ? nl++ : nl - 1;
+            while (j > 0 && tk[j - 1] < key) {
+              tk[j] = tk[j - 1];
+              tc[j] = tc[j - 1];
+              --j;
+            }
+            tk[j] = key;
+            tc[j] = h_comp[i];
+          }
+        } else {
+          kv.clear();
+          for (uint64_t i = qa; i < qe; ++i) kv.emplace_back(total_key(h_val[i]), h_comp[i]);
+          nl = std::min<size_t>(query_cut, kv.size());
+          std::partial_sort(kv.begin(), kv.begin() + (long)nl, kv.end(),
+                            [](const std::pair<int32_t, uint32_t>& a, const std::pair<int32_t, uint32_t>& c) {
+                              if (a.first != c.first) return a.first > c.first;
+                              return a.second < c.second;
+                            });
+        }
+        uint64_t np = 0;
+        uint32_t nb = 0;
+        for (size_t i = 0; i < nl; ++i) {
+          const uint32_t c = query_cut <= kSmall ? sel[i] : kv[i].second;
+          nb += list_nb[c];
+          np += list_np[c];
+          max_list_nb = std::max(max_list_nb, list_nb[c]);
+        }
+        const uint32_t c0 = nl ? (query_cut <= kSmall ? sel[0] : kv[0].second) : 0xffffffffu;
+        if (nl) max_nb = std::max(max_nb, list_nb[c0]);
+        dots_cap = std::max(dots_cap, nb);
+        keys[(size_t)q] = ((uint64_t)(0xffffffffu - (uint32_t)std::min<uint64_t>(np, 0xffffffffull)) << 32) | (uint32_t)q;
+      }
+    }
+    out3[0] = dots_cap;
+    out3[1] = max_nb;
+    out3[2] = max_list_nb;
+    sort_plan_keys(keys, tmp);
+    order->resize(2 * (size_t)nq);
+    uint32_t* o = order->data();
+    for (uint32_t i = 0; i < nq; ++i) o[i] = (uint32_t)keys[i];
+  } catch (const std::bad_alloc&) {
+    return fail(SGPU_ENOMEM, "out of host memory planning a query batch");
+  }
+  return SGPU_OK;
+}
+
+}
```
